# tlepoint/fhe.rs

Measured on NVIDIA H100. Metric: bfv_ct_mul_relin_per_sec_n32768_14x62bit, higher is better.
Workload: dtype u64

## Files before the change

### fhe_rs_b200/csrc/capi.cu

```cuda
#include <algorithm>
#include <atomic>
#include <cstring>
#include <map>
#include <memory>
#include <mutex>
#include <string>
#include <vector>

#include "../../include/fhe_b200.h"
#include "engine.hpp"
#include "host/precompute.hpp"

using namespace fhe_b200;

namespace {

thread_local std::string g_last_error;

struct ScalerData {
  ScalerTablesH h;
  ScalerDev dev;
};

struct LevelData {
  u32 level = 0, L = 0, E = 0, K = 0;
  RowIds ctx_ids, mul_ids;
  std::vector<u64> mul_moduli;
  ScalerData ext, down;
  bool has_sd = false;
  SwitchDownDev sd;
  u64 q_mod_t = 0;
  std::vector<u64> delta;
  const u64 *d_delta = nullptr, *d_delta_s = nullptr;
};

template <typename ToDev, typename IndexOf>
void upload_scaler_tables(ScalerData& s, const std::vector<u64>& to_moduli, ToDev&& to_dev, IndexOf&& index_of) {
  ScalerDev& d = s.dev;
  std::memset(&d, 0, sizeof(d));
  d.n_from = s.h.n_from; d.n_to = s.h.n_to; d.is_one = s.h.is_one; d.shift = s.h.shift;
  d.tg_lo = s.h.theta_gamma_lo; d.tg_hi = s.h.theta_gamma_hi; d.tg_sign = s.h.theta_gamma_sign;
  for (size_t j = 0; j < to_moduli.size(); j++) d.to_ids[j] = (unsigned short)index_of(to_moduli[j]);
  d.all_solinas = switches().no_solinas ? 0 : 1;
  for (u64 q : to_moduli)
    if ((q >> 61) != 1 || ((1ull << 62) - q) >= (1ull << 28)) d.all_solinas = 0;
  d.gamma = to_dev(s.h.gamma);
  d.omega = to_dev(s.h.omega);
  d.to_lo = to_dev(s.h.theta_omega_lo);
  d.to_hi = to_dev(s.h.theta_omega_hi);
  d.to_sign = to_dev(s.h.theta_omega_sign);
  std::vector<unsigned char> order;
  d.n_pos = 0;
  for (int sg = 0; sg < 2; sg++)
    for (size_t i = 0; i < s.h.theta_omega_sign.size(); i++)
      if ((int)s.h.theta_omega_sign[i] == sg && (s.h.theta_omega_lo[i] | s.h.theta_omega_hi[i]) != 0) {
        order.push_back((unsigned char)i);
        d.n_pos += sg == 0;
      }
  d.n_terms = (u32)order.size();
  if (order.empty()) order.push_back(0);
  d.to_order = to_dev(order);
  d.tgar_lo = to_dev(s.h.theta_garner_lo);
  d.tgar_hi = to_dev(s.h.theta_garner_hi);
}

}

struct fhe_b200_params {
  std::atomic<int> refs{1};
  int device = -1;
  u32 N = 0, logn = 0, Lmax = 0;
  std::vector<u64> moduli, ext, primes, psi;
  std::vector<u32> moduli_sizes;
  BigUint t;
  bool t_small = false;
  PlainMod t_mod{0, 0, 0};
  std::vector<NttTablesH> tables;
  std::vector<LimbDev> h_limbs;
  LimbDev* d_limbs = nullptr;
  std::vector<void*> d_allocs;
  cudaMemPool_t pool = nullptr;
  mutable cudaStream_t side[4] = {nullptr, nullptr, nullptr, nullptr};
  mutable std::mutex mu;
  mutable std::map<u32, std::unique_ptr<LevelData>> levels;
  mutable std::map<u32, int*> perms;

  template <typename T>
  T* to_dev(const std::vector<T>& v) const {
    if (device < 0 || v.empty()) return nullptr;
    T* d = nullptr;
    struct Restore {
      int prev = -1;
      ~Restore() { if (prev >= 0) cudaSetDevice(prev); }
    } restore;
    if (cudaGetDevice(&restore.prev) != cudaSuccess) { cudaGetLastError(); restore.prev = -1; }
    if (restore.prev == device) restore.prev = -1;
    else FHE_CUDA(cudaSetDevice(device));
    FHE_CUDA(cudaMalloc(&d, v.size() * sizeof(T)));
    const_cast<fhe_b200_params*>(this)->d_allocs.push_back(d);
    FHE_CUDA(cudaMemcpy(d, v.data(), v.size() * sizeof(T), cudaMemcpyHostToDevice));
    return d;
  }
  int prime_index(u64 q) const {
    for (size_t i = 0; i < primes.size(); i++)
      if (primes[i] == q) return (int)i;
    return -1;
  }
  void upload_scaler(ScalerData& s, const std::vector<u64>& to_moduli) const {
    upload_scaler_tables(s, to_moduli, [&](const auto& v) { return to_dev(v); }, [&](u64 q) { return prime_index(q); });
  }

  const LevelData& level(u32 lv) const {
    std::lock_guard<std::mutex> g(mu);
    auto it = levels.find(lv);
    if (it != levels.end()) return *it->second;
    if (lv >= Lmax) throw FheError(FHE_B200_INVALID_LEVEL, "InvalidLevel: level " + std::to_string(lv));
    std::unique_ptr<LevelData> d(new LevelData());
    d->level = lv;
    d->L = Lmax - lv;
    u32 bits = 0;
    for (u32 i = 0; i < d->L; i++) bits += moduli_sizes[i];
    d->E = (bits + 60 + 61) / 62;
    d->K = d->L + d->E;
    if (d->K > (u32)kMaxPos) throw FheError(FHE_B200_UNSUPPORTED, "too many limbs");
    std::vector<u64> ctx(moduli.begin(), moduli.begin() + d->L);
    d->mul_moduli = ctx;
    d->mul_moduli.insert(d->mul_moduli.end(), ext.begin(), ext.begin() + d->E);
    std::memset(&d->ctx_ids, 0, sizeof(RowIds));
    std::memset(&d->mul_ids, 0, sizeof(RowIds));
    d->ctx_ids.limbs_per_poly = d->L;
    d->mul_ids.limbs_per_poly = d->K;
    for (u32 i = 0; i < d->L; i++) d->ctx_ids.ids[i] = d->mul_ids.ids[i] = (unsigned short)i;
    for (u32 j = 0; j < d->E; j++) d->mul_ids.ids[d->L + j] = (unsigned short)(Lmax + j);
    RnsContextH from(ctx), to(d->mul_moduli);
    d->ext.h = make_scaler_tables(from, to, BigUint(1), BigUint(1));
    d->down.h = make_scaler_tables(to, from, t, from.product);
    upload_scaler(d->ext, d->mul_moduli);
    upload_scaler(d->down, ctx);
    if (d->L >= 2) {
      d->has_sd = true;
      u64 ql = ctx.back();
      std::vector<u64> half_mod, inv, inv_s;
      for (u32 i = 0; i + 1 < d->L; i++) {
        u64 qi = ctx[i], iv;
        if (!invmod_h(ql % qi, qi, &iv)) throw FheError(FHE_B200_INVALID_MODULUS, "NonCoprimeModuli");
        half_mod.push_back(qi - (ql / 2) % qi);
        inv.push_back(iv);
        inv_s.push_back(ModulusH(qi).shoup(iv));
      }
      d->sd.q_last = ql;
      d->sd.q_last_half = ql / 2;
      d->sd.half_mod = to_dev(half_mod);
      d->sd.inv = to_dev(inv);
      d->sd.inv_s = to_dev(inv_s);
    }
    if (t_small) d->q_mod_t = from.product.mod_u64(t_mod.t);
    std::vector<u64> delta_s;
    for (u64 qi : ctx) {
      u64 iv;
      if (!invmod_h(qi - t.mod_u64(qi), qi, &iv)) throw FheError(FHE_B200_INVALID_MODULUS, "PlaintextModulusNotCoprime");
      d->delta.push_back(iv);
      delta_s.push_back(ModulusH(qi).shoup(iv));
    }
    d->d_delta = to_dev(d->delta);
    d->d_delta_s = to_dev(delta_s);
    auto* raw = d.get();
    levels[lv] = std::move(d);
    return *raw;
  }

  const int* perm(u32 exponent) const {
    std::lock_guard<std::mutex> g(mu);
    auto it = perms.find(exponent);
    if (it != perms.end()) return it->second;
    std::vector<int> p(N);
    auto brev = [&](u32 x) {
      u32 r = 0;
      for (u32 b = 0; b < logn; b++) r |= ((x >> b) & 1) << (logn - 1 - b);
      return r;
    };
    u64 power = (exponent - 1) / 2;
    for (u32 j = 0; j < N; j++) {
      p[brev(j)] = (int)brev((u32)(power & (N - 1)));
      power += exponent;
    }
    int* d = to_dev(p);
    perms[exponent] = d;
    return d;
  }
};

struct fhe_b200_batch {
  const fhe_b200_params* par;
  u32 count, parts, level, limbs;
  int repr;
  bool mul_basis;
  u64* d;
  size_t words_per_ct() const { return ((size_t)parts * limbs) << par->logn; }
};

struct fhe_b200_ksk {
  const fhe_b200_params* par;
  u32 ct_level, ksk_level, n_dig, Lk;
  u32 log_base;
  u64 *k0, *k1;
};

struct fhe_b200_multiplicator {
  const fhe_b200_params* par;
  u32 level = 0, L = 0, K = 0;
  u32 nc_l = 0, nc_r = 0, nc_d = 0;
  std::vector<u64> mul_moduli, plan_primes;
  RowIds mul_ids;
  std::vector<LimbDev> h_limbs;
  LimbDev* d_limbs = nullptr;
  ScalerData ext_l, ext_r, down;
  std::vector<void*> d_allocs;
  template <typename T>
  T* to_dev(const std::vector<T>& v) {
    if (v.empty()) return nullptr;
    T* d = nullptr;
    FHE_CUDA(cudaMalloc(&d, v.size() * sizeof(T)));
    d_allocs.push_back(d);
    FHE_CUDA(cudaMemcpy(d, v.data(), v.size() * sizeof(T), cudaMemcpyHostToDevice));
    return d;
  }
  int prime_index(u64 q) const {
    for (size_t i = 0; i < plan_primes.size(); i++)
      if (plan_primes[i] == q) return (int)i;
    return -1;
  }
  void upload_scaler(ScalerData& sd, const std::vector<u64>& to_moduli) {
    upload_scaler_tables(sd, to_moduli, [&](const auto& v) { return to_dev(v); }, [&](u64 q) { return prime_index(q); });
  }
};

struct fhe_b200_encoder {
  const fhe_b200_params* par;
  bool has_ntt = false;
  u64 psi_t = 0;
  NttTablesH tables;
  std::vector<u32> index_map;
  std::vector<LimbDev> h_limbs;
  LimbDev* d_limbs = nullptr;
  u32* d_inv_map = nullptr;
  RowIds t_ids;
  std::vector<void*> d_allocs;
  template <typename T>
  T* to_dev(const std::vector<T>& v) {
    if (par->device < 0 || v.empty()) return nullptr;
    T* d = nullptr;
    FHE_CUDA(cudaMalloc(&d, v.size() * sizeof(T)));
    d_allocs.push_back(d);
    FHE_CUDA(cudaMemcpy(d, v.data(), v.size() * sizeof(T), cudaMemcpyHostToDevice));
    return d;
  }
};

namespace {

void params_release(const fhe_b200_params* cp) {
  fhe_b200_params* p = const_cast<fhe_b200_params*>(cp);
  if (!p || p->refs.fetch_sub(1) != 1) return;
  if (p->device >= 0) {
    int prev = -1;
    cudaGetDevice(&prev);
    cudaSetDevice(p->device);
    for (void* d : p->d_allocs) cudaFree(d);
    for (cudaStream_t ss : p->side)
      if (ss) cudaStreamDestroy(ss);
    if (p->pool) {
      cudaDeviceSynchronize();
      cudaMemPoolDestroy(p->pool);
    }
    if (prev >= 0) cudaSetDevice(prev);
    cudaGetLastError();
  }
  delete p;
}
const fhe_b200_params* params_retain(const fhe_b200_params* p) {
  const_cast<fhe_b200_params*>(p)->refs.fetch_add(1);
  return p;
}

template <typename ToDev>
LimbDev make_limb_dev(u64 q, const NttTablesH& t, ToDev&& to_dev) {
  ModulusH m(q);
  LimbDev d;
  std::memset(&d, 0, sizeof(d));
  d.p = q; d.p2 = 2 * q; d.bhi = m.bhi; d.blo = m.blo; d.c128 = m.c128;
  d.ninv = t.ninv; d.zn = t.zn;
  const u64 cc = (1ull << 62) - q;
  const bool sol = (q >> 61) == 1 && cc < (1ull << 28) && !switches().no_solinas;
  const bool sol_ntt = switches().solinas_ntt;
  auto pairs = [&](const std::vector<u64>& v, const std::vector<u64>& shoup) {
    std::vector<ulonglong2> o(v.size());
    for (size_t k = 0; k < v.size(); k++) {
      o[k].x = v[k];
      o[k].y = (sol && sol_ntt) ? (u64)((((u128)v[k]) << 32) % q) : shoup[k];
    }
    return o;
  };
  d.sol_c = sol ? cc : 0;
  d.sol_ntt = (sol && sol_ntt) ? 1 : 0;
  d.ninv_s = (sol && sol_ntt) ? (u64)((((u128)t.ninv) << 32) % q) : t.ninv_s;
  d.zn_s = (sol && sol_ntt) ? (u64)((((u128)t.zn) << 32) % q) : t.zn_s;
  d.om = to_dev(pairs(t.om, t.om_s));
  d.zi = to_dev(pairs(t.zi, t.zi_s));
  return d;
}

struct DeviceGuard {
  int prev = -1;
  explicit DeviceGuard(const fhe_b200_params* p) {
    if (p->device < 0) throw FheError(FHE_B200_NO_DEVICE, "parameter set was created without a CUDA device");
    if (cudaGetDevice(&prev) != cudaSuccess) { cudaGetLastError(); prev = -1; }
    if (prev != p->device) FHE_CUDA(cudaSetDevice(p->device));
    else prev = -1;
  }
  ~DeviceGuard() {
    if (prev >= 0) cudaSetDevice(prev);
  }
  DeviceGuard(const DeviceGuard&) = delete;
  DeviceGuard& operator=(const DeviceGuard&) = delete;
};

struct ScopedDevice {
  int prev = -1;
  explicit ScopedDevice(int device) {
    if (device < 0) return;
    if (cudaGetDevice(&prev) != cudaSuccess) prev = -1;
    if (prev == device) prev = -1;
    else cudaSetDevice(device);
    cudaGetLastError();
  }
  ~ScopedDevice() {
    if (prev >= 0) cudaSetDevice(prev);
    cudaGetLastError();
  }
};

struct DevPtr {
  void* p = nullptr;
  ~DevPtr() { if (p) { cudaFree(p); cudaGetLastError(); } }
  void* release() { void* r = p; p = nullptr; return r; }
};

struct Workspace {
  cudaStream_t st;
  cudaMemPool_t pool;
  std::vector<void*> ptrs;
  Workspace(const fhe_b200_params* par, cudaStream_t s) : st(s), pool(par->pool) {}
  u64* words(size_t n) {
    void* p = nullptr;
    FHE_CUDA(cudaMallocFromPoolAsync(&p, n * sizeof(u64), pool, st));
    ptrs.push_back(p);
    return (u64*)p;
  }
  ~Workspace() {
    for (void* p : ptrs) cudaFreeAsync(p, st);
  }
};

u32 chunk_size() { return switches().chunk; }

struct ChunkRunner {
  const fhe_b200_params* par;
  cudaStream_t user;
  u32 count, chunk, ns;
  cudaEvent_t ev[5] = {nullptr, nullptr, nullptr, nullptr, nullptr};
  static u32 streams() { return switches().streams; }
  ChunkRunner(const fhe_b200_params* p, u32 n, cudaStream_t st) : par(p), user(st), count(n), chunk(chunk_size()), ns(1) {
    if (streams() < 2 || count <= chunk || chunk < streams()) return;
    ns = streams();
    chunk = (chunk + ns - 1) / ns;
    {
      std::lock_guard<std::mutex> g(par->mu);
      for (u32 i = 0; i < ns; i++)
        if (!par->side[i]) FHE_CUDA(cudaStreamCreateWithFlags(&par->side[i], cudaStreamNonBlocking));
    }
    for (u32 i = 0; i <= ns; i++) FHE_CUDA(cudaEventCreateWithFlags(&ev[i], cudaEventDisableTiming));
    FHE_CUDA(cudaEventRecord(ev[ns], user));
    for (u32 i = 0; i < ns; i++) FHE_CUDA(cudaStreamWaitEvent(par->side[i], ev[ns], 0));
  }
  template <class F>
  void run(F&& body) {
    u32 k = 0;
    for (u32 c0 = 0; c0 < count; c0 += chunk, k++) body(c0, std::min(chunk, count - c0), ns > 1 ? par->side[k % ns] : user);
    join();
  }
  void join() {
    if (ns < 2 || joined) return;
    joined = true;
    for (u32 i = 0; i < ns; i++)
      if (cudaEventRecord(ev[i], par->side[i]) == cudaSuccess) cudaStreamWaitEvent(user, ev[i], 0);
  }
  ~ChunkRunner() {
    join();
    for (cudaEvent_t e : ev)
      if (e) cudaEventDestroy(e);
  }
  bool joined = false;
};

void check_same(const fhe_b200_batch* a, const fhe_b200_batch* b) {
  if (a->par != b->par) throw FheError(FHE_B200_CONTEXT_MISMATCH, "ParameterMismatch: batches use different parameters");
  if (a->level != b->level) throw FheError(FHE_B200_INVALID_LEVEL, "InvalidLevel: operands are at different levels");
  if (a->mul_basis != b->mul_basis || a->limbs != b->limbs)
    throw FheError(FHE_B200_CONTEXT_MISMATCH, "PolynomialContextMismatch");
}
void need_repr(const fhe_b200_batch* b, int repr) {
  if (b->repr != repr) throw FheError(FHE_B200_INVALID_REPRESENTATION, "IncorrectRepresentation");
}
const RowIds& ids_of(const fhe_b200_batch* b) {
  const LevelData& lv = b->par->level(b->level);
  return b->mul_basis ? lv.mul_ids : lv.ctx_ids;
}

void key_switch_core(const fhe_b200_params* par, const fhe_b200_ksk* k, const u64* c2, u32 cts, const u64* base0,
                     const u64* base1, u64* out0, u64* out1, u32 out_ct_rows, Workspace& ws, cudaStream_t st) {
  const LevelData& kl = par->level(k->ksk_level);
  const u32 L = k->n_dig, Lk = k->Lk;
  u64* inter = ws.words(((size_t)cts * L * Lk) << par->logn);
  bool adjacent = false;
  if (k->log_base) {
    u64* dig = ws.words(((size_t)cts * L) << par->logn);
    launch_decompose(c2, dig, cts, L, k->log_base, par->logn, st);
    launch_ntt(dig, inter, cts * L, kl.ctx_ids, par->d_limbs, par->logn, false, 1, false, st, true);
  } else {
  u64 qmax = 0, qmin = ~0ull;
  for (u32 i = 0; i < L; i++) qmax = std::max(qmax, par->moduli[i]);
  for (u32 j = 0; j < Lk; j++) qmin = std::min(qmin, par->moduli[j]);
  const bool reduce = qmax > 4 * qmin - 1 || qmin < (1ull << 8);
  adjacent = Lk > 1 && ntt_uses_tma(cts * L * Lk, kl.ctx_ids, par->logn, Lk, c2, inter);
  if (adjacent && switches().ksmac == Switches::KSMAC_FUSED &&
      launch_key_switch_tma(c2, inter, k->k0, k->k1, base0, base1, out0, out1, cts, L, Lk, out_ct_rows, kl.ctx_ids,
                            par->d_limbs, par->logn, reduce, st))
    return;
  launch_ntt(c2, inter, cts * L * Lk, kl.ctx_ids, par->d_limbs, par->logn, false, Lk, reduce, st, true, adjacent, L);
  }
  launch_ksmac(inter, k->k0, k->k1, base0, base1, out0, out1, cts, L, Lk, out_ct_rows, kl.ctx_ids, par->d_limbs,
               par->logn, st, adjacent);
}

void key_switch_apply(const fhe_b200_params* par, const fhe_b200_ksk* k, const u64* c2, u32 cts, u64* out,
                      int base_mode, u64* base, Workspace& ws, cudaStream_t st) {
  const LevelData& cl = par->level(k->ct_level);
  const u32 L = cl.L, Lk = k->Lk, logn = par->logn;
  const size_t row = (size_t)1 << logn;
  if (Lk == L) {
    const u64* b0 = base_mode == 1 ? out : base_mode == 2 ? base : nullptr;
    const u64* b1 = base_mode == 1 ? out + L * row : nullptr;
    key_switch_core(par, k, c2, cts, b0, b1, out, out + L * row, 2 * L, ws, st);
    return;
  }
  u64* cur = ws.words((size_t)cts * 2 * Lk * row);
  key_switch_core(par, k, c2, cts, nullptr, nullptr, cur, cur + Lk * row, 2 * Lk, ws, st);
  const LevelData& kl = par->level(k->ksk_level);
  launch_ntt(cur, cur, cts * 2 * Lk, kl.ctx_ids, par->d_limbs, logn, true, 1, false, st);
  for (u32 lv = k->ksk_level; lv < k->ct_level; lv++) {
    const LevelData& from = par->level(lv);
    u64* nxt = ws.words((size_t)cts * 2 * (from.L - 1) * row);
    launch_switch_down(from.sd, cur, nxt, cts * 2, from.L, from.ctx_ids, par->d_limbs, logn, st);
    cur = nxt;
  }
  launch_ntt(cur, cur, cts * 2 * L, cl.ctx_ids, par->d_limbs, logn, false, 1, false, st);
  if (base_mode == 1) {
    launch_ew(EW_ADD, out, cur, (size_t)cts * 2 * L, cl.ctx_ids, par->d_limbs, logn, st);
  } else {
    FHE_CUDA(cudaMemcpyAsync(out, cur, (size_t)cts * 2 * L * row * sizeof(u64), cudaMemcpyDeviceToDevice, st));
    if (base_mode == 2) {
      FHE_CUDA(cudaMemset2DAsync(base + L * row, 2 * L * row * sizeof(u64), 0, L * row * sizeof(u64), cts, st));
      launch_ew(EW_ADD, out, base, (size_t)cts * 2 * L, cl.ctx_ids, par->d_limbs, logn, st);
    }
  }
}

void mul_core(const fhe_b200_params* par, const LevelData& lv, const u64* a, const u64* b, u32 cts, u64* out0,
              u64* out1, int split, Workspace& ws, cudaStream_t st) {
  const u32 L = lv.L, E = lv.E, K = lv.K, logn = par->logn;
  const size_t row = (size_t)1 << logn;
  u64* A_l = ws.words((size_t)cts * 2 * L * row);
  u64* A_r = ws.words((size_t)cts * 2 * L * row);
  u64* X_l = ws.words((size_t)cts * 2 * E * row);
  u64* X_r = ws.words((size_t)cts * 2 * E * row);
  u64* T = ws.words((size_t)cts * 3 * K * row);
  RowIds ext_ids;
  std::memset(&ext_ids, 0, sizeof(ext_ids));
  ext_ids.limbs_per_poly = E;
  for (u32 j = 0; j < E; j++) ext_ids.ids[j] = lv.mul_ids.ids[L + j];
  launch_ntt(a, A_l, cts * 2 * L, lv.ctx_ids, par->d_limbs, logn, true, 1, false, st);
  launch_ntt(b, A_r, cts * 2 * L, lv.ctx_ids, par->d_limbs, logn, true, 1, false, st);
  launch_scale(lv.ext.dev, par->d_limbs, A_l, X_l, nullptr, cts * 2, E, L, E, 0, logn, st);
  launch_scale(lv.ext.dev, par->d_limbs, A_r, X_r, nullptr, cts * 2, E, L, E, 0, logn, st);
  launch_ntt(X_l, X_l, cts * 2 * E, ext_ids, par->d_limbs, logn, false, 1, false, st);
  launch_ntt(X_r, X_r, cts * 2 * E, ext_ids, par->d_limbs, logn, false, 1, false, st);
  if (!launch_tensor_inverse_ntt(a, b, X_l, X_r, T, cts, L, K, lv.mul_ids, par->d_limbs, logn, st)) {
    launch_tensor(a, b, X_l, X_r, T, cts, L, L, L, K, lv.mul_ids, par->d_limbs, logn, st);
    launch_ntt(T, T, cts * 3 * K, lv.mul_ids, par->d_limbs, logn, true, 1, false, st);
  }
  launch_scale(lv.down.dev, par->d_limbs, T, out0, out1, cts * 3, L, 0, L, split, logn, st);
}

void mul_core_parts(const fhe_b200_params* par, const LevelData& lv, const u64* a, u32 na, const u64* b, u32 nb, u32 cts,
                    u64* out, Workspace& ws, cudaStream_t st) {
  const u32 L = lv.L, E = lv.E, K = lv.K, logn = par->logn, nc = na + nb - 1;
  const size_t row = (size_t)1 << logn;
  RowIds ext_ids;
  std::memset(&ext_ids, 0, sizeof(ext_ids));
  ext_ids.limbs_per_poly = E;
  for (u32 j = 0; j < E; j++) ext_ids.ids[j] = lv.mul_ids.ids[L + j];
  const u64* src[2] = {a, b};
  const u32 np[2] = {na, nb};
  u64* X[2];
  for (int s = 0; s < 2; s++) {
    u64* pb = ws.words((size_t)cts * np[s] * L * row);
    X[s] = ws.words((size_t)cts * np[s] * E * row);
    launch_ntt(src[s], pb, cts * np[s] * L, lv.ctx_ids, par->d_limbs, logn, true, 1, false, st);
    launch_scale(lv.ext.dev, par->d_limbs, pb, X[s], nullptr, cts * np[s], E, L, E, 0, logn, st);
    launch_ntt(X[s], X[s], cts * np[s] * E, ext_ids, par->d_limbs, logn, false, 1, false, st);
  }
  u64* T = ws.words((size_t)cts * nc * K * row);
  launch_tensor_nm(a, b, X[0], X[1], T, cts, L, E, na, nb, lv.mul_ids, par->d_limbs, logn, st);
  launch_ntt(T, T, cts * nc * K, lv.mul_ids, par->d_limbs, logn, true, 1, false, st);
  launch_scale(lv.down.dev, par->d_limbs, T, out, nullptr, cts * nc, L, 0, L, 0, logn, st);
}

void mul_core_general(const fhe_b200_multiplicator* m, const u64* a, const u64* b, u32 cts, u64* out, Workspace& ws,
                      cudaStream_t st) {
  const fhe_b200_params* par = m->par;
  const LevelData& lv = par->level(m->level);
  const u32 L = m->L, K = m->K, logn = par->logn;
  const size_t row = (size_t)1 << logn;
  const u64* src[2] = {a, b};
  const ScalerData* ext[2] = {&m->ext_l, &m->ext_r};
  const u32 nc[2] = {m->nc_l, m->nc_r};
  u64* X[2] = {nullptr, nullptr};
  for (int s = 0; s < 2; s++) {
    const u32 E = K - nc[s];
    if (!E) continue;
    u64* pb = ws.words((size_t)cts * 2 * L * row);
    X[s] = ws.words((size_t)cts * 2 * E * row);
    launch_ntt(src[s], pb, cts * 2 * L, lv.ctx_ids, par->d_limbs, logn, true, 1, false, st);
    launch_scale(ext[s]->dev, m->d_limbs, pb, X[s], nullptr, cts * 2, E, nc[s], E, 0, logn, st);
    RowIds ids;
    std::memset(&ids, 0, sizeof(ids));
    ids.limbs_per_poly = E;
    for (u32 j = 0; j < E; j++) ids.ids[j] = m->mul_ids.ids[nc[s] + j];
    launch_ntt(X[s], X[s], cts * 2 * E, ids, m->d_limbs, logn, false, 1, false, st);
  }
  u64* T = ws.words((size_t)cts * 3 * K * row);
  launch_tensor(a, b, X[0], X[1], T, cts, L, nc[0], nc[1], K, m->mul_ids, m->d_limbs, logn, st);
  launch_ntt(T, T, cts * 3 * K, m->mul_ids, m->d_limbs, logn, true, 1, false, st);
  if (m->nc_d)
    FHE_CUDA(cudaMemcpy2DAsync(out, L * row * 8, T, K * row * 8, m->nc_d * row * 8, (size_t)cts * 3,
                               cudaMemcpyDeviceToDevice, st));
  launch_scale(m->down.dev, m->d_limbs, T, out + m->nc_d * row, nullptr, cts * 3, L, m->nc_d, L - m->nc_d, 0, logn, st);
}

}

extern "C" {

#define API_BEGIN try {
#define API_END                                                                   \
  }                                                                               \
  catch (const FheError& e) { g_last_error = e.what(); return e.code; }           \
  catch (const CudaFail& f) {                                                     \
    g_last_error = std::string(f.what) + ": " + cudaGetErrorString(f.err);        \
    cudaGetLastError();                                                           \
    return f.err == cudaErrorMemoryAllocation ? FHE_B200_OUT_OF_MEMORY : FHE_B200_CUDA_ERROR; \
  }                                                                               \
  catch (const std::bad_alloc&) { g_last_error = "host out of memory"; return FHE_B200_OUT_OF_MEMORY; } \
  catch (const std::exception& e) { g_last_error = e.what(); return FHE_B200_INVALID_ARGUMENT; } \
  return FHE_B200_OK;
#define REQUIRE(c, code, msg) \
  do { if (!(c)) throw FheError(code, msg); } while (0)

const char* fhe_b200_version(void) { return "fhe_b200 0.1 (sm_90a)"; }
const char* fhe_b200_last_error(void) { return g_last_error.c_str(); }
uint64_t fhe_b200_launch_count(void) { return g_launches.load(); }

static int params_build(int device, uint32_t degree, const std::vector<u64>& moduli, const uint8_t* pt,
                        uint32_t pt_len, const uint64_t* psi, fhe_b200_params** out) {
  API_BEGIN
  REQUIRE(out && pt && pt_len, FHE_B200_INVALID_ARGUMENT, "null argument");
  REQUIRE(degree >= 8 && degree <= 65536 && (degree & (degree - 1)) == 0, FHE_B200_INVALID_DEGREE,
          "InvalidPolynomialDegree: " + std::to_string(degree));
  REQUIRE(!moduli.empty() && moduli.size() < 32, FHE_B200_INVALID_ARGUMENT, "MissingCiphertextModulusSpecification");
  std::unique_ptr<fhe_b200_params, void (*)(const fhe_b200_params*)> p(new fhe_b200_params(), params_release);
  struct Restore {
    int prev = -1;
    ~Restore() { if (prev >= 0) cudaSetDevice(prev); }
  } restore;
  if (device >= 0 && cudaGetDevice(&restore.prev) != cudaSuccess) { cudaGetLastError(); restore.prev = -1; }
  p->device = device;
  p->N = degree;
  p->logn = (u32)__builtin_ctz(degree);
  p->Lmax = (u32)moduli.size();
  p->moduli = moduli;
  p->t = BigUint::from_le_bytes(pt, pt_len);
  REQUIRE(!p->t.is_zero(), FHE_B200_INVALID_ARGUMENT, "plaintext modulus is zero");
  if (p->t.bits() <= 62 && p->t.to_u64() >= 2) {
    const ModulusH tm(p->t.to_u64());
    p->t_small = true;
    p->t_mod = PlainMod{tm.p, tm.bhi, tm.blo};
  }
  BigUint Q(1);
  for (size_t i = 0; i < moduli.size(); i++) {
    ModulusH m(moduli[i]);
    for (size_t j = 0; j < i; j++) REQUIRE(moduli[j] != moduli[i], FHE_B200_INVALID_MODULUS, "DuplicateModuli");
    REQUIRE(moduli[i] % (2 * (u64)degree) == 1 && is_prime_u64(moduli[i]), FHE_B200_NTT_UNAVAILABLE,
            "CiphertextModulusNotNttFriendly: " + std::to_string(moduli[i]));
    u64 tm = p->t.mod_u64(moduli[i]), dummy;
    REQUIRE(tm != 0 && invmod_h(tm, moduli[i], &dummy), FHE_B200_INVALID_MODULUS, "PlaintextModulusNotCoprime");
    p->moduli_sizes.push_back(64 - (u32)clz64(moduli[i]));
    Q = Q * BigUint(moduli[i]);
  }
  REQUIRE(p->t < Q, FHE_B200_INVALID_ARGUMENT, "PlaintextModulusExceedsCiphertextModulus");
  u64 ub = 1ull << 62;
  while (p->ext.size() != moduli.size() + 1) {
    REQUIRE(generate_prime(62, 2 * (u64)degree, ub, &ub), FHE_B200_INVALID_MODULUS, "NotEnoughPrimes");
    bool dup = false;
    for (u64 q : p->ext) dup |= q == ub;
    for (u64 q : moduli) dup |= q == ub;
    if (!dup) p->ext.push_back(ub);
  }
  p->primes = moduli;
  p->primes.insert(p->primes.end(), p->ext.begin(), p->ext.end());
  if (device >= 0) {
    int ndev = 0;
    if (cudaGetDeviceCount(&ndev) != cudaSuccess || device >= ndev) {
      cudaGetLastError();
      throw FheError(FHE_B200_NO_DEVICE, "CUDA device " + std::to_string(device) + " not available");
    }
    FHE_CUDA(cudaSetDevice(device));
    cudaMemPoolProps props;
    std::memset(&props, 0, sizeof(props));
    props.allocType = cudaMemAllocationTypePinned;
    props.handleTypes = cudaMemHandleTypeNone;
    props.location.type = cudaMemLocationTypeDevice;
    props.location.id = device;
    FHE_CUDA(cudaMemPoolCreate(&p->pool, &props));
    unsigned long long thr = ~0ull;
    FHE_CUDA(cudaMemPoolSetAttribute(p->pool, cudaMemPoolAttrReleaseThreshold, &thr));
    int off = 0;
    FHE_CUDA(cudaMemPoolSetAttribute(p->pool, cudaMemPoolReuseAllowInternalDependencies, &off));
  }
  for (size_t i = 0; i < p->primes.size(); i++) {
    u64 q = p->primes[i];
    u64 r = psi ? psi[i] : default_psi(q, degree);
    p->psi.push_back(r);
    p->tables.push_back(make_ntt_tables(q, degree, r));
    p->h_limbs.push_back(make_limb_dev(q, p->tables.back(), [&](const std::vector<ulonglong2>& v) { return p->to_dev(v); }));
  }
  p->d_limbs = p->to_dev(p->h_limbs);
  *out = p.release();
  API_END
}

int fhe_b200_params_create(int device, uint32_t degree, const uint64_t* moduli, uint32_t n_moduli,
                           const uint8_t* plaintext_le, uint32_t plaintext_len, const uint64_t* psi,
                           fhe_b200_params** out) {
  if (!moduli || !n_moduli) { g_last_error = "null moduli"; return FHE_B200_INVALID_ARGUMENT; }
  std::vector<u64> m(moduli, moduli + n_moduli);
  return params_build(device, degree, m, plaintext_le, plaintext_len, psi, out);
}

int fhe_b200_params_create_from_sizes(int device, uint32_t degree, const uint32_t* sizes, uint32_t n_moduli,
                                      const uint8_t* plaintext_le, uint32_t plaintext_len, fhe_b200_params** out) {
  if (!sizes || !n_moduli) { g_last_error = "null sizes"; return FHE_B200_INVALID_ARGUMENT; }
  if (degree < 8 || (degree & (degree - 1))) { g_last_error = "InvalidPolynomialDegree"; return FHE_B200_INVALID_DEGREE; }
  std::vector<u64> m;
  for (uint32_t i = 0; i < n_moduli; i++) {
    if (sizes[i] > 62 || sizes[i] < 10) { g_last_error = "InvalidModulusSize"; return FHE_B200_INVALID_MODULUS; }
    u64 ub = 1ull << sizes[i];
    for (;;) {
      u64 q;
      if (!generate_prime((int)sizes[i], 2 * (u64)degree, ub, &q)) { g_last_error = "NotEnoughPrimes"; return FHE_B200_INVALID_MODULUS; }
      bool dup = false;
      for (u64 x : m) dup |= x == q;
      if (!dup) { m.push_back(q); break; }
      ub = q;
    }
  }
  return params_build(device, degree, m, plaintext_le, plaintext_len, nullptr, out);
}

int fhe_b200_params_destroy(fhe_b200_params* p) {
  params_release(p);
  return FHE_B200_OK;
}
uint32_t fhe_b200_params_degree(const fhe_b200_params* p) { return p ? p->N : 0; }
uint32_t fhe_b200_params_n_moduli(const fhe_b200_params* p) { return p ? p->Lmax : 0; }
int fhe_b200_params_moduli(const fhe_b200_params* p, uint64_t* out) {
  if (!p || !out) return FHE_B200_INVALID_ARGUMENT;
  for (u32 i = 0; i < p->Lmax; i++) out[i] = p->moduli[i];
  return FHE_B200_OK;
}
int fhe_b200_params_mul_basis(const fhe_b200_params* p, uint32_t level, uint64_t* out, uint32_t* n) {
  API_BEGIN
  REQUIRE(p && n, FHE_B200_INVALID_ARGUMENT, "null argument");
  const LevelData& lv = p->level(level);
  *n = lv.K;
  if (out) for (u32 i = 0; i < lv.K; i++) out[i] = lv.mul_moduli[i];
  API_END
}
int fhe_b200_params_psi(const fhe_b200_params* p, uint64_t q, uint64_t* psi) {
  if (!p || !psi) return FHE_B200_INVALID_ARGUMENT;
  int i = p->prime_index(q);
  if (i < 0) { g_last_error = "prime not in parameter set"; return FHE_B200_INVALID_MODULUS; }
  *psi = p->psi[i];
  return FHE_B200_OK;
}

static int batch_alloc(const fhe_b200_params* p, uint32_t count, uint32_t parts, uint32_t level, int repr,
                       bool mul_basis, fhe_b200_batch** out) {
  API_BEGIN
  REQUIRE(p && out, FHE_B200_INVALID_ARGUMENT, "null argument");
  REQUIRE(count > 0 && parts > 0, FHE_B200_INVALID_ARGUMENT, "empty batch");
  REQUIRE(repr == FHE_B200_POWER_BASIS || repr == FHE_B200_NTT, FHE_B200_INVALID_REPRESENTATION, "bad representation");
  DeviceGuard g(p);
  const LevelData& lv = p->level(level);
  std::unique_ptr<fhe_b200_batch> b(new fhe_b200_batch());
  b->par = p; b->count = count; b->parts = parts; b->level = level; b->repr = repr;
  b->mul_basis = mul_basis;
  b->limbs = mul_basis ? lv.K : lv.L;
  b->d = nullptr;
  FHE_CUDA(cudaMalloc(&b->d, b->words_per_ct() * count * sizeof(u64)));
  params_retain(p);
  *out = b.release();
  API_END
}
int fhe_b200_batch_alloc(const fhe_b200_params* p, uint32_t count, uint32_t parts, uint32_t level, int repr,
                         fhe_b200_batch** out) {
  return batch_alloc(p, count, parts, level, repr, false, out);
}
int fhe_b200_batch_alloc_mul_basis(const fhe_b200_params* p, uint32_t count, uint32_t parts, uint32_t level,
                                   int repr, fhe_b200_batch** out) {
  return batch_alloc(p, count, parts, level, repr, true, out);
}
int fhe_b200_batch_free(fhe_b200_batch* b) {
  if (!b) return FHE_B200_OK;
  {
    ScopedDevice g(b->par->device);
    cudaFree(b->d);
    cudaGetLastError();
  }
  params_release(b->par);
  delete b;
  return FHE_B200_OK;
}
int fhe_b200_batch_info(const fhe_b200_batch* b, uint32_t* count, uint32_t* parts, uint32_t* level, uint32_t* limbs,
                        int* repr) {
  if (!b) return FHE_B200_INVALID_ARGUMENT;
  if (count) *count = b->count;
  if (parts) *parts = b->parts;
  if (level) *level = b->level;
  if (limbs) *limbs = b->limbs;
  if (repr) *repr = b->repr;
  return FHE_B200_OK;
}
int fhe_b200_batch_upload(fhe_b200_batch* b, uint32_t first, uint32_t n, const uint64_t* host, void* stream) {
  API_BEGIN
  REQUIRE(b && host, FHE_B200_INVALID_ARGUMENT, "null argument");
  REQUIRE((uint64_t)first + n <= b->count, FHE_B200_INVALID_ARGUMENT, "range exceeds batch");
  DeviceGuard g(b->par);
  size_t w = b->words_per_ct();
  FHE_CUDA(cudaMemcpyAsync(b->d + w * first, host, w * n * sizeof(u64), cudaMemcpyHostToDevice, (cudaStream_t)stream));
  API_END
}
int fhe_b200_batch_download(const fhe_b200_batch* b, uint32_t first, uint32_t n, uint64_t* host, void* stream) {
  API_BEGIN
  REQUIRE(b && host, FHE_B200_INVALID_ARGUMENT, "null argument");
  REQUIRE((uint64_t)first + n <= b->count, FHE_B200_INVALID_ARGUMENT, "range exceeds batch");
  DeviceGuard g(b->par);
  size_t w = b->words_per_ct();
  FHE_CUDA(cudaMemcpyAsync(host, b->d + w * first, w * n * sizeof(u64), cudaMemcpyDeviceToHost, (cudaStream_t)stream));
  FHE_CUDA(cudaStreamSynchronize((cudaStream_t)stream));
  API_END
}
int fhe_b200_batch_download_async(const fhe_b200_batch* b, uint32_t first, uint32_t n, uint64_t* host, void* stream) {
  API_BEGIN
  REQUIRE(b && host, FHE_B200_INVALID_ARGUMENT, "null argument");
  REQUIRE((uint64_t)first + n <= b->count, FHE_B200_INVALID_ARGUMENT, "range exceeds batch");
  DeviceGuard g(b->par);
  size_t w = b->words_per_ct();
  FHE_CUDA(cudaMemcpyAsync(host, b->d + w * first, w * n * sizeof(u64), cudaMemcpyDeviceToHost, (cudaStream_t)stream));
  API_END
}
int fhe_b200_batch_copy(fhe_b200_batch* dst, const fhe_b200_batch* src, void* stream) {
  API_BEGIN
  REQUIRE(dst && src, FHE_B200_INVALID_ARGUMENT, "null argument");
  check_same(dst, src);
  REQUIRE(dst->parts == src->parts && dst->count == src->count, FHE_B200_BAD_POLY_COUNT, "shapes differ");
  DeviceGuard g(src->par);
  FHE_CUDA(cudaMemcpyAsync(dst->d, src->d, src->words_per_ct() * src->count * sizeof(u64), cudaMemcpyDeviceToDevice,
                           (cudaStream_t)stream));
  dst->repr = src->repr;
  API_END
}
int fhe_b200_host_alloc(size_t bytes, int write_combined, void** out) {
  API_BEGIN
  REQUIRE(out && bytes, FHE_B200_INVALID_ARGUMENT, "null argument");
  void* p = nullptr;
  FHE_CUDA(cudaHostAlloc(&p, bytes, cudaHostAllocPortable | (write_combined ? cudaHostAllocWriteCombined : 0)));
  *out = p;
  API_END
}
int fhe_b200_host_free(void* p) {
  API_BEGIN
  if (p) FHE_CUDA(cudaFreeHost(p));
  API_END
}
int fhe_b200_batch_device_ptr(const fhe_b200_batch* b, uint64_t** dptr, size_t* n_words) {
  if (!b || !dptr) return FHE_B200_INVALID_ARGUMENT;
  *dptr = (uint64_t*)b->d;
  if (n_words) *n_words = b->words_per_ct() * b->count;
  return FHE_B200_OK;
}

int fhe_b200_ksk_upload(const fhe_b200_params* p, uint32_t ciphertext_level, uint32_t ksk_level, const uint64_t* c0,
                        const uint64_t* c1, uint32_t n_digits, fhe_b200_ksk** out) {
  API_BEGIN
  REQUIRE(p && c0 && c1 && out, FHE_B200_INVALID_ARGUMENT, "null argument");
  DeviceGuard g(p);
  const LevelData& cl = p->level(ciphertext_level);
  const LevelData& kl = p->level(ksk_level);
  REQUIRE(ksk_level <= ciphertext_level, FHE_B200_INVALID_LEVEL, "key level must not exceed the ciphertext level");
  u32 log_base = 0;
  if (kl.L == 1) {
    REQUIRE(cl.L == 1, FHE_B200_CONTEXT_MISMATCH, "ParameterMismatch: a single-modulus key serves the last level only");
    const u64 q = p->moduli[0];
    const u32 log_modulus = 64 - (u32)clz64(q - 1);
    log_base = log_modulus / 2;
    REQUIRE(log_base >= 1, FHE_B200_UNSUPPORTED, "modulus too small for the decomposition");
    REQUIRE(n_digits == (log_modulus + log_base - 1) / log_base, FHE_B200_CONTEXT_MISMATCH,
            "n_digits must be ceil(log_modulus / log_base) for a single-modulus key");
  } else {
    REQUIRE(n_digits == cl.L, FHE_B200_CONTEXT_MISMATCH, "n_digits must equal the ciphertext level's limb count");
  }
  std::unique_ptr<fhe_b200_ksk> k(new fhe_b200_ksk());
  k->par = p; k->ct_level = ciphertext_level; k->ksk_level = ksk_level; k->n_dig = n_digits; k->Lk = kl.L;
  k->log_base = log_base;
  size_t bytes = ((size_t)n_digits * kl.L << p->logn) * sizeof(u64);
  DevPtr g0, g1;
  FHE_CUDA(cudaMalloc(&g0.p, bytes));
  FHE_CUDA(cudaMalloc(&g1.p, bytes));
  const size_t rowb = sizeof(u64) << p->logn;
  for (u32 i = 0; i < n_digits; i++) {
    FHE_CUDA(cudaMemcpy2D((char*)g0.p + i * rowb, n_digits * rowb, (const char*)c0 + (size_t)i * kl.L * rowb, rowb, rowb,
                          kl.L, cudaMemcpyHostToDevice));
    FHE_CUDA(cudaMemcpy2D((char*)g1.p + i * rowb, n_digits * rowb, (const char*)c1 + (size_t)i * kl.L * rowb, rowb, rowb,
                          kl.L, cudaMemcpyHostToDevice));
  }
  k->k0 = (u64*)g0.release();
  k->k1 = (u64*)g1.release();
  params_retain(p);
  *out = k.release();
  API_END
}
int fhe_b200_ksk_free(fhe_b200_ksk* k) {
  if (!k) return FHE_B200_OK;
  {
    ScopedDevice g(k->par->device);
    cudaFree(k->k0);
    cudaFree(k->k1);
    cudaGetLastError();
  }
  params_release(k->par);
  delete k;
  return FHE_B200_OK;
}

static int ntt_batch(fhe_b200_batch* b, bool inverse, void* stream) {
  API_BEGIN
  REQUIRE(b, FHE_B200_INVALID_ARGUMENT, "null argument");
  need_repr(b, inverse ? FHE_B200_NTT : FHE_B200_POWER_BASIS);
  DeviceGuard g(b->par);
  launch_ntt(b->d, b->d, b->count * b->parts * b->limbs, ids_of(b), b->par->d_limbs, b->par->logn, inverse, 1, false,
             (cudaStream_t)stream);
  FHE_CUDA(cudaGetLastError());
  b->repr = inverse ? FHE_B200_POWER_BASIS : FHE_B200_NTT;
  API_END
}
int fhe_b200_ntt_forward(fhe_b200_batch* b, void* stream) { return ntt_batch(b, false, stream); }
int fhe_b200_ntt_backward(fhe_b200_batch* b, void* stream) { return ntt_batch(b, true, stream); }

static int ew(EwOp op, fhe_b200_batch* a, const fhe_b200_batch* b, void* stream) {
  API_BEGIN
  REQUIRE(a && (b || op == EW_NEG), FHE_B200_INVALID_ARGUMENT, "null argument");
  if (b) {
    check_same(a, b);
    REQUIRE(a->parts == b->parts && a->count == b->count, FHE_B200_BAD_POLY_COUNT, "operand shapes differ");
    REQUIRE(a->repr == b->repr, FHE_B200_INVALID_REPRESENTATION, "IncorrectRepresentation");
  }
  DeviceGuard g(a->par);
  launch_ew(op, a->d, b ? b->d : nullptr, (size_t)a->count * a->parts * a->limbs, ids_of(a), a->par->d_limbs,
            a->par->logn, (cudaStream_t)stream);
  FHE_CUDA(cudaGetLastError());
  API_END
}
int fhe_b200_add(fhe_b200_batch* a, const fhe_b200_batch* b, void* stream) { return ew(EW_ADD, a, b, stream); }
int fhe_b200_sub(fhe_b200_batch* a, const fhe_b200_batch* b, void* stream) { return ew(EW_SUB, a, b, stream); }
int fhe_b200_neg(fhe_b200_batch* a, void* stream) { return ew(EW_NEG, a, nullptr, stream); }

static int plain_op(fhe_b200_batch* a, const uint64_t* host_polys, uint32_t n_polys, u32 op, void* stream) {
  API_BEGIN
  REQUIRE(a && host_polys, FHE_B200_INVALID_ARGUMENT, "null argument");
  REQUIRE(n_polys == 1 || n_polys == a->count, FHE_B200_INVALID_ARGUMENT, "n_polys must be 1 or the batch size");
  REQUIRE(a->parts >= 1, FHE_B200_BAD_POLY_COUNT, "empty ciphertext");
  need_repr(a, FHE_B200_NTT);
  const fhe_b200_params* par = a->par;
  DeviceGuard g(par);
  cudaStream_t st = (cudaStream_t)stream;
  Workspace ws(par, st);
  const size_t words = ((size_t)n_polys * a->limbs) << par->logn;
  u64* pt = ws.words(words);
  FHE_CUDA(cudaMemcpyAsync(pt, host_polys, words * sizeof(u64), cudaMemcpyHostToDevice, st));
  launch_mul_plain(a->d, pt, a->count, a->parts, n_polys, ids_of(a), par->d_limbs, par->logn, st, op);
  FHE_CUDA(cudaGetLastError());
  API_END
}
int fhe_b200_mul_plain(fhe_b200_batch* a, const uint64_t* host_polys, uint32_t n_polys, void* stream) {
  return plain_op(a, host_polys, n_polys, 0, stream);
}
int fhe_b200_add_plain(fhe_b200_batch* a, const uint64_t* host_polys, uint32_t n_polys, int subtract, void* stream) {
  return plain_op(a, host_polys, n_polys, subtract ? 2 : 1, stream);
}

int fhe_b200_dot_product_scalar(const fhe_b200_batch* cts, const fhe_b200_batch* pts, uint32_t n_terms,
                                fhe_b200_batch* out, void* stream) {
  API_BEGIN
  REQUIRE(cts && pts && out, FHE_B200_INVALID_ARGUMENT, "null argument");
  REQUIRE(n_terms > 0 && cts->count > 0 && pts->count > 0, FHE_B200_INVALID_ARGUMENT, "DotProductError::EmptyInput");
  check_same(cts, pts);
  check_same(cts, out);
  REQUIRE(pts->parts == 1, FHE_B200_BAD_POLY_COUNT, "plaintext batch must hold one polynomial per entry");
  REQUIRE(out->parts == cts->parts, FHE_B200_BAD_POLY_COUNT, "DotProductError::CiphertextPolynomialCountMismatch");
  const size_t total = (size_t)out->count * n_terms;
  REQUIRE((cts->count == total || cts->count == n_terms) && (pts->count == total || pts->count == n_terms),
          FHE_B200_INVALID_ARGUMENT, "DotProductError::OperandCountMismatch");
  need_repr(cts, FHE_B200_NTT);
  need_repr(pts, FHE_B200_NTT);
  DeviceGuard g(cts->par);
  launch_dot(cts->d, pts->d, out->d, out->count, n_terms, cts->parts, cts->count, pts->count, ids_of(cts),
             cts->par->d_limbs, cts->par->logn, (cudaStream_t)stream);
  FHE_CUDA(cudaGetLastError());
  out->repr = FHE_B200_NTT;
  API_END
}

int fhe_b200_encoder_create(const fhe_b200_params* p, const uint64_t* psi_t, fhe_b200_encoder** out) {
  API_BEGIN
  REQUIRE(p && out, FHE_B200_INVALID_ARGUMENT, "null argument");
  ScopedDevice g(p->device);
  std::unique_ptr<fhe_b200_encoder> e(new fhe_b200_encoder());
  struct Cleanup {
    fhe_b200_encoder* e;
    ~Cleanup() { if (e) { for (void* d : e->d_allocs) cudaFree(d); cudaGetLastError(); } }
  } cleanup{e.get()};
  e->par = p;
  const u32 N = p->N;
  e->index_map.resize(N);
  auto brev = [&](u64 x) {
    u32 r = 0;
    for (u32 b = 0; b < p->logn; b++) r |= (u32)((x >> b) & 1) << (p->logn - 1 - b);
    return r;
  };
  const u64 m = 2 * (u64)N;
  u64 pos = 1;
  for (u32 i = 0; i < N / 2; i++) {
    e->index_map[i] = brev((pos - 1) >> 1);
    e->index_map[N / 2 + i] = brev((m - pos - 1) >> 1);
    pos = (pos * 3) & (m - 1);
  }
  std::vector<u32> inv(N);
  for (u32 i = 0; i < N; i++) inv[e->index_map[i]] = i;
  e->h_limbs = p->h_limbs;
  std::memset(&e->t_ids, 0, sizeof(RowIds));
  e->t_ids.limbs_per_poly = 1;
  e->t_ids.ids[0] = (unsigned short)p->h_limbs.size();
  const u64 t = p->t_mod.t;
  e->has_ntt = p->t_small && t % m == 1 && is_prime_u64(t);
  if (e->has_ntt) {
    e->psi_t = psi_t ? *psi_t : default_psi(t, N);
    e->tables = make_ntt_tables(t, N, e->psi_t);
    e->h_limbs.push_back(make_limb_dev(t, e->tables, [&](const std::vector<ulonglong2>& v) { return e->to_dev(v); }));
  }
  e->d_limbs = e->to_dev(e->h_limbs);
  e->d_inv_map = e->to_dev(inv);
  params_retain(p);
  cleanup.e = nullptr;
  *out = e.release();
  API_END
}

int fhe_b200_encoder_free(fhe_b200_encoder* e) {
  if (!e) return FHE_B200_OK;
  if (e->par->device >= 0) {
    ScopedDevice g(e->par->device);
    for (void* d : e->d_allocs) cudaFree(d);
    cudaGetLastError();
  }
  params_release(e->par);
  delete e;
  return FHE_B200_OK;
}

int fhe_b200_encode(const fhe_b200_encoder* e, int encoding, int is_signed, const void* values, size_t n_values,
                    fhe_b200_batch* out, void* stream) {
  API_BEGIN
  REQUIRE(e, FHE_B200_INVALID_ARGUMENT, "null encoder");
  const fhe_b200_params* par = e->par;
  DeviceGuard g(par);
  REQUIRE(out, FHE_B200_INVALID_ARGUMENT, "null argument");
  REQUIRE(encoding == FHE_B200_ENCODING_POLY || encoding == FHE_B200_ENCODING_SIMD, FHE_B200_INVALID_ARGUMENT,
          "unknown encoding");
  REQUIRE(par->t_small, FHE_B200_UNSUPPORTED, "the plaintext modulus does not fit a u64 Modulus");
  const bool simd = encoding == FHE_B200_ENCODING_SIMD;
  REQUIRE(!simd || e->has_ntt, FHE_B200_NTT_UNAVAILABLE, "EncodingError::SimdUnavailable");
  REQUIRE(out->par == par, FHE_B200_CONTEXT_MISMATCH, "ParameterMismatch");
  REQUIRE(!out->mul_basis, FHE_B200_CONTEXT_MISMATCH, "PolynomialContextMismatch");
  const LevelData& lv = par->level(out->level);
  REQUIRE(out->parts == 1, FHE_B200_BAD_POLY_COUNT, "a plaintext batch has one polynomial per entry");
  const size_t N = par->N;
  const size_t count = std::max<size_t>(1, (n_values + N - 1) / N);
  REQUIRE(out->count == count, FHE_B200_INVALID_ARGUMENT, "batch must hold max(1, ceil(n_values / N)) plaintexts");
  REQUIRE(values || !n_values, FHE_B200_INVALID_ARGUMENT, "null values");
  const u32 L = lv.L, logn = par->logn;
  const bool poly_u64 = !simd && !is_signed;
  u64 qmin = ~0ull;
  for (u32 j = 0; j < L; j++) qmin = std::min(qmin, par->moduli[j]);
  const bool reduce = poly_u64 || par->t_mod.t > 4 * qmin - 1;
  const char* src = (const char*)values;
  ChunkRunner chunks(par, (u32)count, (cudaStream_t)stream);
  chunks.run([&](u32 c0, u32 n, cudaStream_t st) {
    Workspace ws(par, st);
    const size_t v0 = (size_t)c0 * N, vn = n_values > v0 ? std::min(n_values - v0, (size_t)n * N) : 0;
    u64* staged = ws.words(std::max<size_t>(vn, 1));
    if (vn) FHE_CUDA(cudaMemcpyAsync(staged, src + v0 * sizeof(u64), vn * sizeof(u64), cudaMemcpyDefault, st));
    const u64* coeffs = staged;
    if (!(poly_u64 && vn == (size_t)n * N)) {
      u64* c = ws.words((size_t)n * N);
      launch_encode_load(staged, c, n, vn, simd ? e->d_inv_map : nullptr, is_signed != 0, par->t_mod, logn, st);
      if (simd) launch_ntt(c, c, n, e->t_ids, e->d_limbs, logn, true, 1, false, st);
      coeffs = c;
    }
    launch_ntt(coeffs, out->d + (size_t)c0 * L * N, n * L, lv.ctx_ids, e->d_limbs, logn, false, L, reduce, st);
  });
  FHE_CUDA(cudaGetLastError());
  out->repr = FHE_B200_NTT;
  API_END
}

static void check_plain_batch(const fhe_b200_batch* a, const fhe_b200_batch* pts) {
  REQUIRE(a && pts, FHE_B200_INVALID_ARGUMENT, "null argument");
  check_same(a, pts);
  REQUIRE(pts->count == 1 || pts->count == a->count, FHE_B200_INVALID_ARGUMENT, "plaintext count must be 1 or the batch size");
  REQUIRE(a->parts >= 1 && pts->parts == 1, FHE_B200_BAD_POLY_COUNT, "plaintext batch must hold one polynomial per entry");
  need_repr(a, FHE_B200_NTT);
  need_repr(pts, FHE_B200_NTT);
}

int fhe_b200_mul_plain_batch(fhe_b200_batch* a, const fhe_b200_batch* pts, void* stream) {
  API_BEGIN
  check_plain_batch(a, pts);
  DeviceGuard g(a->par);
  launch_mul_plain(a->d, pts->d, a->count, a->parts, pts->count, ids_of(a), a->par->d_limbs, a->par->logn,
                   (cudaStream_t)stream, 0);
  FHE_CUDA(cudaGetLastError());
  API_END
}

int fhe_b200_add_plain_batch(fhe_b200_batch* a, const fhe_b200_batch* pts, int subtract, void* stream) {
  API_BEGIN
  check_plain_batch(a, pts);
  const fhe_b200_params* par = a->par;
  REQUIRE(par->t_small && par->t_mod.t < par->moduli[0], FHE_B200_UNSUPPORTED,
          "to_poly needs t below the first ciphertext modulus");
  DeviceGuard g(par);
  const LevelData& lv = par->level(a->level);
  const u32 L = lv.L, logn = par->logn;
  const size_t N = par->N;
  u64 qmin = ~0ull;
  for (u32 j = 0; j < L; j++) qmin = std::min(qmin, par->moduli[j]);
  const bool reduce = par->t_mod.t > 4 * qmin - 1;
  RowIds q0_ids;
  std::memset(&q0_ids, 0, sizeof(RowIds));
  q0_ids.limbs_per_poly = 1;
  auto to_poly = [&](u32 p0, u32 n, u64* m, Workspace& ws, cudaStream_t st) {
    u64* x = ws.words((size_t)n * N);
    FHE_CUDA(cudaMemcpy2DAsync(x, N * 8, pts->d + (size_t)p0 * L * N, L * N * 8, N * 8, n, cudaMemcpyDeviceToDevice, st));
    launch_ntt(x, x, n, q0_ids, par->d_limbs, logn, true, 1, false, st);
    launch_to_poly_load(x, (size_t)n * N, par->t_mod, lv.q_mod_t, st);
    launch_ntt(x, m, n * L, lv.ctx_ids, par->d_limbs, logn, false, L, reduce, st);
  };
  cudaStream_t user = (cudaStream_t)stream;
  Workspace shared_ws(par, user);
  const bool shared = pts->count == 1;
  u64* m_shared = nullptr;
  if (shared) {
    m_shared = shared_ws.words((size_t)L * N);
    to_poly(0, 1, m_shared, shared_ws, user);
  }
  ChunkRunner chunks(par, a->count, user);
  chunks.run([&](u32 c0, u32 n, cudaStream_t st) {
    Workspace ws(par, st);
    const u64* m = m_shared;
    if (!shared) {
      u64* mc = ws.words((size_t)n * L * N);
      to_poly(c0, n, mc, ws, st);
      m = mc;
    }
    launch_add_scaled(a->d + (size_t)c0 * a->parts * L * N, m, n, a->parts, shared ? 1 : n, lv.d_delta, lv.d_delta_s,
                      subtract != 0, lv.ctx_ids, par->d_limbs, logn, st);
  });
  FHE_CUDA(cudaGetLastError());
  API_END
}

int fhe_b200_mul(const fhe_b200_batch* a, const fhe_b200_batch* b, fhe_b200_batch* out3, void* stream) {
  API_BEGIN
  REQUIRE(a && b && out3, FHE_B200_INVALID_ARGUMENT, "null argument");
  check_same(a, b);
  check_same(a, out3);
  REQUIRE(!a->mul_basis, FHE_B200_CONTEXT_MISMATCH, "PolynomialContextMismatch");
  REQUIRE(a->parts >= 1 && b->parts >= 1 && out3->parts == a->parts + b->parts - 1, FHE_B200_BAD_POLY_COUNT,
          "MultiplicationPolynomialCount: expected n x m -> n + m - 1 parts");
  REQUIRE(a->count == b->count && a->count == out3->count, FHE_B200_INVALID_ARGUMENT, "batch sizes differ");
  need_repr(a, FHE_B200_NTT);
  need_repr(b, FHE_B200_NTT);
  DeviceGuard g(a->par);
  cudaStream_t st_user = (cudaStream_t)stream;
  const fhe_b200_params* par = a->par;
  const LevelData& lv = par->level(a->level);
  const size_t row = (size_t)1 << par->logn;
  const u32 na = a->parts, nb = b->parts, nc = na + nb - 1;
  ChunkRunner chunks(par, a->count, st_user);
  chunks.run([&](u32 c0, u32 n, cudaStream_t st) {
    Workspace ws(par, st);
    u64* o = out3->d + (size_t)c0 * nc * lv.L * row;
    const u64* pa = a->d + (size_t)c0 * na * lv.L * row;
    const u64* pb = b->d + (size_t)c0 * nb * lv.L * row;
    if (na == 2 && nb == 2) mul_core(par, lv, pa, pb, n, o, nullptr, 0, ws, st);
    else mul_core_parts(par, lv, pa, na, pb, nb, n, o, ws, st);
    launch_ntt(o, o, n * nc * lv.L, lv.ctx_ids, par->d_limbs, par->logn, false, 1, false, st);
  });
  FHE_CUDA(cudaGetLastError());
  out3->repr = FHE_B200_NTT;
  API_END
}

static void check_ksk(const fhe_b200_ksk* k, const fhe_b200_params* par, u32 level) {
  REQUIRE(k->par == par, FHE_B200_CONTEXT_MISMATCH, "ParameterMismatch: key belongs to other parameters");
  REQUIRE(k->ct_level == level, FHE_B200_INVALID_LEVEL, "InvalidLevel: key is for another ciphertext level");
}

int fhe_b200_relinearize(const fhe_b200_batch* ct3, const fhe_b200_ksk* rk, fhe_b200_batch* out2, void* stream) {
  API_BEGIN
  REQUIRE(ct3 && rk && out2, FHE_B200_INVALID_ARGUMENT, "null argument");
  check_same(ct3, out2);
  REQUIRE(!ct3->mul_basis, FHE_B200_CONTEXT_MISMATCH, "PolynomialContextMismatch");
  REQUIRE(ct3->parts == 3 && out2->parts == 2, FHE_B200_BAD_POLY_COUNT, "InvalidPolynomialCount: expected 3 -> 2");
  REQUIRE(ct3->count == out2->count, FHE_B200_INVALID_ARGUMENT, "batch sizes differ");
  need_repr(ct3, FHE_B200_NTT);
  check_ksk(rk, ct3->par, ct3->level);
  DeviceGuard g(ct3->par);
  cudaStream_t st_user = (cudaStream_t)stream;
  const fhe_b200_params* par = ct3->par;
  const LevelData& lv = par->level(ct3->level);
  const size_t row = (size_t)1 << par->logn, L = lv.L;
  ChunkRunner chunks(par, ct3->count, st_user);
  chunks.run([&](u32 c0, u32 n, cudaStream_t st) {
    Workspace ws(par, st);
    const u64* src = ct3->d + (size_t)c0 * 3 * L * row;
    u64* dst = out2->d + (size_t)c0 * 2 * L * row;
    u64* c2 = ws.words((size_t)n * L * row);
    FHE_CUDA(cudaMemcpy2DAsync(dst, 2 * L * row * 8, src, 3 * L * row * 8, 2 * L * row * 8, n, cudaMemcpyDeviceToDevice, st));
    FHE_CUDA(cudaMemcpy2DAsync(c2, L * row * 8, src + 2 * L * row, 3 * L * row * 8, L * row * 8, n, cudaMemcpyDeviceToDevice, st));
    launch_ntt(c2, c2, n * (u32)L, lv.ctx_ids, par->d_limbs, par->logn, true, 1, false, st);
    key_switch_apply(par, rk, c2, n, dst, 1, nullptr, ws, st);
  });
  FHE_CUDA(cudaGetLastError());
  out2->repr = FHE_B200_NTT;
  API_END
}

int fhe_b200_mul_relin(const fhe_b200_batch* a, const fhe_b200_batch* b, const fhe_b200_ksk* rk, int mod_switch,
                       fhe_b200_batch* out2, void* stream) {
  API_BEGIN
  REQUIRE(a && b && rk && out2, FHE_B200_INVALID_ARGUMENT, "null argument");
  check_same(a, b);
  REQUIRE(a->par == out2->par, FHE_B200_CONTEXT_MISMATCH, "ParameterMismatch");
  REQUIRE(!a->mul_basis && !out2->mul_basis, FHE_B200_CONTEXT_MISMATCH, "PolynomialContextMismatch");
  REQUIRE(a->parts == 2 && b->parts == 2 && out2->parts == 2, FHE_B200_BAD_POLY_COUNT,
          "MultiplicationPolynomialCount: expected 2 x 2 -> 2");
  REQUIRE(a->count == b->count && a->count == out2->count, FHE_B200_INVALID_ARGUMENT, "batch sizes differ");
  need_repr(a, FHE_B200_NTT);
  need_repr(b, FHE_B200_NTT);
  check_ksk(rk, a->par, a->level);
  const fhe_b200_params* par = a->par;
  const LevelData& lv = par->level(a->level);
  if (mod_switch) {
    REQUIRE(lv.L >= 2, FHE_B200_NO_MORE_CONTEXT, "NoMoreContext");
    REQUIRE(out2->level == a->level + 1, FHE_B200_INVALID_LEVEL, "output batch must be one level down");
  } else {
    REQUIRE(out2->level == a->level, FHE_B200_INVALID_LEVEL, "output batch must be at the operand level");
  }
  DeviceGuard g(par);
  const size_t row = (size_t)1 << par->logn, L = lv.L;
  ChunkRunner chunks(par, a->count, (cudaStream_t)stream);
  chunks.run([&](u32 c0, u32 n, cudaStream_t st) {
    Workspace ws(par, st);
    u64* o = mod_switch ? ws.words((size_t)n * 2 * L * row) : out2->d + (size_t)c0 * 2 * L * row;
    u64* c2 = ws.words((size_t)n * L * row);
    mul_core(par, lv, a->d + (size_t)c0 * 2 * L * row, b->d + (size_t)c0 * 2 * L * row, n, o, c2, 1, ws, st);
    launch_ntt(o, o, n * 2 * (u32)L, lv.ctx_ids, par->d_limbs, par->logn, false, 1, false, st);
    key_switch_apply(par, rk, c2, n, o, 1, nullptr, ws, st);
    if (mod_switch) {
      launch_ntt(o, o, n * 2 * (u32)L, lv.ctx_ids, par->d_limbs, par->logn, true, 1, false, st);
      u64* dst = out2->d + (size_t)c0 * 2 * (L - 1) * row;
      launch_switch_down(lv.sd, o, dst, n * 2, (u32)L, lv.ctx_ids, par->d_limbs, par->logn, st);
      const LevelData& nl = par->level(a->level + 1);
      launch_ntt(dst, dst, n * 2 * (u32)(L - 1), nl.ctx_ids, par->d_limbs, par->logn, false, 1, false, st);
    }
  });
  FHE_CUDA(cudaGetLastError());
  out2->repr = FHE_B200_NTT;
  API_END
}

int fhe_b200_multiplicator_create(const fhe_b200_params* p, uint32_t level, const uint8_t* lhs_num, uint32_t lhs_num_len,
                                  const uint8_t* lhs_den, uint32_t lhs_den_len, const uint8_t* rhs_num,
                                  uint32_t rhs_num_len, const uint8_t* rhs_den, uint32_t rhs_den_len,
                                  const uint64_t* extended_basis, uint32_t n_basis, const uint64_t* psi,
                                  const uint8_t* post_num, uint32_t post_num_len, const uint8_t* post_den,
                                  uint32_t post_den_len, fhe_b200_multiplicator** out) {
  API_BEGIN
  REQUIRE(p && out && extended_basis && n_basis && lhs_num && lhs_den && rhs_num && rhs_den && post_num && post_den,
          FHE_B200_INVALID_ARGUMENT, "null argument");
  REQUIRE(n_basis <= (u32)kMaxPos, FHE_B200_UNSUPPORTED, "too many limbs");
  const LevelData& lv = p->level(level);
  DeviceGuard g(p);
  std::unique_ptr<fhe_b200_multiplicator> m(new fhe_b200_multiplicator());
  struct Cleanup {
    fhe_b200_multiplicator* m;
    ~Cleanup() { if (m) { for (void* d : m->d_allocs) cudaFree(d); cudaGetLastError(); } }
  } cleanup{m.get()};
  m->par = p;
  m->level = level;
  m->L = lv.L;
  m->K = n_basis;
  m->mul_moduli.assign(extended_basis, extended_basis + n_basis);
  for (u32 i = 0; i < n_basis; i++) {
    const u64 q = extended_basis[i];
    for (u32 j = 0; j < i; j++) REQUIRE(extended_basis[j] != q, FHE_B200_INVALID_MODULUS, "DuplicateModuli");
    REQUIRE(q >= 2 && (q >> 62) == 0, FHE_B200_INVALID_MODULUS, "InvalidModulus: " + std::to_string(q));
    REQUIRE(q % (2 * (u64)p->N) == 1 && is_prime_u64(q), FHE_B200_NTT_UNAVAILABLE,
            "modulus does not support the NTT: " + std::to_string(q));
  }
  m->plan_primes = p->primes;
  m->h_limbs = p->h_limbs;
  std::memset(&m->mul_ids, 0, sizeof(RowIds));
  m->mul_ids.limbs_per_poly = n_basis;
  for (u32 i = 0; i < n_basis; i++) {
    const u64 q = extended_basis[i];
    int idx = m->prime_index(q);
    if (idx >= 0 && psi && psi[i] != p->psi[(size_t)idx] && (size_t)idx < p->primes.size())
      throw FheError(FHE_B200_INVALID_ARGUMENT, "psi differs from the parameter set's root for " + std::to_string(q));
    if (idx < 0) {
      const u64 r = psi ? psi[i] : default_psi(q, p->N);
      NttTablesH t = make_ntt_tables(q, p->N, r);
      idx = (int)m->plan_primes.size();
      m->plan_primes.push_back(q);
      m->h_limbs.push_back(make_limb_dev(q, t, [&](const std::vector<ulonglong2>& v) { return m->to_dev(v); }));
    }
    m->mul_ids.ids[i] = (unsigned short)idx;
  }
  m->d_limbs = m->to_dev(m->h_limbs);
  std::vector<u64> base(p->moduli.begin(), p->moduli.begin() + lv.L);
  RnsContextH from(base), to(m->mul_moduli);
  auto factor = [](const uint8_t* b, uint32_t n) { return BigUint::from_le_bytes(b, n); };
  const BigUint ln = factor(lhs_num, lhs_num_len), ld = factor(lhs_den, lhs_den_len);
  const BigUint rn = factor(rhs_num, rhs_num_len), rd = factor(rhs_den, rhs_den_len);
  const BigUint pn = factor(post_num, post_num_len), pd = factor(post_den, post_den_len);
  REQUIRE(!ld.is_zero() && !rd.is_zero() && !pd.is_zero(), FHE_B200_INVALID_ARGUMENT, "zero denominator");
  m->ext_l.h = make_scaler_tables(from, to, ln, ld);
  m->ext_r.h = make_scaler_tables(from, to, rn, rd);
  m->down.h = make_scaler_tables(to, from, pn, pd);
  auto common = [&](const ScalerData& sd, const std::vector<u64>& x, const std::vector<u64>& y) {
    u32 n = 0;
    if (sd.h.is_one)
      while (n < x.size() && n < y.size() && x[n] == y[n]) n++;
    return n;
  };
  m->nc_l = common(m->ext_l, base, m->mul_moduli);
  m->nc_r = common(m->ext_r, base, m->mul_moduli);
  m->nc_d = common(m->down, m->mul_moduli, base);
  m->upload_scaler(m->ext_l, m->mul_moduli);
  m->upload_scaler(m->ext_r, m->mul_moduli);
  m->upload_scaler(m->down, base);
  params_retain(p);
  cleanup.m = nullptr;
  *out = m.release();
  API_END
}

int fhe_b200_multiplicator_free(fhe_b200_multiplicator* m) {
  if (!m) return FHE_B200_OK;
  if (m->par->device >= 0) {
    ScopedDevice g(m->par->device);
    for (void* d : m->d_allocs) cudaFree(d);
    cudaGetLastError();
  }
  params_release(m->par);
  delete m;
  return FHE_B200_OK;
}

int fhe_b200_multiplicator_multiply(const fhe_b200_multiplicator* m, const fhe_b200_batch* a, const fhe_b200_batch* b,
                                    const fhe_b200_ksk* rk, int mod_switch, fhe_b200_batch* out, void* stream) {
  API_BEGIN
  REQUIRE(m && a && b && out, FHE_B200_INVALID_ARGUMENT, "null argument");
  const fhe_b200_params* par = m->par;
  REQUIRE(a->par == par && b->par == par && out->par == par, FHE_B200_CONTEXT_MISMATCH, "ParameterMismatch");
  REQUIRE(a->level == m->level && b->level == m->level, FHE_B200_INVALID_LEVEL, "InvalidLevel");
  REQUIRE(!a->mul_basis && !b->mul_basis && !out->mul_basis, FHE_B200_CONTEXT_MISMATCH, "PolynomialContextMismatch");
  const u32 out_parts = rk ? 2 : 3;
  REQUIRE(a->parts == 2 && b->parts == 2 && out->parts == out_parts, FHE_B200_BAD_POLY_COUNT,
          "MultiplicationPolynomialCount");
  REQUIRE(a->count == b->count && a->count == out->count, FHE_B200_INVALID_ARGUMENT, "batch sizes differ");
  need_repr(a, FHE_B200_NTT);
  need_repr(b, FHE_B200_NTT);
  if (rk) {
    REQUIRE(rk->par == par && rk->ct_level == m->level, FHE_B200_CONTEXT_MISMATCH,
            "ParameterMismatch: relinearization key and multiplicator contexts differ");
  }
  const LevelData& lv = par->level(m->level);
  if (mod_switch) {
    REQUIRE(lv.L >= 2, FHE_B200_NO_MORE_CONTEXT, "NoMoreContext");
    REQUIRE(out->level == m->level + 1, FHE_B200_INVALID_LEVEL, "output batch must be one level down");
  } else {
    REQUIRE(out->level == m->level, FHE_B200_INVALID_LEVEL, "output batch must be at the operand level");
  }
  DeviceGuard g(par);
  const size_t row = (size_t)1 << par->logn, L = lv.L;
  ChunkRunner chunks(par, a->count, (cudaStream_t)stream);
  chunks.run([&](u32 c0, u32 n, cudaStream_t st) {
    Workspace ws(par, st);
    const bool direct = !rk && !mod_switch;
    u64* W = direct ? out->d + (size_t)c0 * 3 * L * row : ws.words((size_t)n * 3 * L * row);
    mul_core_general(m, a->d + (size_t)c0 * 2 * L * row, b->d + (size_t)c0 * 2 * L * row, n, W, ws, st);
    u64* o = W;
    if (rk) {
      o = mod_switch ? ws.words((size_t)n * 2 * L * row) : out->d + (size_t)c0 * 2 * L * row;
      u64* c2 = ws.words((size_t)n * L * row);
      FHE_CUDA(cudaMemcpy2DAsync(o, 2 * L * row * 8, W, 3 * L * row * 8, 2 * L * row * 8, n, cudaMemcpyDeviceToDevice, st));
      FHE_CUDA(cudaMemcpy2DAsync(c2, L * row * 8, W + 2 * L * row, 3 * L * row * 8, L * row * 8, n,
                                 cudaMemcpyDeviceToDevice, st));
      launch_ntt(o, o, n * 2 * (u32)L, lv.ctx_ids, par->d_limbs, par->logn, false, 1, false, st);
      key_switch_apply(par, rk, c2, n, o, 1, nullptr, ws, st);
    } else {
      launch_ntt(o, o, n * 3 * (u32)L, lv.ctx_ids, par->d_limbs, par->logn, false, 1, false, st);
    }
    if (mod_switch) {
      launch_ntt(o, o, n * out_parts * (u32)L, lv.ctx_ids, par->d_limbs, par->logn, true, 1, false, st);
      u64* dst = out->d + (size_t)c0 * out_parts * (L - 1) * row;
      launch_switch_down(lv.sd, o, dst, n * out_parts, (u32)L, lv.ctx_ids, par->d_limbs, par->logn, st);
      const LevelData& nl = par->level(m->level + 1);
      launch_ntt(dst, dst, n * out_parts * (u32)(L - 1), nl.ctx_ids, par->d_limbs, par->logn, false, 1, false, st);
    }
  });
  FHE_CUDA(cudaGetLastError());
  out->repr = FHE_B200_NTT;
  API_END
}

int fhe_b200_substitute(const fhe_b200_batch* in, uint32_t exponent, fhe_b200_batch* out, void* stream) {
  API_BEGIN
  REQUIRE(in && out && in != out, FHE_B200_INVALID_ARGUMENT, "null or aliased argument");
  check_same(in, out);
  REQUIRE(in->parts == out->parts && in->count == out->count, FHE_B200_BAD_POLY_COUNT, "shapes differ");
  const fhe_b200_params* par = in->par;
  exponent %= 2 * par->N;
  REQUIRE(exponent & 1, FHE_B200_INVALID_EXPONENT, "InvalidSubstitutionExponent");
  DeviceGuard g(par);
  const size_t rows = (size_t)in->count * in->parts * in->limbs;
  if (in->repr == FHE_B200_NTT)
    launch_gather(in->d, out->d, rows, par->perm(exponent), par->logn, (cudaStream_t)stream);
  else
    launch_substitute_power(in->d, out->d, rows, exponent, ids_of(in), par->d_limbs, par->logn, (cudaStream_t)stream);
  FHE_CUDA(cudaGetLastError());
  out->repr = in->repr;
  API_END
}

int fhe_b200_galois(const fhe_b200_batch* ct, uint32_t exponent, const fhe_b200_ksk* gk, fhe_b200_batch* out,
                    void* stream) {
  API_BEGIN
  REQUIRE(ct && gk && out && ct != out, FHE_B200_INVALID_ARGUMENT, "null or aliased argument");
  check_same(ct, out);
  REQUIRE(!ct->mul_basis, FHE_B200_CONTEXT_MISMATCH, "PolynomialContextMismatch");
  REQUIRE(ct->parts == 2 && out->parts == 2, FHE_B200_BAD_POLY_COUNT, "InvalidPolynomialCount: expected 2");
  REQUIRE(ct->count == out->count, FHE_B200_INVALID_ARGUMENT, "batch sizes differ");
  need_repr(ct, FHE_B200_NTT);
  check_ksk(gk, ct->par, ct->level);
  const fhe_b200_params* par = ct->par;
  exponent %= 2 * par->N;
  REQUIRE(exponent & 1, FHE_B200_INVALID_EXPONENT, "InvalidSubstitutionExponent");
  DeviceGuard g(par);
  const LevelData& lv = par->level(ct->level);
  const size_t row = (size_t)1 << par->logn, L = lv.L;
  const int* perm = par->perm(exponent);
  ChunkRunner chunks(par, ct->count, (cudaStream_t)stream);
  chunks.run([&](u32 c0, u32 n, cudaStream_t st) {
    Workspace ws(par, st);
    const u64* src = ct->d + (size_t)c0 * 2 * L * row;
    u64* dst = out->d + (size_t)c0 * 2 * L * row;
    u64* s = ws.words((size_t)n * 2 * L * row);
    u64* c2 = ws.words((size_t)n * L * row);
    launch_gather(src, s, (size_t)n * 2 * L, perm, par->logn, st);
    FHE_CUDA(cudaMemcpy2DAsync(c2, L * row * 8, s + L * row, 2 * L * row * 8, L * row * 8, n, cudaMemcpyDeviceToDevice, st));
    launch_ntt(c2, c2, n * (u32)L, lv.ctx_ids, par->d_limbs, par->logn, true, 1, false, st);
    key_switch_apply(par, gk, c2, n, dst, 2, s, ws, st);
  });
  FHE_CUDA(cudaGetLastError());
  out->repr = FHE_B200_NTT;
  API_END
}

int fhe_b200_key_switch(const fhe_b200_batch* pb, uint32_t part, const fhe_b200_ksk* k, fhe_b200_batch* out2,
                        void* stream) {
  API_BEGIN
  REQUIRE(pb && k && out2, FHE_B200_INVALID_ARGUMENT, "null argument");
  REQUIRE(pb->par == out2->par && pb->par == k->par, FHE_B200_CONTEXT_MISMATCH, "ParameterMismatch");
  REQUIRE(!pb->mul_basis && !out2->mul_basis, FHE_B200_CONTEXT_MISMATCH, "PolynomialContextMismatch");
  REQUIRE(part < pb->parts && out2->parts == 2, FHE_B200_BAD_POLY_COUNT, "bad part index / output parts");
  REQUIRE(pb->level == k->ct_level && out2->level == k->ksk_level, FHE_B200_INVALID_LEVEL, "InvalidLevel");
  REQUIRE(pb->count == out2->count, FHE_B200_INVALID_ARGUMENT, "batch sizes differ");
  need_repr(pb, FHE_B200_POWER_BASIS);
  const fhe_b200_params* par = pb->par;
  DeviceGuard g(par);
  cudaStream_t st_user = (cudaStream_t)stream;
  const size_t row = (size_t)1 << par->logn, L = pb->limbs, Lk = k->Lk;
  ChunkRunner chunks(par, pb->count, st_user);
  chunks.run([&](u32 c0, u32 n, cudaStream_t st) {
    Workspace ws(par, st);
    u64* c2 = ws.words((size_t)n * L * row);
    FHE_CUDA(cudaMemcpy2DAsync(c2, L * row * 8, pb->d + ((size_t)c0 * pb->parts + part) * L * row,
                               pb->parts * L * row * 8, L * row * 8, n, cudaMemcpyDeviceToDevice, st));
    u64* dst = out2->d + (size_t)c0 * 2 * Lk * row;
    key_switch_core(par, k, c2, n, nullptr, nullptr, dst, dst + Lk * row, 2 * (u32)Lk, ws, st);
  });
  FHE_CUDA(cudaGetLastError());
  out2->repr = FHE_B200_NTT;
  API_END
}

int fhe_b200_switch_down(fhe_b200_batch* b, void* stream) {
  API_BEGIN
  REQUIRE(b, FHE_B200_INVALID_ARGUMENT, "null argument");
  REQUIRE(!b->mul_basis, FHE_B200_CONTEXT_MISMATCH, "PolynomialContextMismatch");
  need_repr(b, FHE_B200_NTT);
  const fhe_b200_params* par = b->par;
  const LevelData& lv = par->level(b->level);
  REQUIRE(lv.L >= 2, FHE_B200_NO_MORE_CONTEXT, "NoMoreContext");
  DeviceGuard g(par);
  cudaStream_t st = (cudaStream_t)stream;
  const LevelData& nl = par->level(b->level + 1);
  const u32 polys = b->count * b->parts;
  Workspace ws(par, st);
  u64* tmp = ws.words((size_t)polys * nl.L << par->logn);
  launch_ntt(b->d, b->d, polys * lv.L, lv.ctx_ids, par->d_limbs, par->logn, true, 1, false, st);
  launch_switch_down(lv.sd, b->d, tmp, polys, lv.L, lv.ctx_ids, par->d_limbs, par->logn, st);
  launch_ntt(tmp, b->d, polys * nl.L, nl.ctx_ids, par->d_limbs, par->logn, false, 1, false, st);
  FHE_CUDA(cudaGetLastError());
  b->level += 1;
  b->limbs = nl.L;
  API_END
}

int fhe_b200_scale(const fhe_b200_batch* in, int which, fhe_b200_batch* out, void* stream) {
  API_BEGIN
  REQUIRE(in && out && in != out, FHE_B200_INVALID_ARGUMENT, "null or aliased argument");
  REQUIRE(in->par == out->par, FHE_B200_CONTEXT_MISMATCH, "ParameterMismatch");
  REQUIRE(in->level == out->level, FHE_B200_INVALID_LEVEL, "InvalidLevel");
  REQUIRE(in->count == out->count && in->parts == out->parts, FHE_B200_BAD_POLY_COUNT, "shapes differ");
  REQUIRE(which == 0 || which == 1, FHE_B200_INVALID_ARGUMENT, "which must be 0 or 1");
  REQUIRE(in->mul_basis == (which == 1) && out->mul_basis == (which == 0), FHE_B200_CONTEXT_MISMATCH,
          "PolynomialContextMismatch");
  need_repr(in, FHE_B200_NTT);
  const fhe_b200_params* par = in->par;
  DeviceGuard g(par);
  cudaStream_t st = (cudaStream_t)stream;
  const LevelData& lv = par->level(in->level);
  const size_t row = (size_t)1 << par->logn;
  const u32 polys = in->count * in->parts;
  Workspace ws(par, st);
  u64* pb = ws.words((size_t)polys * in->limbs * row);
  launch_ntt(in->d, pb, polys * in->limbs, ids_of(in), par->d_limbs, par->logn, true, 1, false, st);
  if (which == 0) {
    FHE_CUDA(cudaMemcpy2DAsync(out->d, lv.K * row * 8, in->d, lv.L * row * 8, lv.L * row * 8, polys,
                               cudaMemcpyDeviceToDevice, st));
    u64* x = ws.words((size_t)polys * lv.E * row);
    launch_scale(lv.ext.dev, par->d_limbs, pb, x, nullptr, polys, lv.E, lv.L, lv.E, 0, par->logn, st);
    RowIds ext_ids;
    std::memset(&ext_ids, 0, sizeof(ext_ids));
    ext_ids.limbs_per_poly = lv.E;
    for (u32 j = 0; j < lv.E; j++) ext_ids.ids[j] = lv.mul_ids.ids[lv.L + j];
    launch_ntt(x, x, polys * lv.E, ext_ids, par->d_limbs, par->logn, false, 1, false, st);
    FHE_CUDA(cudaMemcpy2DAsync(out->d + lv.L * row, lv.K * row * 8, x, lv.E * row * 8, lv.E * row * 8, polys,
                               cudaMemcpyDeviceToDevice, st));
  } else {
    launch_scale(lv.down.dev, par->d_limbs, pb, out->d, nullptr, polys, lv.L, 0, lv.L, 0, par->logn, st);
    launch_ntt(out->d, out->d, polys * lv.L, lv.ctx_ids, par->d_limbs, par->logn, false, 1, false, st);
  }
  FHE_CUDA(cudaGetLastError());
  out->repr = FHE_B200_NTT;
  API_END
}

static PackDev pack_desc(const fhe_b200_batch* b) {
  const fhe_b200_params* par = b->par;
  const LevelData& lv = par->level(b->level);
  PackDev P;
  std::memset(&P, 0, sizeof(P));
  P.limbs = b->limbs;
  u32 off = 0;
  for (u32 i = 0; i < b->limbs; i++) {
    const u64 q = b->mul_basis ? lv.mul_moduli[i] : par->moduli[i];
    const u32 nb = 64 - (u32)clz64(q - 1);
    P.nbits[i] = (unsigned char)nb;
    P.offs[i] = off;
    off += nb * (par->N / 8);
  }
  P.poly_bytes = off;
  return P;
}
int fhe_b200_poly_packed_bytes(const fhe_b200_params* p, uint32_t level, size_t* nbytes) {
  API_BEGIN
  REQUIRE(p && nbytes, FHE_B200_INVALID_ARGUMENT, "null argument");
  const LevelData& lv = p->level(level);
  size_t n = 0;
  for (u32 i = 0; i < lv.L; i++) n += (size_t)(64 - clz64(p->moduli[i] - 1)) * (p->N / 8);
  *nbytes = n;
  API_END
}
int fhe_b200_batch_packed_bytes(const fhe_b200_batch* b, size_t* nbytes) {
  API_BEGIN
  REQUIRE(b && nbytes, FHE_B200_INVALID_ARGUMENT, "null argument");
  *nbytes = pack_desc(b).poly_bytes;
  API_END
}
int fhe_b200_batch_pack(const fhe_b200_batch* b, uint32_t first, uint32_t n, uint8_t* host_out, void* stream) {
  API_BEGIN
  REQUIRE(b && host_out, FHE_B200_INVALID_ARGUMENT, "null argument");
  REQUIRE((uint64_t)first + n <= b->count, FHE_B200_INVALID_ARGUMENT, "range exceeds batch");
  const fhe_b200_params* par = b->par;
  DeviceGuard g(par);
  cudaStream_t st = (cudaStream_t)stream;
  const PackDev P = pack_desc(b);
  const size_t rows = (size_t)n * b->parts * b->limbs, row = (size_t)1 << par->logn;
  Workspace ws(par, st);
  const u64* src = b->d + b->words_per_ct() * first;
  if (b->repr == FHE_B200_NTT) {
    u64* pb = ws.words(rows * row);
    launch_ntt(src, pb, (u32)rows, ids_of(b), par->d_limbs, par->logn, true, 1, false, st);
    src = pb;
  }
  const size_t nbytes = (size_t)n * b->parts * P.poly_bytes;
  unsigned char* dbytes = (unsigned char*)ws.words((nbytes + 7) / 8);
  launch_pack(P, src, dbytes, rows, par->logn, st);
  FHE_CUDA(cudaGetLastError());
  FHE_CUDA(cudaMemcpyAsync(host_out, dbytes, nbytes, cudaMemcpyDeviceToHost, st));
  FHE_CUDA(cudaStreamSynchronize(st));
  API_END
}
int fhe_b200_batch_unpack(fhe_b200_batch* b, uint32_t first, uint32_t n, const uint8_t* host_in, void* stream) {
  API_BEGIN
  REQUIRE(b && host_in, FHE_B200_INVALID_ARGUMENT, "null argument");
  REQUIRE((uint64_t)first + n <= b->count, FHE_B200_INVALID_ARGUMENT, "range exceeds batch");
  const fhe_b200_params* par = b->par;
  DeviceGuard g(par);
  cudaStream_t st = (cudaStream_t)stream;
  const PackDev P = pack_desc(b);
  const size_t rows = (size_t)n * b->parts * b->limbs;
  Workspace ws(par, st);
  const size_t nbytes = (size_t)n * b->parts * P.poly_bytes;
  unsigned char* dbytes = (unsigned char*)ws.words((nbytes + 7) / 8);
  FHE_CUDA(cudaMemcpyAsync(dbytes, host_in, nbytes, cudaMemcpyHostToDevice, st));
  u64* dst = b->d + b->words_per_ct() * first;
  launch_unpack(P, dbytes, dst, rows, par->logn, st);
  if (b->repr == FHE_B200_NTT)
    launch_ntt(dst, dst, (u32)rows, ids_of(b), par->d_limbs, par->logn, false, 1, false, st);
  FHE_CUDA(cudaGetLastError());
  API_END
}

int fhe_b200_sync(void* stream) {
  API_BEGIN
  FHE_CUDA(cudaStreamSynchronize((cudaStream_t)stream));
  API_END
}

int fhe_b200_debug_scaler_tables(const fhe_b200_params* p, uint32_t level, int which, uint32_t* n_from, uint32_t* n_to,
                                 uint32_t* shift, uint64_t* gamma, uint64_t* omega, uint64_t* theta_gamma,
                                 uint64_t* theta_omega_lo, uint64_t* theta_omega_hi, uint8_t* theta_omega_sign,
                                 uint64_t* theta_garner_lo, uint64_t* theta_garner_hi) {
  API_BEGIN
  REQUIRE(p, FHE_B200_INVALID_ARGUMENT, "null argument");
  const LevelData& lv = p->level(level);
  const ScalerTablesH& h = which ? lv.down.h : lv.ext.h;
  if (n_from) *n_from = h.n_from;
  if (n_to) *n_to = h.n_to;
  if (shift) *shift = h.shift;
  auto cp = [](uint64_t* dst, const std::vector<u64>& v) {
    if (dst) for (size_t i = 0; i < v.size(); i++) dst[i] = v[i];
  };
  cp(gamma, h.gamma);
  cp(omega, h.omega);
  if (theta_gamma) { theta_gamma[0] = h.theta_gamma_lo; theta_gamma[1] = h.theta_gamma_hi; theta_gamma[2] = h.theta_gamma_sign; }
  cp(theta_omega_lo, h.theta_omega_lo);
  cp(theta_omega_hi, h.theta_omega_hi);
  if (theta_omega_sign) for (size_t i = 0; i < h.theta_omega_sign.size(); i++) theta_omega_sign[i] = h.theta_omega_sign[i];
  cp(theta_garner_lo, h.theta_garner_lo);
  cp(theta_garner_hi, h.theta_garner_hi);
  API_END
}

int fhe_b200_debug_ntt_tables(const fhe_b200_params* p, uint64_t q, uint64_t* omegas, uint64_t* omegas_shoup,
                              uint64_t* zetas_inv, uint64_t* zetas_inv_shoup, uint64_t* size_inv) {
  API_BEGIN
  REQUIRE(p, FHE_B200_INVALID_ARGUMENT, "null argument");
  int i = p->prime_index(q);
  REQUIRE(i >= 0, FHE_B200_INVALID_MODULUS, "prime not in parameter set");
  const NttTablesH& t = p->tables[i];
  auto cp = [](uint64_t* dst, const std::vector<u64>& v) {
    if (dst) for (size_t k = 0; k < v.size(); k++) dst[k] = v[k];
  };
  cp(omegas, t.om);
  cp(omegas_shoup, t.om_s);
  cp(zetas_inv, t.zi);
  cp(zetas_inv_shoup, t.zi_s);
  if (size_inv) *size_inv = t.ninv;
  API_END
}

int fhe_b200_debug_encoder_tables(const fhe_b200_encoder* e, uint32_t level, uint32_t* index_map, uint64_t* omegas,
                                  uint64_t* zetas_inv, uint64_t* q_mod_t, uint64_t* delta) {
  API_BEGIN
  REQUIRE(e, FHE_B200_INVALID_ARGUMENT, "null argument");
  const fhe_b200_params* p = e->par;
  const LevelData& lv = p->level(level);
  if (index_map) std::copy(e->index_map.begin(), e->index_map.end(), index_map);
  if (omegas || zetas_inv) {
    REQUIRE(e->has_ntt, FHE_B200_NTT_UNAVAILABLE, "NttOperatorUnavailable: plaintext modulus");
    if (omegas) std::copy(e->tables.om.begin(), e->tables.om.end(), omegas);
    if (zetas_inv) std::copy(e->tables.zi.begin(), e->tables.zi.end(), zetas_inv);
  }
  if (q_mod_t) {
    REQUIRE(p->t_small, FHE_B200_UNSUPPORTED, "the plaintext modulus does not fit a u64 Modulus");
    *q_mod_t = lv.q_mod_t;
  }
  if (delta) std::copy(lv.delta.begin(), lv.delta.end(), delta);
  API_END
}

}
```

### fhe_rs_b200/csrc/engine.hpp

```cpp
#pragma once
#include <atomic>
#include <cuda.h>
#include <cuda_runtime.h>

#include "ntt.cuh"

namespace fhe_b200 {

extern std::atomic<unsigned long long> g_launches;

struct Switches {
  enum Ntt { NTT_FAST, NTT_AUTO, NTT_TMA };
  enum Ksmac { KSMAC_FUSED, KSMAC_TMA, KSMAC_CLASSIC };
  u32 chunk;
  u32 streams;
  Ntt ntt;
  bool generic_ntt;
  bool solinas_ntt;
  bool no_solinas;
  bool no_tensor_fusion;
  bool classic_scaler;
  Ksmac ksmac;
  int tma_cols;
  int scale_unroll;
  u32 ks_stages;
  bool generic_tiles() const { return generic_ntt || solinas_ntt; }
  bool tma_allowed() const { return ntt != NTT_FAST && !generic_tiles(); }
};
const Switches& switches();

typedef CUresult (*EncodeTiledFn)(CUtensorMap*, CUtensorMapDataType, cuuint32_t, void*, const cuuint64_t*,
                                  const cuuint64_t*, const cuuint32_t*, const cuuint32_t*, CUtensorMapInterleave,
                                  CUtensorMapSwizzle, CUtensorMapL2promotion, CUtensorMapFloatOOBfill);
EncodeTiledFn tensor_map_encoder();
bool box_map(CUtensorMap* m, const u64* base, u64 rows, u32 logn, u32 box_cols, u32 box_rows);
int sm_count();

struct CudaFail {
  cudaError_t err;
  const char* what;
};
#define FHE_CUDA(x)                                         \
  do {                                                      \
    cudaError_t e__ = (x);                                  \
    if (e__ != cudaSuccess) throw CudaFail{e__, #x};        \
  } while (0)

void ensure_dynamic_smem(const void* kernel, size_t bytes);

struct RowIds {
  u32 limbs_per_poly;
  unsigned short ids[kMaxPos];
};

void launch_ntt(const u64* in, u64* out, u32 n_rows, const RowIds& ids, const LimbDev* limbs, u32 logn,
                bool inverse, u32 in_div, bool reduce_on_load, cudaStream_t st, bool lazy_out = false,
                bool digit_adjacent = false, u32 n_dig = 1);

bool launch_tensor_inverse_ntt(const u64* a, const u64* b, const u64* xa, const u64* xb, u64* T, u32 cts, u32 L, u32 K,
                               const RowIds& mul_ids, const LimbDev* limbs, u32 logn, cudaStream_t st);

enum EwOp { EW_ADD = 0, EW_SUB = 1, EW_NEG = 2 };
void launch_ew(EwOp op, u64* a, const u64* b, size_t n_rows, const RowIds& ids, const LimbDev* limbs, u32 logn,
               cudaStream_t st);

void launch_mul_plain(u64* a, const u64* pt, u32 cts, u32 parts, u32 n_pt, const RowIds& ids, const LimbDev* limbs,
                      u32 logn, cudaStream_t st, u32 op = 0);

void launch_dot(const u64* ct, const u64* pt, u64* out, u32 groups, u32 n_terms, u32 parts, u32 ct_count,
                u32 pt_count, const RowIds& ids, const LimbDev* limbs, u32 logn, cudaStream_t st);

void launch_tensor(const u64* a, const u64* b, const u64* xa, const u64* xb, u64* out, u32 cts, u32 L, u32 nca,
                   u32 ncb, u32 K, const RowIds& mul_ids, const LimbDev* limbs, u32 logn, cudaStream_t st);

void launch_tensor_nm(const u64* a, const u64* b, const u64* xa, const u64* xb, u64* out, u32 cts, u32 L, u32 E, u32 na,
                      u32 nb, const RowIds& mul_ids, const LimbDev* limbs, u32 logn, cudaStream_t st);

struct ScalerDev {
  u32 n_from, n_to, is_one, shift;
  u64 tg_lo, tg_hi;
  u32 tg_sign;
  u32 all_solinas;
  const u64* gamma;
  const u64* omega;
  const u64* to_lo;
  const u64* to_hi;
  const unsigned char* to_sign;
  const unsigned char* to_order;
  u32 n_pos, n_terms;
  const u64* tgar_lo;
  const u64* tgar_hi;
  unsigned short to_ids[kMaxPos];
};
void launch_scale(const ScalerDev& S, const LimbDev* limbs, const u64* in, u64* out0, u64* out1, u32 polys,
                  u32 out_rows_per_poly, u32 start, u32 n_out, int split3, u32 logn, cudaStream_t st);

void launch_ksmac(const u64* inter, const u64* k0, const u64* k1, const u64* base0, const u64* base1, u64* out0,
                  u64* out1, u32 cts, u32 n_dig, u32 Lk, u32 out_ct_rows, const RowIds& ids, const LimbDev* limbs,
                  u32 logn, cudaStream_t st, bool adjacent = false);

bool ntt_uses_tma(u32 n_rows, const RowIds& ids, u32 logn, u32 in_div, const u64* in, const u64* out);

bool launch_key_switch_tma(const u64* c2, u64* inter, const u64* k0, const u64* k1, const u64* base0,
                           const u64* base1, u64* out0, u64* out1, u32 cts, u32 n_dig, u32 Lk, u32 out_ct_rows,
                           const RowIds& ids, const LimbDev* limbs, u32 logn, bool reduce, cudaStream_t st);

void launch_decompose(const u64* in, u64* out, size_t polys, u32 n_dig, u32 log_base, u32 logn, cudaStream_t st);

void launch_gather(const u64* in, u64* out, size_t n_rows, const int* perm, u32 logn, cudaStream_t st);
void launch_substitute_power(const u64* in, u64* out, size_t n_rows, u32 exponent, const RowIds& ids,
                             const LimbDev* limbs, u32 logn, cudaStream_t st);

struct SwitchDownDev {
  u64 q_last, q_last_half;
  const u64* half_mod;
  const u64* inv;
  const u64* inv_s;
};
void launch_switch_down(const SwitchDownDev& S, const u64* in, u64* out, u32 polys, u32 L, const RowIds& ids,
                        const LimbDev* limbs, u32 logn, cudaStream_t st);

struct PlainMod {
  u64 t, bhi, blo;
};
void launch_encode_load(const u64* staged, u64* coeffs, u32 n_pt, size_t n_values, const u32* inv_map, bool is_signed,
                        const PlainMod& T, u32 logn, cudaStream_t st);
void launch_to_poly_load(u64* x, size_t n_words, const PlainMod& T, u64 q_mod_t, cudaStream_t st);
void launch_add_scaled(u64* a, const u64* m, u32 cts, u32 parts, u32 n_pt, const u64* delta, const u64* delta_s,
                       bool subtract, const RowIds& ids, const LimbDev* limbs, u32 logn, cudaStream_t st);

struct PackDev {
  u32 limbs;
  unsigned char nbits[kMaxPos];
  u32 offs[kMaxPos];
  u32 poly_bytes;
};
void launch_pack(const PackDev& P, const u64* words, unsigned char* bytes, size_t n_rows, u32 logn, cudaStream_t st);
void launch_unpack(const PackDev& P, const unsigned char* bytes, u64* words, size_t n_rows, u32 logn, cudaStream_t st);

}
```

### fhe_rs_b200/csrc/ntt.cu

```cuda
#include <algorithm>
#include <climits>
#include <cstdint>
#include <cstdlib>
#include <cstring>
#include <map>
#include <mutex>
#include <utility>

#include "engine.hpp"
#include "ntt_fast.cuh"
#include "ntt_tma.cuh"

namespace fhe_b200 {

std::atomic<unsigned long long> g_launches{0};

const Switches& switches() {
  static const Switches s = [] {
    auto set = [](const char* name) { return getenv(name) != nullptr; };
    auto is = [](const char* name, const char* value) {
      const char* e = getenv(name);
      return e && !strcmp(e, value);
    };
    auto number = [](const char* name, int dflt) {
      const char* e = getenv(name);
      return e ? atoi(e) : dflt;
    };
    auto clamped = [&](const char* name, int dflt, int lo, int hi) {
      const int v = number(name, dflt);
      return (u32)(v < lo ? lo : v > hi ? hi : v);
    };
    Switches w;
    w.chunk = clamped("FHE_B200_CHUNK", 256, 1, INT_MAX);
    w.streams = clamped("FHE_B200_STREAMS", 2, 1, 4);
    w.ntt = is("FHE_B200_NTT", "fast") ? Switches::NTT_FAST : is("FHE_B200_NTT", "tma") ? Switches::NTT_TMA
                                                                                         : Switches::NTT_AUTO;
    w.generic_ntt = set("FHE_B200_GENERIC_NTT");
    w.solinas_ntt = set("FHE_B200_SOLINAS_NTT");
    w.no_solinas = set("FHE_B200_NO_SOLINAS");
    w.no_tensor_fusion = set("FHE_B200_NO_TENSOR_FUSION");
    w.classic_scaler = is("FHE_B200_SCALER", "classic");
    w.ksmac = is("FHE_B200_KSMAC", "tma")       ? Switches::KSMAC_TMA
              : is("FHE_B200_KSMAC", "classic") ? Switches::KSMAC_CLASSIC
                                                : Switches::KSMAC_FUSED;
    w.tma_cols = number("FHE_B200_TMA_COLS", 3);
    w.scale_unroll = number("FHE_B200_SCALE_UNROLL", 2);
    w.ks_stages = clamped("FHE_B200_KS_STAGES", 2, 2, 4);
    return w;
  }();
  return s;
}

EncodeTiledFn tensor_map_encoder() {
  static EncodeTiledFn fn = [] {
    void* p = nullptr;
    cudaDriverEntryPointQueryResult q = cudaDriverEntryPointSymbolNotFound;
    if (cudaGetDriverEntryPoint("cuTensorMapEncodeTiled", &p, cudaEnableDefault, &q) != cudaSuccess ||
        q != cudaDriverEntryPointSuccess)
      p = nullptr;
    cudaGetLastError();
    return (EncodeTiledFn)p;
  }();
  return fn;
}

bool box_map(CUtensorMap* m, const u64* base, u64 rows, u32 logn, u32 box_cols, u32 box_rows) {
  const cuuint64_t gdim[2] = {(cuuint64_t)1 << logn, rows};
  const cuuint64_t gstride[1] = {(cuuint64_t)8 << logn};
  const cuuint32_t box[2] = {box_cols, box_rows};
  const cuuint32_t es[2] = {1, 1};
  return tensor_map_encoder() &&
         tensor_map_encoder()(m, CU_TENSOR_MAP_DATA_TYPE_UINT64, 2, (void*)base, gdim, gstride, box, es,
                              CU_TENSOR_MAP_INTERLEAVE_NONE, CU_TENSOR_MAP_SWIZZLE_NONE,
                              CU_TENSOR_MAP_L2_PROMOTION_L2_128B, CU_TENSOR_MAP_FLOAT_OOB_FILL_NONE) == CUDA_SUCCESS;
}

int sm_count() {
  static std::mutex mu;
  static std::map<int, int> cache;
  int dev = 0;
  FHE_CUDA(cudaGetDevice(&dev));
  std::lock_guard<std::mutex> g(mu);
  auto it = cache.find(dev);
  if (it != cache.end()) return it->second;
  int n = 0;
  FHE_CUDA(cudaDeviceGetAttribute(&n, cudaDevAttrMultiProcessorCount, dev));
  return cache[dev] = n;
}

void ensure_dynamic_smem(const void* kernel, size_t bytes) {
  if (bytes <= 48 * 1024) return;
  static std::mutex mu;
  static std::map<std::pair<int, const void*>, size_t> granted;
  int dev = 0;
  FHE_CUDA(cudaGetDevice(&dev));
  std::lock_guard<std::mutex> g(mu);
  size_t& have = granted[std::make_pair(dev, kernel)];
  if (have >= bytes) return;
  FHE_CUDA(cudaFuncSetAttribute(kernel, cudaFuncAttributeMaxDynamicSharedMemorySize, (int)bytes));
  have = bytes;
}

namespace {

constexpr int kTileLog = 12;

template <int LOGP, int LOGB, bool INV>
void run_rows(const NttArgs& a, cudaStream_t st) {
  constexpr u32 T = 1u << (LOGP + LOGB);
  const u32 tiles = (1u << a.logn1) >> LOGB;
  const u32 threads = T / 8 >= 256 ? 256 : (T / 8 < 32 ? 32 : T / 8);
  const size_t smem = (T + (T >> 5) + 1) * sizeof(u64);
  ntt_rows_kernel<LOGP, LOGB, INV><<<a.n_rows * tiles, threads, smem, st>>>(a);
  g_launches++;
}
template <int LOGP, int LOGB, bool INV>
void run_cols(const NttArgs& a, cudaStream_t st) {
  constexpr u32 T = 1u << (LOGP + LOGB);
  const u32 tiles = (1u << (a.logn - LOGP)) >> LOGB;
  const size_t smem = (T + (T >> 5) + 1) * sizeof(u64);
  ntt_cols_kernel<LOGP, LOGB, INV><<<a.n_rows * tiles, 256, smem, st>>>(a);
  g_launches++;
}

template <int LOGP, bool COLS, bool INV, int TLOG>
void run_fast(const NttArgs& a, cudaStream_t st) {
  constexpr size_t smem = 2 * FastTile<LOGP, COLS, INV, TLOG>::TW * sizeof(u64);
  ensure_dynamic_smem((const void*)ntt_fast_kernel<LOGP, COLS, INV, TLOG>, smem);
  constexpr int LOGB = TLOG - LOGP;
  const u32 tiles = COLS ? ((1u << (a.logn - LOGP)) >> LOGB) : ((1u << a.logn1) >> LOGB);
  ntt_fast_kernel<LOGP, COLS, INV, TLOG><<<a.n_rows * tiles, 1 << (TLOG - 3), smem, st>>>(a);
  g_launches++;
}
template <bool INV>
void run_fast_cols_for(const NttArgs& a, cudaStream_t st) {
  switch (a.logn1) {
    case 7: run_fast<7, true, INV, 11>(a, st); break;
    case 8: run_fast<8, true, INV, 11>(a, st); break;
    case 9: run_fast<9, true, INV, 11>(a, st); break;
    case 10: run_fast<10, true, INV, 12>(a, st); break;
    default: break;
  }
}

template <bool INV>
void run_single(const NttArgs& a, cudaStream_t st) {
  switch (a.logn) {
    case 3: run_rows<3, 0, INV>(a, st); break;
    case 4: run_rows<4, 0, INV>(a, st); break;
    case 5: run_rows<5, 0, INV>(a, st); break;
    case 6: run_rows<6, 0, INV>(a, st); break;
    case 7: run_rows<7, 0, INV>(a, st); break;
    case 8: run_rows<8, 0, INV>(a, st); break;
    case 9: run_rows<9, 0, INV>(a, st); break;
    case 10: run_rows<10, 0, INV>(a, st); break;
    case 11: run_rows<11, 0, INV>(a, st); break;
    case 12: run_rows<12, 0, INV>(a, st); break;
    default: break;
  }
}
template <bool INV>
void run_cols_for(const NttArgs& a, cudaStream_t st) {
  switch (a.logn1) {
    case 7: run_cols<7, kTileLog - 7, INV>(a, st); break;
    case 8: run_cols<8, kTileLog - 8, INV>(a, st); break;
    case 9: run_cols<9, kTileLog - 9, INV>(a, st); break;
    case 10: run_cols<10, kTileLog - 10, INV>(a, st); break;
    default: break;
  }
}

struct TmaFail {};
CUtensorMap rows_map(const u64* base, u64 rows, u32 logn, u32 box_rows) {
  CUtensorMap m;
  const cuuint64_t gdim[2] = {16, (rows << logn) >> 4};
  const cuuint64_t gstride[1] = {128};
  const cuuint32_t box[2] = {16, box_rows};
  const cuuint32_t es[2] = {1, 1};
  if (gdim[1] >= (1ull << 31) ||
      tensor_map_encoder()(&m, CU_TENSOR_MAP_DATA_TYPE_UINT64, 2, (void*)base, gdim, gstride, box, es,
                           CU_TENSOR_MAP_INTERLEAVE_NONE, CU_TENSOR_MAP_SWIZZLE_128B, CU_TENSOR_MAP_L2_PROMOTION_L2_128B,
                           CU_TENSOR_MAP_FLOAT_OOB_FILL_NONE) != CUDA_SUCCESS)
    throw TmaFail{};
  return m;
}
CUtensorMap cols_map(const u64* base, u64 rows, u32 logn, u32 box_rows) {
  CUtensorMap m;
  const cuuint64_t gdim[3] = {64, (cuuint64_t)1 << (logn - 6), rows};
  const cuuint64_t gstride[2] = {512, (cuuint64_t)8 << logn};
  const cuuint32_t box[3] = {16, box_rows, 1};
  const cuuint32_t es[3] = {1, 1, 1};
  if (tensor_map_encoder()(&m, CU_TENSOR_MAP_DATA_TYPE_UINT64, 3, (void*)base, gdim, gstride, box, es,
                           CU_TENSOR_MAP_INTERLEAVE_NONE, CU_TENSOR_MAP_SWIZZLE_NONE, CU_TENSOR_MAP_L2_PROMOTION_L2_128B,
                           CU_TENSOR_MAP_FLOAT_OOB_FILL_NONE) != CUDA_SUCCESS)
    throw TmaFail{};
  return m;
}

constexpr int kRowsRlog = 4;

template <bool INV, int STAGES, int MINB>
void run_tma_rows_one(const u64* in, u64 in_rows, u64* out, u64 out_rows, NttTmaArgs A, cudaStream_t st) {
  using Cfg = RowsCfg<kRowsRlog, STAGES>;
  const CUtensorMap mi = rows_map(in, in_rows, A.logn, 4 * Cfg::R), mo = rows_map(out, out_rows, A.logn, 4 * Cfg::R);
  A.tiles_per_row = (1u << (A.logn - 6)) / Cfg::R;
  A.tiles_total = A.lpp * A.tiles_per_row * A.n_polys;
  const u32 grid = std::min<u64>(A.tiles_total, (u64)sm_count() * MINB);
  if (!INV && A.lazy_out) {
    auto k = ntt_tma_rows_kernel<INV, kRowsRlog, STAGES, MINB, !INV>;
    ensure_dynamic_smem((const void*)k, Cfg::SMEM);
    k<<<grid, Cfg::NT + 32, Cfg::SMEM, st>>>(mi, mo, A);
  } else {
    auto k = ntt_tma_rows_kernel<INV, kRowsRlog, STAGES, MINB, false>;
    ensure_dynamic_smem((const void*)k, Cfg::SMEM);
    k<<<grid, Cfg::NT + 32, Cfg::SMEM, st>>>(mi, mo, A);
  }
  g_launches++;
}
template <bool INV, int STAGES, int MINB>
void run_tma_rows_pair(const u64* in, u64 in_rows, u64* out, u64 out_rows, NttTmaArgs A, cudaStream_t st) {
  using Cfg = RowsCfg<kRowsRlog, STAGES>;
  constexpr size_t smem = (size_t)STAGES * 2 * Cfg::TILE_BYTES + Cfg::TW_PAIRS * 16 + 2 * STAGES * 8 + 1024;
  const CUtensorMap mi = rows_map(in, in_rows, A.logn, 4 * Cfg::R), mo = rows_map(out, out_rows, A.logn, 4 * Cfg::R);
  A.tiles_per_row = (1u << (A.logn - 6)) / Cfg::R;
  A.n_polys /= 2;
  A.tiles_total = A.lpp * A.tiles_per_row * A.n_polys;
  const u32 grid = std::min<u64>(A.tiles_total, (u64)sm_count() * MINB);
  if (!INV && A.lazy_out) {
    auto k = ntt_tma_rows_pair_kernel<INV, kRowsRlog, STAGES, MINB, !INV>;
    ensure_dynamic_smem((const void*)k, smem);
    k<<<grid, Cfg::NT + 32, smem, st>>>(mi, mo, A);
  } else {
    auto k = ntt_tma_rows_pair_kernel<INV, kRowsRlog, STAGES, MINB, false>;
    ensure_dynamic_smem((const void*)k, smem);
    k<<<grid, Cfg::NT + 32, smem, st>>>(mi, mo, A);
  }
  g_launches++;
}

template <bool INV>
void run_tma_rows(const u64* in, u64 in_rows, u64* out, u64 out_rows, const NttTmaArgs& A, cudaStream_t st) {
  if (A.n_polys % 2 == 0 && !(A.digit_adjacent && A.n_dig % 2))
    run_tma_rows_pair<INV, 3, 3>(in, in_rows, out, out_rows, A, st);
  else
    run_tma_rows_one<INV, 4, 4>(in, in_rows, out, out_rows, A, st);
}
template <int LOGP, bool INV, int STAGES, int MINB>
void run_tma_cols(const u64* in, u64 in_rows, u64* out, u64 out_rows, NttTmaArgs A, cudaStream_t st) {
  using Cfg = ColsCfg<LOGP, STAGES>;
  const CUtensorMap mi = cols_map(in, in_rows, A.logn, Cfg::BOX_ROWS), mo = cols_map(out, out_rows, A.logn, Cfg::BOX_ROWS);
  A.tiles_per_row = 4;
  A.tiles_total = A.lpp * 4 * A.n_polys;
  const u32 grid = std::min<u64>(A.tiles_total, (u64)sm_count() * MINB);
  if (!INV && A.reduce_on_load) {
    auto k = ntt_tma_cols_kernel<LOGP, INV, STAGES, MINB, !INV>;
    ensure_dynamic_smem((const void*)k, Cfg::SMEM);
    k<<<grid, Cfg::NT + 32, Cfg::SMEM, st>>>(mi, mo, A);
  } else {
    auto k = ntt_tma_cols_kernel<LOGP, INV, STAGES, MINB, false>;
    ensure_dynamic_smem((const void*)k, Cfg::SMEM);
    k<<<grid, Cfg::NT + 32, Cfg::SMEM, st>>>(mi, mo, A);
  }
  g_launches++;
}
template <bool INV>
void run_tma_cols_for(const u64* in, u64 in_rows, u64* out, u64 out_rows, const NttTmaArgs& A, cudaStream_t st) {
  const bool d2 = switches().tma_cols == 2;
  switch (A.logn - 6) {
    case 7:
      if (d2) run_tma_cols<7, INV, 2, 6>(in, in_rows, out, out_rows, A, st);
      else run_tma_cols<7, INV, 3, 4>(in, in_rows, out, out_rows, A, st);
      break;
    case 8:
      if (d2) run_tma_cols<8, INV, 2, 3>(in, in_rows, out, out_rows, A, st);
      else run_tma_cols<8, INV, 3, 2>(in, in_rows, out, out_rows, A, st);
      break;
    case 9:
      if (d2) run_tma_cols<9, INV, 2, 1>(in, in_rows, out, out_rows, A, st);
      else run_tma_cols<9, INV, 3, 1>(in, in_rows, out, out_rows, A, st);
      break;
    default: throw TmaFail{};
  }
}

bool launch_ntt_tma(const u64* in, u64* out, u32 n_rows, const RowIds& ids, const LimbDev* limbs, u32 logn, bool inverse,
                    u32 in_div, bool reduce_on_load, cudaStream_t st, bool lazy_out, bool digit_adjacent, u32 n_dig) {
  const u32 lpp = ids.limbs_per_poly;
  if (logn < 13 || logn > 15 || !tensor_map_encoder()) return false;
  if (n_rows % lpp != 0 || (in_div != 1 && in_div != lpp)) return false;
  if (digit_adjacent && ((n_rows / lpp) % n_dig != 0 || n_dig == 0)) return false;
  if ((reinterpret_cast<uintptr_t>(in) | reinterpret_cast<uintptr_t>(out)) & 127) return false;
  NttTmaArgs A;
  std::memset(&A, 0, sizeof(A));
  A.limbs = limbs;
  A.n_polys = n_rows / lpp;
  A.lpp = lpp;
  A.logn = logn;
  A.digit_adjacent = digit_adjacent ? 1 : 0;
  A.n_dig = digit_adjacent ? n_dig : 1;
  for (int i = 0; i < kMaxPos; i++) A.ids[i] = ids.ids[i];
  const u64 in_rows = in_div == 1 ? n_rows : n_rows / lpp;
  try {
    NttTmaArgs first = A, second = A;
    first.in_bcast = first.limb_inner = in_div != 1;
    if (!inverse) {
      first.reduce_on_load = reduce_on_load;
      second.lazy_out = lazy_out;
      run_tma_cols_for<false>(in, in_rows, out, n_rows, first, st);
      run_tma_rows<false>(out, n_rows, out, n_rows, second, st);
    } else {
      if (reduce_on_load || in_div != 1) return false;
      run_tma_rows<true>(in, in_rows, out, n_rows, first, st);
      run_tma_cols_for<true>(out, n_rows, out, n_rows, second, st);
    }
  } catch (const TmaFail&) {
    return false;
  }
  return true;
}

template <int STAGES, int MINB>
void run_tensor_rows(const CUtensorMap& ma, const CUtensorMap& mb, const CUtensorMap& mxa, const CUtensorMap& mxb,
                     const CUtensorMap& mo, TensorRowsArgs A, cudaStream_t st) {
  using Cfg = TensorRowsCfg<kRowsRlog, STAGES>;
  auto k = ntt_tma_tensor_rows_kernel<kRowsRlog, STAGES, MINB>;
  ensure_dynamic_smem((const void*)k, Cfg::SMEM);
  const u32 grid = std::min<u64>(A.items_total, (u64)sm_count() * MINB);
  k<<<grid, Cfg::NT + 32, Cfg::SMEM, st>>>(ma, mb, mxa, mxb, mo, A);
  g_launches++;
}

bool launch_tensor_intt_tma(const u64* a, const u64* b, const u64* xa, const u64* xb, u64* T, u32 cts, u32 L, u32 K,
                            const RowIds& mul_ids, const LimbDev* limbs, u32 logn, cudaStream_t st) {
  constexpr u32 R = 1u << kRowsRlog;
  const u32 E = K - L;
  try {
    const CUtensorMap ma = rows_map(a, (u64)cts * 2 * L, logn, 4 * R), mb = rows_map(b, (u64)cts * 2 * L, logn, 4 * R);
    const CUtensorMap mxa = rows_map(xa, (u64)cts * 2 * E, logn, 4 * R), mxb = rows_map(xb, (u64)cts * 2 * E, logn, 4 * R);
    const CUtensorMap mo = rows_map(T, (u64)cts * 3 * K, logn, 4 * R);
    TensorRowsArgs A;
    std::memset(&A, 0, sizeof(A));
    A.limbs = limbs; A.cts = cts; A.L = L; A.K = K; A.logn = logn;
    A.tiles_per_row = (1u << (logn - 6)) / R;
    A.items_total = K * A.tiles_per_row * cts;
    for (int i = 0; i < kMaxPos; i++) A.ids[i] = mul_ids.ids[i];
    run_tensor_rows<2, 2>(ma, mb, mxa, mxb, mo, A, st);
    NttTmaArgs C;
    std::memset(&C, 0, sizeof(C));
    C.limbs = limbs; C.n_polys = cts * 3; C.lpp = K; C.logn = logn; C.n_dig = 1;
    for (int i = 0; i < kMaxPos; i++) C.ids[i] = mul_ids.ids[i];
    run_tma_cols_for<true>(T, (u64)cts * 3 * K, T, (u64)cts * 3 * K, C, st);
  } catch (const TmaFail&) {
    return false;
  }
  return true;
}

template <int STAGES>
void run_ks_rows_mac(const CUtensorMap& mi, const CUtensorMap& m0, const CUtensorMap& m1, const KsRowsArgs& A,
                     cudaStream_t st) {
  using Cfg = KsRowsCfg<STAGES>;
  auto k = ks_rows_mac_tma_kernel<STAGES, 3>;
  const size_t smem = Cfg::smem(A.n_dig);
  ensure_dynamic_smem((const void*)k, smem);
  int per_sm = 0;
  FHE_CUDA(cudaOccupancyMaxActiveBlocksPerMultiprocessor(&per_sm, (const void*)k, Cfg::NT + 32, smem));
  const u32 grid = (u32)std::min<u64>(A.items_total, (u64)sm_count() * std::max(per_sm, 1));
  k<<<grid, Cfg::NT + 32, smem, st>>>(mi, m0, m1, A);
  g_launches++;
}

}

bool ntt_uses_tma(u32 n_rows, const RowIds& ids, u32 logn, u32 in_div, const u64* in, const u64* out) {
  const Switches& sw = switches();
  const u32 lpp = ids.limbs_per_poly;
  if (!sw.tma_allowed() || logn < 13 || logn > 15 || !tensor_map_encoder()) return false;
  if (n_rows % lpp != 0 || (in_div != 1 && in_div != lpp)) return false;
  if ((reinterpret_cast<uintptr_t>(in) | reinterpret_cast<uintptr_t>(out)) & 127) return false;
  return sw.ntt == Switches::NTT_TMA || n_rows / lpp >= 8;
}

bool launch_tensor_inverse_ntt(const u64* a, const u64* b, const u64* xa, const u64* xb, u64* T, u32 cts, u32 L, u32 K,
                               const RowIds& mul_ids, const LimbDev* limbs, u32 logn, cudaStream_t st) {
  if (switches().no_tensor_fusion || K <= L || !ntt_uses_tma(cts * 3 * K, mul_ids, logn, 1, T, T)) return false;
  if ((reinterpret_cast<uintptr_t>(a) | reinterpret_cast<uintptr_t>(b) | reinterpret_cast<uintptr_t>(xa) |
       reinterpret_cast<uintptr_t>(xb)) & 127)
    return false;
  return launch_tensor_intt_tma(a, b, xa, xb, T, cts, L, K, mul_ids, limbs, logn, st);
}

bool launch_key_switch_tma(const u64* c2, u64* inter, const u64* k0, const u64* k1, const u64* base0,
                           const u64* base1, u64* out0, u64* out1, u32 cts, u32 n_dig, u32 Lk, u32 out_ct_rows,
                           const RowIds& ids, const LimbDev* limbs, u32 logn, bool reduce, cudaStream_t st) {
  const int stages = switches().ks_stages >= 3 ? 3 : 2;
  using Cfg = KsRowsCfg<2>;
  const u32 n_rows = cts * n_dig * Lk;
  if (logn < 13 || logn > 15 || !tensor_map_encoder() || ids.limbs_per_poly != Lk || n_dig == 0 || n_dig > 256)
    return false;
  if ((reinterpret_cast<uintptr_t>(c2) | reinterpret_cast<uintptr_t>(inter) | reinterpret_cast<uintptr_t>(k0) |
       reinterpret_cast<uintptr_t>(k1)) & 127)
    return false;
  if ((stages == 3 ? KsRowsCfg<3>::smem(n_dig) : Cfg::smem(n_dig)) > 227 * 1024) return false;
  CUtensorMap m0, m1;
  if (!box_map(&m0, k0, (u64)Lk * n_dig, logn, Cfg::TC, n_dig) || !box_map(&m1, k1, (u64)Lk * n_dig, logn, Cfg::TC, n_dig))
    return false;
  try {
    const CUtensorMap mi = rows_map(inter, n_rows, logn, 4 * Cfg::R);
    NttTmaArgs C;
    std::memset(&C, 0, sizeof(C));
    C.limbs = limbs;
    C.n_polys = cts * n_dig;
    C.lpp = Lk;
    C.in_bcast = C.limb_inner = 1;
    C.digit_adjacent = 1;
    C.n_dig = n_dig;
    C.reduce_on_load = reduce ? 1 : 0;
    C.logn = logn;
    for (int i = 0; i < kMaxPos; i++) C.ids[i] = ids.ids[i];
    run_tma_cols_for<false>(c2, (u64)cts * n_dig, inter, n_rows, C, st);
    KsRowsArgs A;
    std::memset(&A, 0, sizeof(A));
    A.limbs = limbs;
    A.base0 = base0; A.base1 = base1; A.out0 = out0; A.out1 = out1;
    A.cts = cts; A.n_dig = n_dig; A.Lk = Lk; A.out_ct_rows = out_ct_rows; A.logn = logn;
    A.tiles_per_row = (1u << logn) / Cfg::TC;
    A.items_total = Lk * A.tiles_per_row * cts;
    for (int i = 0; i < kMaxPos; i++) A.ids[i] = ids.ids[i];
    if (stages == 3) run_ks_rows_mac<3>(mi, m0, m1, A, st);
    else run_ks_rows_mac<2>(mi, m0, m1, A, st);
  } catch (const TmaFail&) {
    return false;
  }
  return true;
}

void launch_ntt(const u64* in, u64* out, u32 n_rows, const RowIds& ids, const LimbDev* limbs, u32 logn,
                bool inverse, u32 in_div, bool reduce_on_load, cudaStream_t st, bool lazy_out, bool digit_adjacent,
                u32 n_dig) {
  if (n_rows == 0) return;
  NttArgs a;
  a.in = in;
  a.out = out;
  a.limbs = limbs;
  a.n_rows = n_rows;
  a.limbs_per_poly = ids.limbs_per_poly;
  a.in_div = in_div;
  a.reduce_on_load = reduce_on_load ? 1 : 0;
  a.lazy_out = (lazy_out && !inverse) ? 1 : 0;
  a.logn = logn;
  for (int i = 0; i < kMaxPos; i++) a.ids[i] = ids.ids[i];
  if (logn <= 12) {
    a.logn1 = 0;
    if (inverse) run_single<true>(a, st); else run_single<false>(a, st);
    return;
  }
  a.logn1 = logn - 6;
  NttArgs second = a;
  second.in = out;
  second.in_div = 1;
  second.reduce_on_load = 0;
  if (ntt_uses_tma(n_rows, ids, logn, in_div, in, out) &&
      launch_ntt_tma(in, out, n_rows, ids, limbs, logn, inverse, in_div, reduce_on_load, st, lazy_out, digit_adjacent,
                     n_dig))
    return;
  if (digit_adjacent) throw CudaFail{cudaErrorNotSupported, "digit-adjacent NTT output needs the TMA kernels"};
  if (switches().generic_tiles()) {
    if (!inverse) {
      run_cols_for<false>(a, st);
      run_rows<6, 6, false>(second, st);
    } else {
      run_rows<6, 6, true>(a, st);
      run_cols_for<true>(second, st);
    }
    return;
  }
  if (!inverse) {
    run_fast_cols_for<false>(a, st);
    run_fast<6, false, false, 10>(second, st);
  } else {
    run_fast<6, false, true, 10>(a, st);
    run_fast_cols_for<true>(second, st);
  }
}

}
```

### fhe_rs_b200/csrc/ntt_tma.cuh

```cuda
#pragma once
#include <cuda.h>

#include "ntt.cuh"

namespace fhe_b200 {

struct NttTmaArgs {
  const LimbDev* limbs;
  u32 n_polys;
  u32 lpp;
  u32 in_bcast;
  u32 digit_adjacent;
  u32 n_dig;
  u32 reduce_on_load;
  u32 lazy_out;
  u32 logn;
  u32 tiles_per_row;
  u32 tiles_total;
  u32 limb_inner;
  unsigned short ids[kMaxPos];
};

namespace tma {

__device__ __forceinline__ u32 smem_u32(const void* p) { return (u32)__cvta_generic_to_shared(p); }
__device__ __forceinline__ void mbar_init(u32 bar, u32 count) {
  asm volatile("mbarrier.init.shared::cta.b64 [%0], %1;" ::"r"(bar), "r"(count) : "memory");
}
__device__ __forceinline__ void mbar_expect_tx(u32 bar, u32 bytes) {
  asm volatile("mbarrier.arrive.expect_tx.shared::cta.b64 _, [%0], %1;" ::"r"(bar), "r"(bytes) : "memory");
}
__device__ __forceinline__ void mbar_arrive(u32 bar) {
  asm volatile("mbarrier.arrive.shared::cta.b64 _, [%0];" ::"r"(bar) : "memory");
}
__device__ __forceinline__ u32 mbar_try_wait(u32 bar, u32 parity, u32 ns) {
  u32 ok;
  asm volatile(
      "{\n\t"
      ".reg .pred p;\n\t"
      "mbarrier.try_wait.parity.shared::cta.b64 p, [%1], %2, %3;\n\t"
      "selp.u32 %0, 1, 0, p;\n\t"
      "}"
      : "=r"(ok)
      : "r"(bar), "r"(parity), "r"(ns)
      : "memory");
  return ok;
}
__device__ __forceinline__ void mbar_wait(u32 bar, u32 parity) {
  u32 tries = 0;
  while (!mbar_try_wait(bar, parity, 100000u)) {
    if (++tries > 4000000u) __trap();
  }
}
__device__ __forceinline__ void fence_proxy_async() { asm volatile("fence.proxy.async.shared::cta;" ::: "memory"); }
__device__ __forceinline__ void bulk_commit() { asm volatile("cp.async.bulk.commit_group;" ::: "memory"); }
template <int N>
__device__ __forceinline__ void bulk_wait_read() {
  asm volatile("cp.async.bulk.wait_group.read %0;" ::"n"(N) : "memory");
}
__device__ __forceinline__ void bulk_wait_all() { asm volatile("cp.async.bulk.wait_group 0;" ::: "memory"); }
template <int NT>
__device__ __forceinline__ void consumer_sync() {
  asm volatile("bar.sync 1, %0;" ::"n"(NT) : "memory");
}

__device__ __forceinline__ void load_2d(u32 dst, const CUtensorMap* tm, u32 c0, u32 c1, u32 bar) {
  asm volatile(
      "cp.async.bulk.tensor.2d.shared::cluster.global.tile.mbarrier::complete_tx::bytes [%0], [%1, {%2, %3}], [%4];"
      ::"r"(dst), "l"(tm), "r"(c0), "r"(c1), "r"(bar)
      : "memory");
}
__device__ __forceinline__ void store_2d(const CUtensorMap* tm, u32 c0, u32 c1, u32 src) {
  asm volatile("cp.async.bulk.tensor.2d.global.shared::cta.tile.bulk_group [%0, {%1, %2}], [%3];" ::"l"(tm), "r"(c0),
               "r"(c1), "r"(src)
               : "memory");
}
__device__ __forceinline__ void load_3d(u32 dst, const CUtensorMap* tm, u32 c0, u32 c1, u32 c2, u32 bar) {
  asm volatile(
      "cp.async.bulk.tensor.3d.shared::cluster.global.tile.mbarrier::complete_tx::bytes [%0], [%1, {%2, %3, %4}], "
      "[%5];" ::"r"(dst),
      "l"(tm), "r"(c0), "r"(c1), "r"(c2), "r"(bar)
      : "memory");
}
__device__ __forceinline__ void store_3d(const CUtensorMap* tm, u32 c0, u32 c1, u32 c2, u32 src) {
  asm volatile("cp.async.bulk.tensor.3d.global.shared::cta.tile.bulk_group [%0, {%1, %2, %3}], [%4];" ::"l"(tm),
               "r"(c0), "r"(c1), "r"(c2), "r"(src)
               : "memory");
}
__device__ __forceinline__ void prefetch_map(const CUtensorMap* tm) {
  asm volatile("prefetch.tensormap [%0];" ::"l"(tm) : "memory");
}

__device__ __forceinline__ u64 lds64(u32 a) {
  u64 v;
  asm volatile("ld.shared.u64 %0, [%1];" : "=l"(v) : "r"(a));
  return v;
}
__device__ __forceinline__ void sts64(u32 a, u64 v) { asm volatile("st.shared.u64 [%0], %1;" ::"r"(a), "l"(v) : "memory"); }
__device__ __forceinline__ ulonglong2 lds128(u32 a) {
  ulonglong2 v;
  asm volatile("ld.shared.v2.u64 {%0, %1}, [%2];" : "=l"(v.x), "=l"(v.y) : "r"(a));
  return v;
}
__device__ __forceinline__ void sts128(u32 a, u64 x, u64 y) {
  asm volatile("st.shared.v2.u64 [%0], {%1, %2};" ::"r"(a), "l"(x), "l"(y) : "memory");
}

template <int NS>
__device__ __forceinline__ void fwd_stages(u64* v, const ulonglong2* tw, u64 p, u64 p2) {
  constexpr int R = 1 << NS;
#pragma unroll
  for (int u = 0; u < NS; u++) {
    const int half = R >> (u + 1);
#pragma unroll
    for (int m = 0; m < (1 << u); m++) {
      const ulonglong2 w = tw[(1 << u) - 1 + m];
#pragma unroll
      for (int e = 0; e < half; e++) {
        const int jj = m * 2 * half + e;
        bf_fwd<false>(v[jj], v[jj + half], w.x, w.y, p, p2, 0);
      }
    }
  }
}
template <class TW>
__device__ __forceinline__ void fwd_stages3_staged(u64* v, u64 p, u64 p2, const TW& tw) {
#pragma unroll
  for (int u = 0; u < 3; u++) {
    const int half = 8 >> (u + 1);
    ulonglong2 w[4];
#pragma unroll
    for (int m = 0; m < (1 << u); m++) w[m] = tw(u, m);
#pragma unroll
    for (int m = 0; m < (1 << u); m++) {
#pragma unroll
      for (int e = 0; e < half; e++) {
        const int jj = m * 2 * half + e;
        bf_fwd<false>(v[jj], v[jj + half], w[m].x, w[m].y, p, p2, 0);
      }
    }
  }
}
struct LastStage {
  u64 ninv, ninv_s, zn, zn_s;
};
template <int NS, typename LS>
__device__ __forceinline__ void inv_stages(u64* v, const ulonglong2* tz, u64 p, u64 p2, bool last, const LS& L) {
  constexpr int R = 1 << NS;
#pragma unroll
  for (int u = NS - 1; u >= 0; u--) {
    const int half = R >> (u + 1);
    if (u == 0 && last) {
#pragma unroll
      for (int e = 0; e < half; e++) {
        const u64 a = v[e], b2 = v[e + half];
        v[e] = csub(mul_shoup_lazy(a + b2, L.ninv, L.ninv_s, p), p);
        v[e + half] = csub(mul_shoup_lazy(p2 + a - b2, L.zn, L.zn_s, p), p);
      }
    } else {
#pragma unroll
      for (int m = 0; m < (1 << u); m++) {
        const ulonglong2 z = tz[(1 << u) - 1 + m];
#pragma unroll
        for (int e = 0; e < half; e++) {
          const int jj = m * 2 * half + e;
          bf_inv<false>(v[jj], v[jj + half], z.x, z.y, p, p2, 0);
        }
      }
    }
  }
}

struct TileWalk {
  u32 jt, p, n_polys;
  __device__ __forceinline__ void init(u32 idx, u32 np) {
    n_polys = np;
    jt = idx / np;
    p = idx - jt * np;
  }
  __device__ __forceinline__ bool next() {
    if (++p == n_polys) {
      p = 0;
      jt++;
      return true;
    }
    return false;
  }
};

__device__ __forceinline__ u32 out_row_of(const NttTmaArgs& A, u32 p, u32 j) {
  if (A.digit_adjacent) {
    const u32 ct = p / A.n_dig, d = p - ct * A.n_dig;
    return (ct * A.lpp + j) * A.n_dig + d;
  }
  return p * A.lpp + j;
}

}

template <int RLOG, int STAGES>
struct RowsCfg {
  static constexpr u32 R = 1u << RLOG;
  static constexpr u32 NT = 8 * R;
  static constexpr u32 TILE_BYTES = 512 * R;
  static constexpr u32 TW_PAIRS = 63 * R;
  static constexpr u32 SMEM = STAGES * TILE_BYTES + TW_PAIRS * 16 + 2 * STAGES * 8 + 1024;
};

template <bool INV, int RLOG, int STAGES, int MINB, bool LAZY>
__global__ void __launch_bounds__(RowsCfg<RLOG, STAGES>::NT + 32, MINB)
    ntt_tma_rows_kernel(const __grid_constant__ CUtensorMap tm_in, const __grid_constant__ CUtensorMap tm_out,
                        const NttTmaArgs A) {
  using namespace tma;
  using Cfg = RowsCfg<RLOG, STAGES>;
  constexpr u32 R = Cfg::R, NT = Cfg::NT, TILE_BYTES = Cfg::TILE_BYTES;
  extern __shared__ unsigned char smem_raw[];
  const u32 base = (smem_u32(smem_raw) + 1023u) & ~1023u;
  const u32 tw_base = base + STAGES * TILE_BYTES;
  const u32 bar_full = tw_base + Cfg::TW_PAIRS * 16;
  const u32 bar_done = bar_full + STAGES * 8;

  if (threadIdx.x == 0) {
#pragma unroll
    for (int s = 0; s < STAGES; s++) {
      mbar_init(bar_full + 8 * s, 1);
      mbar_init(bar_done + 8 * s, NT);
    }
    asm volatile("fence.mbarrier_init.release.cluster;" ::: "memory");
  }
  __syncthreads();

  const u32 lo = (u32)(((u64)A.tiles_total * blockIdx.x) / gridDim.x);
  const u32 hi = (u32)(((u64)A.tiles_total * (blockIdx.x + 1)) / gridDim.x);
  const u32 n = hi - lo;
  const u32 box_rows_per_row = (1u << A.logn) >> 4;

  if (threadIdx.x >= NT) {
    if (threadIdx.x != NT) return;
    prefetch_map(&tm_in);
    prefetch_map(&tm_out);
    TileWalk wl, ws;
    wl.init(lo, A.n_polys);
    ws.init(lo, A.n_polys);
    auto coord = [&](const TileWalk& w, bool input) -> u32 {
      const u32 j = w.jt / A.tiles_per_row, tau = w.jt - j * A.tiles_per_row;
      const u32 row = (input && A.in_bcast) ? w.p : out_row_of(A, w.p, j);
      return row * box_rows_per_row + tau * (4 * R);
    };
    u32 loaded = 0;
    auto load_next = [&]() {
      const u32 s = loaded % STAGES;
      mbar_expect_tx(bar_full + 8 * s, TILE_BYTES);
      load_2d(base + s * TILE_BYTES, &tm_in, 0, coord(wl, true), bar_full + 8 * s);
      wl.next();
      loaded++;
    };
    while (loaded < n && loaded < (u32)STAGES) load_next();
    for (u32 i = 0; i < n; i++) {
      const u32 s = i % STAGES;
      mbar_wait(bar_done + 8 * s, (i / STAGES) & 1);
      store_2d(&tm_out, 0, coord(ws, false), base + s * TILE_BYTES);
      bulk_commit();
      ws.next();
      if (loaded < n) {
        bulk_wait_read<0>();
        load_next();
      }
    }
    bulk_wait_all();
    return;
  }

  const u32 tid = threadIdx.x;
  const u32 x = tid & 7, b = tid >> 3;
  u32 off0[8];
#pragma unroll
  for (int e = 0; e < 8; e++) {
    const u32 i = 64 * b + x + 8 * e;
    off0[e] = ((i >> 4) << 7) | ((((i >> 1) & 7) ^ ((i >> 4) & 7)) << 4) | ((i & 1) << 3);
  }
  u32 off1[4];
#pragma unroll
  for (int k = 0; k < 4; k++) {
    const u32 i = 64 * b + 8 * x + 2 * k;
    off1[k] = ((i >> 4) << 7) | ((((i >> 1) & 7) ^ ((i >> 4) & 7)) << 4);
  }
  const u32 tw0 = tw_base + 16 * (b);
  const u32 tw1 = tw_base + 16 * (R * 1 + (b << 1));
  const u32 tw2 = tw_base + 16 * (R * 3 + (b << 2));
  const u32 tw3 = tw_base + 16 * (R * 7 + tid);
  const u32 tw4 = tw_base + 16 * (R * 15 + tid);
  const u32 tw5 = tw_base + 16 * (R * 31 + tid);

  TileWalk w;
  w.init(lo, A.n_polys);
  bool fresh = true;
  u64 p = 0, p2 = 0;
  const u32 logn1 = A.logn - 6;
  for (u32 i = 0; i < n; i++) {
    if (fresh) {
      const u32 j = w.jt / A.tiles_per_row, tau = w.jt - j * A.tiles_per_row;
      const LimbDev& L = A.limbs[A.ids[j]];
      p = L.p;
      p2 = L.p2;
      const ulonglong2* tab = INV ? L.zi : L.om;
      const u32 row0 = tau * R;
      if (i) consumer_sync<NT>();
#pragma unroll
      for (int tl = 0; tl < 6; tl++) {
        const u32 s = logn1 + tl;
        const u32 g0 = (INV ? ((1u << A.logn) - (2u << s)) : (1u << s)) + (row0 << tl);
        for (u32 k = tid; k < (R << tl); k += NT) {
          const ulonglong2 v = __ldg(tab + g0 + k);
          const u32 dst = tl < 3 ? k : (k & ((1u << (tl >= 3 ? tl - 3 : 0)) - 1)) * (8 * R) + (k >> (tl >= 3 ? tl - 3 : 0));
          sts128(tw_base + 16 * (R * ((1u << tl) - 1) + dst), v.x, v.y);
        }
      }
      consumer_sync<NT>();
    }
    const u32 s = i % STAGES;
    const u32 buf = base + s * TILE_BYTES;
    mbar_wait(bar_full + 8 * s, (i / STAGES) & 1);
    u64 v[8];
    ulonglong2 tw[7];
    if (!INV) {
#pragma unroll
      for (int e = 0; e < 8; e++) v[e] = lds64(buf + off0[e]);
      tw[0] = lds128(tw0);
      tw[1] = lds128(tw1);
      tw[2] = lds128(tw1 + 16);
#pragma unroll
      for (int m = 0; m < 4; m++) tw[3 + m] = lds128(tw2 + 16 * m);
      fwd_stages<3>(v, tw, p, p2);
#pragma unroll
      for (int e = 0; e < 8; e++) sts64(buf + off0[e], v[e]);
      consumer_sync<NT>();
#pragma unroll
      for (int k = 0; k < 4; k++) {
        const ulonglong2 t = lds128(buf + off1[k]);
        v[2 * k] = t.x;
        v[2 * k + 1] = t.y;
      }
      tw[0] = lds128(tw3);
      tw[1] = lds128(tw4);
      tw[2] = lds128(tw4 + 16 * 8 * R);
#pragma unroll
      for (int m = 0; m < 4; m++) tw[3 + m] = lds128(tw5 + 16 * 8 * R * m);
      fwd_stages<3>(v, tw, p, p2);
      if (!LAZY) {
#pragma unroll
        for (int e = 0; e < 8; e++) v[e] = fwd_final<false>(v[e], p, p2, 0);
      }
#pragma unroll
      for (int k = 0; k < 4; k++) sts128(buf + off1[k], v[2 * k], v[2 * k + 1]);
    } else {
#pragma unroll
      for (int k = 0; k < 4; k++) {
        const ulonglong2 t = lds128(buf + off1[k]);
        v[2 * k] = t.x;
        v[2 * k + 1] = t.y;
      }
      tw[0] = lds128(tw3);
      tw[1] = lds128(tw4);
      tw[2] = lds128(tw4 + 16 * 8 * R);
#pragma unroll
      for (int m = 0; m < 4; m++) tw[3 + m] = lds128(tw5 + 16 * 8 * R * m);
      inv_stages<3>(v, tw, p, p2, false, A.limbs[0]);
#pragma unroll
      for (int k = 0; k < 4; k++) sts128(buf + off1[k], v[2 * k], v[2 * k + 1]);
      consumer_sync<NT>();
#pragma unroll
      for (int e = 0; e < 8; e++) v[e] = lds64(buf + off0[e]);
      tw[0] = lds128(tw0);
      tw[1] = lds128(tw1);
      tw[2] = lds128(tw1 + 16);
#pragma unroll
      for (int m = 0; m < 4; m++) tw[3 + m] = lds128(tw2 + 16 * m);
      inv_stages<3>(v, tw, p, p2, false, A.limbs[0]);
#pragma unroll
      for (int e = 0; e < 8; e++) sts64(buf + off0[e], v[e]);
    }
    fence_proxy_async();
    mbar_arrive(bar_done + 8 * s);
    fresh = w.next();
  }
}

template <bool INV, int RLOG, int STAGES, int MINB, bool LAZY>
__global__ void __launch_bounds__(RowsCfg<RLOG, STAGES>::NT + 32, MINB)
    ntt_tma_rows_pair_kernel(const __grid_constant__ CUtensorMap tm_in, const __grid_constant__ CUtensorMap tm_out,
                        const NttTmaArgs A) {
  using namespace tma;
  using Cfg = RowsCfg<RLOG, STAGES>;
  constexpr u32 R = Cfg::R, NT = Cfg::NT, TILE_BYTES = Cfg::TILE_BYTES, STAGE_BYTES = 2 * TILE_BYTES;
  extern __shared__ unsigned char smem_raw[];
  const u32 base = (smem_u32(smem_raw) + 1023u) & ~1023u;
  const u32 tw_base = base + STAGES * STAGE_BYTES;
  const u32 bar_full = tw_base + Cfg::TW_PAIRS * 16;
  const u32 bar_done = bar_full + STAGES * 8;

  if (threadIdx.x == 0) {
#pragma unroll
    for (int s = 0; s < STAGES; s++) {
      mbar_init(bar_full + 8 * s, 1);
      mbar_init(bar_done + 8 * s, NT);
    }
    asm volatile("fence.mbarrier_init.release.cluster;" ::: "memory");
  }
  __syncthreads();

  const u32 lo = (u32)(((u64)A.tiles_total * blockIdx.x) / gridDim.x);
  const u32 hi = (u32)(((u64)A.tiles_total * (blockIdx.x + 1)) / gridDim.x);
  const u32 n = hi - lo;
  const u32 box_rows_per_row = (1u << A.logn) >> 4;

  if (threadIdx.x >= NT) {
    if (threadIdx.x != NT) return;
    prefetch_map(&tm_in);
    prefetch_map(&tm_out);
    TileWalk wl, ws;
    wl.init(lo, A.n_polys);
    ws.init(lo, A.n_polys);
    auto coord = [&](const TileWalk& w, bool input, u32 h) -> u32 {
      const u32 j = w.jt / A.tiles_per_row, tau = w.jt - j * A.tiles_per_row;
      const u32 poly = 2 * w.p + h;
      const u32 row = (input && A.in_bcast) ? poly : out_row_of(A, poly, j);
      return row * box_rows_per_row + tau * (4 * R);
    };
    u32 loaded = 0;
    auto load_next = [&]() {
      const u32 s = loaded % STAGES;
      mbar_expect_tx(bar_full + 8 * s, STAGE_BYTES);
      load_2d(base + s * STAGE_BYTES, &tm_in, 0, coord(wl, true, 0), bar_full + 8 * s);
      load_2d(base + s * STAGE_BYTES + TILE_BYTES, &tm_in, 0, coord(wl, true, 1), bar_full + 8 * s);
      wl.next();
      loaded++;
    };
    while (loaded < n && loaded < (u32)STAGES) load_next();
    for (u32 i = 0; i < n; i++) {
      const u32 s = i % STAGES;
      mbar_wait(bar_done + 8 * s, (i / STAGES) & 1);
      store_2d(&tm_out, 0, coord(ws, false, 0), base + s * STAGE_BYTES);
      store_2d(&tm_out, 0, coord(ws, false, 1), base + s * STAGE_BYTES + TILE_BYTES);
      bulk_commit();
      ws.next();
      if (loaded < n) {
        bulk_wait_read<0>();
        load_next();
      }
    }
    bulk_wait_all();
    return;
  }

  const u32 tid = threadIdx.x;
  const u32 x = tid & 7, b = tid >> 3;
  u32 off0[8];
#pragma unroll
  for (int e = 0; e < 8; e++) {
    const u32 i = 64 * b + x + 8 * e;
    off0[e] = ((i >> 4) << 7) | ((((i >> 1) & 7) ^ ((i >> 4) & 7)) << 4) | ((i & 1) << 3);
  }
  u32 off1[4];
#pragma unroll
  for (int k = 0; k < 4; k++) {
    const u32 i = 64 * b + 8 * x + 2 * k;
    off1[k] = ((i >> 4) << 7) | ((((i >> 1) & 7) ^ ((i >> 4) & 7)) << 4);
  }
  const u32 tw0 = tw_base + 16 * (b);
  const u32 tw1 = tw_base + 16 * (R * 1 + (b << 1));
  const u32 tw2 = tw_base + 16 * (R * 3 + (b << 2));
  const u32 tw3 = tw_base + 16 * (R * 7 + tid);
  const u32 tw4 = tw_base + 16 * (R * 15 + tid);
  const u32 tw5 = tw_base + 16 * (R * 31 + tid);

  TileWalk w;
  w.init(lo, A.n_polys);
  bool fresh = true;
  u64 p = 0, p2 = 0;
  const u32 logn1 = A.logn - 6;
  for (u32 i = 0; i < n; i++) {
    if (fresh) {
      const u32 j = w.jt / A.tiles_per_row, tau = w.jt - j * A.tiles_per_row;
      const LimbDev& L = A.limbs[A.ids[j]];
      p = L.p;
      p2 = L.p2;
      const ulonglong2* tab = INV ? L.zi : L.om;
      const u32 row0 = tau * R;
      if (i) consumer_sync<NT>();
#pragma unroll
      for (int tl = 0; tl < 6; tl++) {
        const u32 s = logn1 + tl;
        const u32 g0 = (INV ? ((1u << A.logn) - (2u << s)) : (1u << s)) + (row0 << tl);
        for (u32 k = tid; k < (R << tl); k += NT) {
          const ulonglong2 v = __ldg(tab + g0 + k);
          const u32 dst = tl < 3 ? k : (k & ((1u << (tl >= 3 ? tl - 3 : 0)) - 1)) * (8 * R) + (k >> (tl >= 3 ? tl - 3 : 0));
          sts128(tw_base + 16 * (R * ((1u << tl) - 1) + dst), v.x, v.y);
        }
      }
      consumer_sync<NT>();
    }
    const u32 s = i % STAGES;
    const u32 buf0 = base + s * STAGE_BYTES;
    mbar_wait(bar_full + 8 * s, (i / STAGES) & 1);
    u64 v[8];
    ulonglong2 tw[7];
    if (!INV) {
      tw[0] = lds128(tw0);
      tw[1] = lds128(tw1);
      tw[2] = lds128(tw1 + 16);
#pragma unroll
      for (int m = 0; m < 4; m++) tw[3 + m] = lds128(tw2 + 16 * m);
    } else {
      tw[0] = lds128(tw3);
      tw[1] = lds128(tw4);
      tw[2] = lds128(tw4 + 16 * 8 * R);
#pragma unroll
      for (int m = 0; m < 4; m++) tw[3 + m] = lds128(tw5 + 16 * 8 * R * m);
    }
#pragma unroll
    for (u32 h = 0; h < 2; h++) {
      const u32 buf = buf0 + h * TILE_BYTES;
      if (!INV) {
#pragma unroll
        for (int e = 0; e < 8; e++) v[e] = lds64(buf + off0[e]);
        fwd_stages<3>(v, tw, p, p2);
#pragma unroll
        for (int e = 0; e < 8; e++) sts64(buf + off0[e], v[e]);
      } else {
#pragma unroll
        for (int k = 0; k < 4; k++) {
          const ulonglong2 t = lds128(buf + off1[k]);
          v[2 * k] = t.x;
          v[2 * k + 1] = t.y;
        }
        inv_stages<3>(v, tw, p, p2, false, A.limbs[0]);
#pragma unroll
        for (int k = 0; k < 4; k++) sts128(buf + off1[k], v[2 * k], v[2 * k + 1]);
      }
    }
    consumer_sync<NT>();
    if (!INV) {
      tw[0] = lds128(tw3);
      tw[1] = lds128(tw4);
      tw[2] = lds128(tw4 + 16 * 8 * R);
#pragma unroll
      for (int m = 0; m < 4; m++) tw[3 + m] = lds128(tw5 + 16 * 8 * R * m);
    } else {
      tw[0] = lds128(tw0);
      tw[1] = lds128(tw1);
      tw[2] = lds128(tw1 + 16);
#pragma unroll
      for (int m = 0; m < 4; m++) tw[3 + m] = lds128(tw2 + 16 * m);
    }
#pragma unroll
    for (u32 h = 0; h < 2; h++) {
      const u32 buf = buf0 + h * TILE_BYTES;
      if (!INV) {
#pragma unroll
        for (int k = 0; k < 4; k++) {
          const ulonglong2 t = lds128(buf + off1[k]);
          v[2 * k] = t.x;
          v[2 * k + 1] = t.y;
        }
        fwd_stages<3>(v, tw, p, p2);
        if (!LAZY) {
#pragma unroll
          for (int e = 0; e < 8; e++) v[e] = fwd_final<false>(v[e], p, p2, 0);
        }
#pragma unroll
        for (int k = 0; k < 4; k++) sts128(buf + off1[k], v[2 * k], v[2 * k + 1]);
      } else {
#pragma unroll
        for (int e = 0; e < 8; e++) v[e] = lds64(buf + off0[e]);
        inv_stages<3>(v, tw, p, p2, false, A.limbs[0]);
#pragma unroll
        for (int e = 0; e < 8; e++) sts64(buf + off0[e], v[e]);
      }
    }
    fence_proxy_async();
    mbar_arrive(bar_done + 8 * s);
    fresh = w.next();
  }
}

struct TensorRowsArgs {
  const LimbDev* limbs;
  u32 cts, L, K, logn;
  u32 tiles_per_row;
  u32 items_total;
  unsigned short ids[kMaxPos];
};

template <int RLOG, int STAGES>
struct TensorRowsCfg {
  static constexpr u32 R = 1u << RLOG;
  static constexpr u32 NT = 8 * R;
  static constexpr u32 TILE_BYTES = 512 * R;
  static constexpr u32 STAGE_BYTES = 4 * TILE_BYTES;
  static constexpr u32 TW_PAIRS = 63 * R;
  static constexpr u32 SMEM = STAGES * STAGE_BYTES + TW_PAIRS * 16 + 2 * STAGES * 8 + 1024;
};

template <int RLOG, int STAGES, int MINB>
__global__ void __launch_bounds__(TensorRowsCfg<RLOG, STAGES>::NT + 32, MINB)
    ntt_tma_tensor_rows_kernel(const __grid_constant__ CUtensorMap tm_a, const __grid_constant__ CUtensorMap tm_b,
                               const __grid_constant__ CUtensorMap tm_xa, const __grid_constant__ CUtensorMap tm_xb,
                               const __grid_constant__ CUtensorMap tm_out, const TensorRowsArgs A) {
  using namespace tma;
  using Cfg = TensorRowsCfg<RLOG, STAGES>;
  constexpr u32 R = Cfg::R, NT = Cfg::NT, TILE_BYTES = Cfg::TILE_BYTES, STAGE_BYTES = Cfg::STAGE_BYTES;
  extern __shared__ unsigned char smem_raw[];
  const u32 base = (smem_u32(smem_raw) + 1023u) & ~1023u;
  const u32 tw_base = base + STAGES * STAGE_BYTES;
  const u32 bar_full = tw_base + Cfg::TW_PAIRS * 16;
  const u32 bar_done = bar_full + STAGES * 8;
  if (threadIdx.x == 0) {
#pragma unroll
    for (int s = 0; s < STAGES; s++) {
      mbar_init(bar_full + 8 * s, 1);
      mbar_init(bar_done + 8 * s, NT);
    }
    asm volatile("fence.mbarrier_init.release.cluster;" ::: "memory");
  }
  __syncthreads();

  const u32 lo = (u32)(((u64)A.items_total * blockIdx.x) / gridDim.x);
  const u32 hi = (u32)(((u64)A.items_total * (blockIdx.x + 1)) / gridDim.x);
  const u32 n = hi - lo;
  const u32 box_rows_per_row = (1u << A.logn) >> 4;
  const u32 E = A.K - A.L;

  if (threadIdx.x >= NT) {
    if (threadIdx.x != NT) return;
    prefetch_map(&tm_a);
    prefetch_map(&tm_b);
    prefetch_map(&tm_xa);
    prefetch_map(&tm_xb);
    prefetch_map(&tm_out);
    TileWalk wl, ws;
    wl.init(lo, A.cts);
    ws.init(lo, A.cts);
    u32 loaded = 0;
    auto load_next = [&]() {
      const u32 s = loaded % STAGES;
      const u32 j = wl.jt / A.tiles_per_row, tau = wl.jt - j * A.tiles_per_row;
      const u32 ct = wl.p;
      const bool pre = j < A.L;
      const u32 rows = pre ? A.L : E, jj = pre ? j : j - A.L;
      const CUtensorMap* ma = pre ? &tm_a : &tm_xa;
      const CUtensorMap* mb = pre ? &tm_b : &tm_xb;
      const u32 r0 = ((ct * 2) * rows + jj) * box_rows_per_row + tau * (4 * R);
      const u32 r1 = ((ct * 2 + 1) * rows + jj) * box_rows_per_row + tau * (4 * R);
      const u32 dst = base + s * STAGE_BYTES, bar = bar_full + 8 * s;
      mbar_expect_tx(bar, STAGE_BYTES);
      load_2d(dst, ma, 0, r0, bar);
      load_2d(dst + TILE_BYTES, ma, 0, r1, bar);
      load_2d(dst + 2 * TILE_BYTES, mb, 0, r0, bar);
      load_2d(dst + 3 * TILE_BYTES, mb, 0, r1, bar);
      wl.next();
      loaded++;
    };
    while (loaded < n && loaded < (u32)STAGES) load_next();
    for (u32 i = 0; i < n; i++) {
      const u32 s = i % STAGES;
      mbar_wait(bar_done + 8 * s, (i / STAGES) & 1);
      const u32 j = ws.jt / A.tiles_per_row, tau = ws.jt - j * A.tiles_per_row;
      const u32 ct = ws.p;
      const u32 src = base + s * STAGE_BYTES;
      store_2d(&tm_out, 0, ((ct * 3 + 0) * A.K + j) * box_rows_per_row + tau * (4 * R), src);
      store_2d(&tm_out, 0, ((ct * 3 + 1) * A.K + j) * box_rows_per_row + tau * (4 * R), src + 2 * TILE_BYTES);
      store_2d(&tm_out, 0, ((ct * 3 + 2) * A.K + j) * box_rows_per_row + tau * (4 * R), src + TILE_BYTES);
      bulk_commit();
      ws.next();
      if (loaded < n) {
        bulk_wait_read<0>();
        load_next();
      }
    }
    bulk_wait_all();
    return;
  }

  const u32 tid = threadIdx.x;
  const u32 x = tid & 7, b = tid >> 3;
  u32 off0[8];
#pragma unroll
  for (int e = 0; e < 8; e++) {
    const u32 i = 64 * b + x + 8 * e;
    off0[e] = ((i >> 4) << 7) | ((((i >> 1) & 7) ^ ((i >> 4) & 7)) << 4) | ((i & 1) << 3);
  }
  u32 off1[4];
#pragma unroll
  for (int k = 0; k < 4; k++) {
    const u32 i = 64 * b + 8 * x + 2 * k;
    off1[k] = ((i >> 4) << 7) | ((((i >> 1) & 7) ^ ((i >> 4) & 7)) << 4);
  }
  const u32 tw0 = tw_base + 16 * (b);
  const u32 tw1 = tw_base + 16 * (R * 1 + (b << 1));
  const u32 tw2 = tw_base + 16 * (R * 3 + (b << 2));
  const u32 tw3 = tw_base + 16 * (R * 7 + tid);
  const u32 tw4 = tw_base + 16 * (R * 15 + tid);
  const u32 tw5 = tw_base + 16 * (R * 31 + tid);

  TileWalk w;
  w.init(lo, A.cts);
  bool fresh = true;
  LimbDev M = A.limbs[0];
  const u32 logn1 = A.logn - 6;
  for (u32 i = 0; i < n; i++) {
    if (fresh) {
      const u32 j = w.jt / A.tiles_per_row, tau = w.jt - j * A.tiles_per_row;
      M = A.limbs[A.ids[j]];
      const ulonglong2* tab = M.zi;
      const u32 row0 = tau * R;
      if (i) consumer_sync<NT>();
#pragma unroll
      for (int tl = 0; tl < 6; tl++) {
        const u32 s = logn1 + tl;
        const u32 g0 = ((1u << A.logn) - (2u << s)) + (row0 << tl);
        for (u32 k = tid; k < (R << tl); k += NT) {
          const ulonglong2 v = __ldg(tab + g0 + k);
          const u32 dst = tl < 3 ? k : (k & ((1u << (tl >= 3 ? tl - 3 : 0)) - 1)) * (8 * R) + (k >> (tl >= 3 ? tl - 3 : 0));
          sts128(tw_base + 16 * (R * ((1u << tl) - 1) + dst), v.x, v.y);
        }
      }
      consumer_sync<NT>();
    }
    const u64 p = M.p, p2 = M.p2;
    const u32 s = i % STAGES;
    const u32 buf = base + s * STAGE_BYTES;
    mbar_wait(bar_full + 8 * s, (i / STAGES) & 1);
#pragma unroll 1
    for (u32 k = 0; k < 4; k++) {
      const u32 i = 64 * b + 8 * x + 2 * k;
      const u32 o = buf + (((i >> 4) << 7) | ((((i >> 1) & 7) ^ ((i >> 4) & 7)) << 4));
      const ulonglong2 a0 = lds128(o), a1 = lds128(o + TILE_BYTES);
      const ulonglong2 b0 = lds128(o + 2 * TILE_BYTES), b1 = lds128(o + 3 * TILE_BYTES);
      const u64 c0x = mulmod_limb_lazy(a0.x, b0.x, M), c0y = mulmod_limb_lazy(a0.y, b0.y, M);
      const u64 c2x = mulmod_limb_lazy(a1.x, b1.x, M), c2y = mulmod_limb_lazy(a1.y, b1.y, M);
      Acc192 sx, sy;
      sx.clear();
      sy.clear();
      sx.mac(a0.x, b1.x);
      sx.mac(a1.x, b0.x);
      sy.mac(a0.y, b1.y);
      sy.mac(a1.y, b0.y);
      const u64 c1x = sx.reduce_lazy(M), c1y = sy.reduce_lazy(M);
      sts128(o, c0x, c0y);
      sts128(o + 2 * TILE_BYTES, c1x, c1y);
      sts128(o + TILE_BYTES, c2x, c2y);
    }
    u64 v[8];
    ulonglong2 tw[7];
    tw[0] = lds128(tw3);
    tw[1] = lds128(tw4);
    tw[2] = lds128(tw4 + 16 * 8 * R);
#pragma unroll
    for (int m = 0; m < 4; m++) tw[3 + m] = lds128(tw5 + 16 * 8 * R * m);
#pragma unroll 1
    for (u32 t = 0; t < 3; t++) {
      const u32 tb = buf + t * TILE_BYTES;
#pragma unroll
      for (int k = 0; k < 4; k++) {
        const ulonglong2 q = lds128(tb + off1[k]);
        v[2 * k] = q.x;
        v[2 * k + 1] = q.y;
      }
      inv_stages<3>(v, tw, p, p2, false, M);
#pragma unroll
      for (int k = 0; k < 4; k++) sts128(tb + off1[k], v[2 * k], v[2 * k + 1]);
    }
    consumer_sync<NT>();
    tw[0] = lds128(tw0);
    tw[1] = lds128(tw1);
    tw[2] = lds128(tw1 + 16);
#pragma unroll
    for (int m = 0; m < 4; m++) tw[3 + m] = lds128(tw2 + 16 * m);
#pragma unroll 1
    for (u32 t = 0; t < 3; t++) {
      const u32 tb = buf + t * TILE_BYTES;
#pragma unroll
      for (int e = 0; e < 8; e++) v[e] = lds64(tb + off0[e]);
      inv_stages<3>(v, tw, p, p2, false, M);
#pragma unroll
      for (int e = 0; e < 8; e++) sts64(tb + off0[e], v[e]);
    }
    fence_proxy_async();
    mbar_arrive(bar_done + 8 * s);
    fresh = w.next();
  }
}

struct KsRowsArgs {
  const LimbDev* limbs;
  const u64 *base0, *base1;
  u64 *out0, *out1;
  u32 cts, n_dig, Lk, out_ct_rows, logn;
  u32 tiles_per_row;
  u32 items_total;
  unsigned short ids[kMaxPos];
};

template <int STAGES>
struct KsRowsCfg {
  static constexpr u32 R = 2;
  static constexpr u32 TC = 64 * R;
  static constexpr u32 TILE_BYTES = 512 * R;
  static constexpr u32 GROUPS = 16;
  static constexpr u32 NT = GROUPS * 8 * R;
  static constexpr u32 TW_PAIRS = 63 * R;
  static constexpr size_t smem(u32 nd) {
    return (size_t)STAGES * nd * TILE_BYTES + 2 * (size_t)nd * TC * 8 + TW_PAIRS * 16 + 2 * STAGES * 8 + 8 + 1024;
  }
};

template <int STAGES, int MINB>
__global__ void __launch_bounds__(KsRowsCfg<STAGES>::NT + 32, MINB)
    ks_rows_mac_tma_kernel(const __grid_constant__ CUtensorMap tm_in, const __grid_constant__ CUtensorMap tm_k0,
                           const __grid_constant__ CUtensorMap tm_k1, const KsRowsArgs A) {
  using namespace tma;
  using Cfg = KsRowsCfg<STAGES>;
  constexpr u32 R = Cfg::R, TC = Cfg::TC, NT = Cfg::NT, TILE_BYTES = Cfg::TILE_BYTES, GROUPS = Cfg::GROUPS;
  extern __shared__ unsigned char smem_raw[];
  const u32 nd = A.n_dig;
  const u32 base = (smem_u32(smem_raw) + 1023u) & ~1023u;
  const u32 stage_bytes = nd * TILE_BYTES;
  const u32 k0_base = base + STAGES * stage_bytes;
  const u32 k1_base = k0_base + nd * TC * 8;
  const u32 tw_base = k1_base + nd * TC * 8;
  const u32 bar_full = tw_base + Cfg::TW_PAIRS * 16;
  const u32 bar_done = bar_full + STAGES * 8;
  const u32 bar_key = bar_done + STAGES * 8;

  if (threadIdx.x == 0) {
#pragma unroll
    for (int s = 0; s < STAGES; s++) {
      mbar_init(bar_full + 8 * s, 1);
      mbar_init(bar_done + 8 * s, NT);
    }
    mbar_init(bar_key, 1);
    asm volatile("fence.mbarrier_init.release.cluster;" ::: "memory");
  }
  __syncthreads();

  const u32 lo = (u32)(((u64)A.items_total * blockIdx.x) / gridDim.x);
  const u32 hi = (u32)(((u64)A.items_total * (blockIdx.x + 1)) / gridDim.x);
  const u32 n = hi - lo;
  const u32 box_rows_per_row = (1u << A.logn) >> 4;

  if (threadIdx.x >= NT) {
    if (threadIdx.x != NT) return;
    prefetch_map(&tm_in);
    TileWalk wl;
    wl.init(lo, A.cts);
    for (u32 i = 0; i < n; i++) {
      const u32 s = i % STAGES;
      if (i >= (u32)STAGES) mbar_wait(bar_done + 8 * s, (i / STAGES - 1) & 1);
      const u32 j = wl.jt / A.tiles_per_row, tau = wl.jt - j * A.tiles_per_row;
      const u32 row0 = (wl.p * A.Lk + j) * nd;
      mbar_expect_tx(bar_full + 8 * s, stage_bytes);
      for (u32 d = 0; d < nd; d++)
        load_2d(base + s * stage_bytes + d * TILE_BYTES, &tm_in, 0, (row0 + d) * box_rows_per_row + tau * (4 * R),
                bar_full + 8 * s);
      wl.next();
    }
    return;
  }

  const u32 tid = threadIdx.x;
  const u32 g = tid >> 4, lt = tid & 15;
  const u32 hmask = 0xffffu << (tid & 16);
  const u32 x = lt & 7, b = lt >> 3;
  const u32 off0 = ((4 * b) << 7) | ((((x >> 1) & 7) ^ (4 * b)) << 4) | ((x & 1) << 3);
  const u32 off1 = ((4 * b + (x >> 1)) << 7) | (((4 * (x & 1)) ^ (4 * b + (x >> 1))) << 4);
  auto x0 = [](int e) -> u32 { return ((u32)(e >> 1) << 7) | ((u32)((e >> 1) ^ (4 * (e & 1))) << 4); };
  const u32 tw0 = tw_base + 16 * (b);
  const u32 tw1 = tw_base + 16 * (R * 1 + (b << 1));
  const u32 tw2 = tw_base + 16 * (R * 3 + (b << 2));
  const u32 tw3 = tw_base + 16 * (R * 7 + lt);
  const u32 tw4 = tw_base + 16 * (R * 15 + lt);
  const u32 tw5 = tw_base + 16 * (R * 31 + lt);
  const u32 c = tid & (TC - 1), o = tid / TC;
  const u32 offc = ((c >> 4) << 7) | ((((c >> 1) & 7) ^ ((c >> 4) & 7)) << 4) | ((c & 1) << 3);
  const u32 key_c = (o ? k1_base : k0_base) + 8 * c;
  const u64* bsrc = o ? A.base1 : A.base0;
  u64* dst = o ? A.out1 : A.out0;

  TileWalk w;
  w.init(lo, A.cts);
  bool fresh = true;
  u32 key_phase = 0;
  const LimbDev* Mp = A.limbs;
  u64 p = 0, p2 = 0;
  const u32 logn1 = A.logn - 6;
  for (u32 i = 0; i < n; i++) {
    const u32 j = w.jt / A.tiles_per_row, tau = w.jt - j * A.tiles_per_row;
    const bool new_keys = fresh;
    if (fresh) {
      Mp = A.limbs + A.ids[j];
      p = Mp->p;
      p2 = Mp->p2;
      if (i) consumer_sync<NT>();
      if (tid == 0) {
        mbar_expect_tx(bar_key, 2 * nd * TC * 8);
        load_2d(k0_base, &tm_k0, tau * TC, j * nd, bar_key);
        load_2d(k1_base, &tm_k1, tau * TC, j * nd, bar_key);
      }
      const u32 row0 = tau * R;
#pragma unroll
      for (int tl = 0; tl < 6; tl++) {
        const u32 s = logn1 + tl;
        const u32 g0 = (1u << s) + (row0 << tl);
        if (tid < (R << tl)) {
          const ulonglong2 v = __ldg(Mp->om + g0 + tid);
          const u32 k = tid;
          const u32 dst_pair = tl < 3 ? k : (k & ((1u << (tl >= 3 ? tl - 3 : 0)) - 1)) * (8 * R) + (k >> (tl >= 3 ? tl - 3 : 0));
          sts128(tw_base + 16 * (R * ((1u << tl) - 1) + dst_pair), v.x, v.y);
        }
      }
      consumer_sync<NT>();
    }
    const size_t oi = (((size_t)w.p * A.out_ct_rows + j) << A.logn) + tau * TC + c;
    const u64 bv = bsrc ? bsrc[oi] : 0;
    const u32 s = i % STAGES;
    const u32 ring = base + s * stage_bytes;
    mbar_wait(bar_full + 8 * s, (i / STAGES) & 1);
    for (u32 d = g; d < nd; d += GROUPS) {
      const u32 a0 = ring + d * TILE_BYTES + off0, a1 = ring + d * TILE_BYTES + off1;
      u64 v[8];
#pragma unroll
      for (int e = 0; e < 8; e++) v[e] = lds64(a0 ^ x0(e));
      fwd_stages3_staged(v, p, p2, [&](int u, int m) {
        return lds128(u == 0 ? tw0 : u == 1 ? tw1 + 16 * m : tw2 + 16 * m);
      });
#pragma unroll
      for (int e = 0; e < 8; e++) sts64(a0 ^ x0(e), v[e]);
      __syncwarp(hmask);
#pragma unroll
      for (int k = 0; k < 4; k++) {
        const ulonglong2 t = lds128(a1 ^ (k << 4));
        v[2 * k] = t.x;
        v[2 * k + 1] = t.y;
      }
      fwd_stages3_staged(v, p, p2, [&](int u, int m) {
        return lds128(u == 0 ? tw3 : u == 1 ? tw4 + 16 * 8 * R * m : tw5 + 16 * 8 * R * m);
      });
#pragma unroll
      for (int k = 0; k < 4; k++) sts128(a1 ^ (k << 4), v[2 * k], v[2 * k + 1]);
    }
    if (new_keys) {
      mbar_wait(bar_key, key_phase);
      key_phase ^= 1;
    }
    consumer_sync<NT>();
    Acc192 acc;
    acc.clear();
#pragma unroll 2
    for (u32 d = 0; d < nd; d++) acc.mac(lds64(ring + d * TILE_BYTES + offc), lds64(key_c + d * TC * 8));
    acc.add64(bv);
    dst[oi] = acc.reduce(*Mp);
    mbar_arrive(bar_done + 8 * s);
    fresh = w.next();
  }
}

template <int LOGP, int STAGES>
struct ColsCfg {
  static constexpr u32 P = 1u << LOGP;
  static constexpr u32 NT = P;
  static constexpr u32 TILE_BYTES = P * 128;
  static constexpr u32 BOX_ROWS = P < 256 ? P : 256;
  static constexpr u32 BOXES = P / BOX_ROWS;
  static constexpr u32 SMEM = STAGES * TILE_BYTES + P * 16 + 2 * STAGES * 8 + 1024;
  static constexpr int NR = (LOGP + 2) / 3;
  static constexpr int REM = LOGP - 3 * (NR - 1);
};

template <int LOGP, bool INV, int NS, int T, bool REDUCE, bool ROLL = false>
__device__ __forceinline__ void cols_round(u32 buf, u32 tw_base, u64 p, u64 p2, const tma::LastStage& L, u64 bhi, u64 blo) {
  using namespace tma;
  constexpr int t = T;
  constexpr u32 NT = 1u << LOGP;
  constexpr int R = 1 << NS;
  constexpr u32 UNITS = (1u << (LOGP + 4 - NS)) / NT;
  constexpr int logstride = LOGP - t - NS;
  constexpr u32 stride_bytes = 128u << logstride;
  constexpr bool HI = (LOGP - 4) >= logstride;
  constexpr u32 D_AHI = HI ? (1u << (LOGP - 4 - logstride)) : 0;
  constexpr u32 D_ADDR = (HI ? (D_AHI << (LOGP - t)) : (1u << (LOGP - 4))) * 128;
  const u32 bcol = threadIdx.x & 15, rest = threadIdx.x >> 4;
  const u32 a_lo = rest & ((1u << logstride) - 1);
  u32 a_hi = rest >> logstride;
  u32 addr = buf + ((a_hi << (LOGP - t)) + a_lo) * 128 + bcol * 8;
#pragma unroll(ROLL ? 1 : 8)
  for (u32 q = 0; q < UNITS; q++) {
    u64 v[R];
#pragma unroll
    for (int e = 0; e < R; e++) {
      v[e] = lds64(addr + e * stride_bytes);
      if (REDUCE) v[e] = barrett64(v[e], p, bhi, blo);
    }
    ulonglong2 tw[R - 1];
#pragma unroll
    for (int u = 0; u < NS; u++) {
      const int tl = t + u;
      if (INV && tl == 0) continue;
      const u32 idx = (INV ? ((1u << LOGP) - (2u << tl)) : (1u << tl)) + (a_hi << u);
#pragma unroll
      for (int m = 0; m < (1 << u); m++) tw[(1 << u) - 1 + m] = lds128(tw_base + 16 * (idx + m));
    }
    if (!INV) fwd_stages<NS>(v, tw, p, p2);
    else inv_stages<NS>(v, tw, p, p2, t == 0, L);
#pragma unroll
    for (int e = 0; e < R; e++) sts64(addr + e * stride_bytes, v[e]);
    addr += D_ADDR;
    a_hi += D_AHI;
  }
}

__device__ __forceinline__ void cols_tile(const NttTmaArgs& A, u32 idx, u32& j, u32& tau, u32& p) {
  if (A.limb_inner) {
    const u32 r = idx / A.lpp;
    j = idx - r * A.lpp;
    tau = r / A.n_polys;
    p = r - tau * A.n_polys;
  } else {
    const u32 jt = idx / A.n_polys;
    p = idx - jt * A.n_polys;
    j = jt / A.tiles_per_row;
    tau = jt - j * A.tiles_per_row;
  }
}

template <int LOGP, bool INV, int STAGES, int MINB, bool REDUCE, bool ROLL = false>
__global__ void __launch_bounds__(ColsCfg<LOGP, STAGES>::NT + 32, MINB)
    ntt_tma_cols_kernel(const __grid_constant__ CUtensorMap tm_in, const __grid_constant__ CUtensorMap tm_out,
                        const NttTmaArgs A) {
  using namespace tma;
  using Cfg = ColsCfg<LOGP, STAGES>;
  constexpr u32 NT = Cfg::NT, TILE_BYTES = Cfg::TILE_BYTES, P = Cfg::P;
  constexpr int NR = Cfg::NR, REM = Cfg::REM;
  extern __shared__ unsigned char smem_raw[];
  const u32 base = (smem_u32(smem_raw) + 1023u) & ~1023u;
  const u32 tw_base = base + STAGES * TILE_BYTES;
  const u32 bar_full = tw_base + P * 16;
  const u32 bar_done = bar_full + STAGES * 8;

  if (threadIdx.x == 0) {
#pragma unroll
    for (int s = 0; s < STAGES; s++) {
      mbar_init(bar_full + 8 * s, 1);
      mbar_init(bar_done + 8 * s, NT);
    }
    asm volatile("fence.mbarrier_init.release.cluster;" ::: "memory");
  }
  __syncthreads();

  const u32 lo = (u32)(((u64)A.tiles_total * blockIdx.x) / gridDim.x);
  const u32 hi = (u32)(((u64)A.tiles_total * (blockIdx.x + 1)) / gridDim.x);
  const u32 n = hi - lo;

  if (threadIdx.x >= NT) {
    if (threadIdx.x != NT) return;
    prefetch_map(&tm_in);
    prefetch_map(&tm_out);
    u32 loaded = 0;
    auto load_next = [&]() {
      const u32 s = loaded % STAGES;
      u32 j, tau, pp;
      cols_tile(A, lo + loaded, j, tau, pp);
      const u32 row = A.in_bcast ? pp : out_row_of(A, pp, j);
      mbar_expect_tx(bar_full + 8 * s, TILE_BYTES);
#pragma unroll
      for (u32 h = 0; h < Cfg::BOXES; h++)
        load_3d(base + s * TILE_BYTES + h * Cfg::BOX_ROWS * 128, &tm_in, tau * 16, h * Cfg::BOX_ROWS, row,
                bar_full + 8 * s);
      loaded++;
    };
    while (loaded < n && loaded < (u32)STAGES) load_next();
    for (u32 i = 0; i < n; i++) {
      const u32 s = i % STAGES;
      mbar_wait(bar_done + 8 * s, (i / STAGES) & 1);
      u32 j, tau, pp;
      cols_tile(A, lo + i, j, tau, pp);
      const u32 row = out_row_of(A, pp, j);
#pragma unroll
      for (u32 h = 0; h < Cfg::BOXES; h++)
        store_3d(&tm_out, tau * 16, h * Cfg::BOX_ROWS, row, base + s * TILE_BYTES + h * Cfg::BOX_ROWS * 128);
      bulk_commit();
      if (loaded < n) {
        bulk_wait_read<0>();
        load_next();
      }
    }
    bulk_wait_all();
    return;
  }

  const u32 tid = threadIdx.x;
  u32 cur_j = 0xffffffffu;
  const LimbDev* Lp = A.limbs;
  u64 p = 0, p2 = 0, bhi = 0, blo = 0;
  LastStage ls = {0, 0, 0, 0};
  for (u32 i = 0; i < n; i++) {
    u32 j, tau_unused, p_unused;
    cols_tile(A, lo + i, j, tau_unused, p_unused);
    if (j != cur_j) {
      Lp = A.limbs + A.ids[j];
      p = Lp->p;
      p2 = Lp->p2;
      if (INV) ls = LastStage{Lp->ninv, Lp->ninv_s, Lp->zn, Lp->zn_s};
      if (REDUCE) {
        bhi = Lp->bhi;
        blo = Lp->blo;
      }
      const ulonglong2* tab = INV ? Lp->zi + ((1u << A.logn) - P) : Lp->om;
      if (cur_j != 0xffffffffu) consumer_sync<NT>();
      for (u32 k = tid; k < P; k += NT) {
        const ulonglong2 v = __ldg(tab + k);
        sts128(tw_base + 16 * k, v.x, v.y);
      }
      consumer_sync<NT>();
      cur_j = j;
    }
    const u32 s = i % STAGES;
    const u32 buf = base + s * TILE_BYTES;
    mbar_wait(bar_full + 8 * s, (i / STAGES) & 1);
    if (!INV) {
#pragma unroll
      for (int r = 0; r < NR; r++) {
        if (r == 0) cols_round<LOGP, false, 3, 0, REDUCE, ROLL>(buf, tw_base, p, p2, ls, bhi, blo);
        else if (r == 1 && NR > 2) cols_round<LOGP, false, 3, 3, false, ROLL>(buf, tw_base, p, p2, ls, bhi, blo);
        else cols_round<LOGP, false, REM, 3 * (NR - 1), false, ROLL>(buf, tw_base, p, p2, ls, bhi, blo);
        if (r < NR - 1) consumer_sync<NT>();
      }
    } else {
#pragma unroll
      for (int r = NR - 1; r >= 0; r--) {
        if (r == 0) cols_round<LOGP, true, 3, 0, false, ROLL>(buf, tw_base, p, p2, ls, bhi, blo);
        else if (r == 1 && NR > 2) cols_round<LOGP, true, 3, 3, false, ROLL>(buf, tw_base, p, p2, ls, bhi, blo);
        else cols_round<LOGP, true, REM, 3 * (NR - 1), false, ROLL>(buf, tw_base, p, p2, ls, bhi, blo);
        if (r > 0) consumer_sync<NT>();
      }
    }
    fence_proxy_async();
    mbar_arrive(bar_done + 8 * s);
  }
}

}
```

Baseline: 3697.

## Fuse forward NTT row passes into tensor and key-switch TMA kernels

The forward NTT of the extension rows and of the relinearization base is split. Only the column pass runs standalone, and the row pass is folded into the consumers: the fused tensor/inverse-NTT kernel and the key-switch MAC kernel, which now loads base tiles through TMA. The two extension scale and NTT launches are also batched into a single launch over contiguous buffers. The goal is to cut full read/write round trips and kernel launches, at the cost of more shared memory for twiddles and base tiles and a weighted work split that may unbalance blocks.

```diff
diff --git a/fhe_rs_b200/csrc/capi.cu b/fhe_rs_b200/csrc/capi.cu
--- a/fhe_rs_b200/csrc/capi.cu
+++ b/fhe_rs_b200/csrc/capi.cu
@@ -417,8 +417,23 @@
   return b->mul_basis ? lv.mul_ids : lv.ctx_ids;
 }
 
+bool ks_fused(const fhe_b200_params* par, const fhe_b200_ksk* k, const u64* c2, u32 cts, bool base_post_cols) {
+  const LevelData& kl = par->level(k->ksk_level);
+  const u32 L = k->n_dig, Lk = k->Lk;
+  return !k->log_base && Lk > 1 && switches().ksmac == Switches::KSMAC_FUSED &&
+         ntt_uses_tma(cts * L * Lk, kl.ctx_ids, par->logn, Lk, c2, c2) &&
+         key_switch_tma_serves(L, Lk, kl.ctx_ids, par->logn, base_post_cols);
+}
+
+bool ks_base_after_cols(const fhe_b200_params* par, const fhe_b200_ksk* k, const u64* c2, u32 cts, const u64* out) {
+  const LevelData& cl = par->level(k->ct_level);
+  return k->Lk == cl.L && ks_fused(par, k, c2, cts, true) &&
+         ntt_uses_tma(cts * 2 * cl.L, cl.ctx_ids, par->logn, 1, out, out);
+}
+
 void key_switch_core(const fhe_b200_params* par, const fhe_b200_ksk* k, const u64* c2, u32 cts, const u64* base0,
-                     const u64* base1, u64* out0, u64* out1, u32 out_ct_rows, Workspace& ws, cudaStream_t st) {
+                     const u64* base1, u64* out0, u64* out1, u32 out_ct_rows, Workspace& ws, cudaStream_t st,
+                     bool base_post_cols = false) {
   const LevelData& kl = par->level(k->ksk_level);
   const u32 L = k->n_dig, Lk = k->Lk;
   u64* inter = ws.words(((size_t)cts * L * Lk) << par->logn);
@@ -433,10 +448,11 @@
   for (u32 j = 0; j < Lk; j++) qmin = std::min(qmin, par->moduli[j]);
   const bool reduce = qmax > 4 * qmin - 1 || qmin < (1ull << 8);
   adjacent = Lk > 1 && ntt_uses_tma(cts * L * Lk, kl.ctx_ids, par->logn, Lk, c2, inter);
-  if (adjacent && switches().ksmac == Switches::KSMAC_FUSED &&
+  if (adjacent && ks_fused(par, k, c2, cts, base_post_cols) &&
       launch_key_switch_tma(c2, inter, k->k0, k->k1, base0, base1, out0, out1, cts, L, Lk, out_ct_rows, kl.ctx_ids,
-                            par->d_limbs, par->logn, reduce, st))
+                            par->d_limbs, par->logn, reduce, st, base_post_cols))
     return;
+  if (base_post_cols) throw CudaFail{cudaErrorNotSupported, "post-cols key-switch bases need the fused key switch"};
   launch_ntt(c2, inter, cts * L * Lk, kl.ctx_ids, par->d_limbs, par->logn, false, Lk, reduce, st, true, adjacent, L);
   }
   launch_ksmac(inter, k->k0, k->k1, base0, base1, out0, out1, cts, L, Lk, out_ct_rows, kl.ctx_ids, par->d_limbs,
@@ -444,16 +460,17 @@
 }
 
 void key_switch_apply(const fhe_b200_params* par, const fhe_b200_ksk* k, const u64* c2, u32 cts, u64* out,
-                      int base_mode, u64* base, Workspace& ws, cudaStream_t st) {
+                      int base_mode, u64* base, Workspace& ws, cudaStream_t st, bool base_post_cols = false) {
   const LevelData& cl = par->level(k->ct_level);
   const u32 L = cl.L, Lk = k->Lk, logn = par->logn;
   const size_t row = (size_t)1 << logn;
   if (Lk == L) {
     const u64* b0 = base_mode == 1 ? out : base_mode == 2 ? base : nullptr;
     const u64* b1 = base_mode == 1 ? out + L * row : nullptr;
-    key_switch_core(par, k, c2, cts, b0, b1, out, out + L * row, 2 * L, ws, st);
+    key_switch_core(par, k, c2, cts, b0, b1, out, out + L * row, 2 * L, ws, st, base_post_cols && base_mode == 1);
     return;
   }
+  if (base_post_cols) throw CudaFail{cudaErrorNotSupported, "post-cols key-switch bases need a key at the ciphertext level"};
   u64* cur = ws.words((size_t)cts * 2 * Lk * row);
   key_switch_core(par, k, c2, cts, nullptr, nullptr, cur, cur + Lk * row, 2 * Lk, ws, st);
   const LevelData& kl = par->level(k->ksk_level);
@@ -480,10 +497,10 @@
               u64* out1, int split, Workspace& ws, cudaStream_t st) {
   const u32 L = lv.L, E = lv.E, K = lv.K, logn = par->logn;
   const size_t row = (size_t)1 << logn;
-  u64* A_l = ws.words((size_t)cts * 2 * L * row);
-  u64* A_r = ws.words((size_t)cts * 2 * L * row);
-  u64* X_l = ws.words((size_t)cts * 2 * E * row);
-  u64* X_r = ws.words((size_t)cts * 2 * E * row);
+  u64* A_l = ws.words((size_t)cts * 4 * L * row);
+  u64* A_r = A_l + (size_t)cts * 2 * L * row;
+  u64* X_l = ws.words((size_t)cts * 4 * E * row);
+  u64* X_r = X_l + (size_t)cts * 2 * E * row;
   u64* T = ws.words((size_t)cts * 3 * K * row);
   RowIds ext_ids;
   std::memset(&ext_ids, 0, sizeof(ext_ids));
@@ -491,11 +508,13 @@
   for (u32 j = 0; j < E; j++) ext_ids.ids[j] = lv.mul_ids.ids[L + j];
   launch_ntt(a, A_l, cts * 2 * L, lv.ctx_ids, par->d_limbs, logn, true, 1, false, st);
   launch_ntt(b, A_r, cts * 2 * L, lv.ctx_ids, par->d_limbs, logn, true, 1, false, st);
-  launch_scale(lv.ext.dev, par->d_limbs, A_l, X_l, nullptr, cts * 2, E, L, E, 0, logn, st);
-  launch_scale(lv.ext.dev, par->d_limbs, A_r, X_r, nullptr, cts * 2, E, L, E, 0, logn, st);
-  launch_ntt(X_l, X_l, cts * 2 * E, ext_ids, par->d_limbs, logn, false, 1, false, st);
-  launch_ntt(X_r, X_r, cts * 2 * E, ext_ids, par->d_limbs, logn, false, 1, false, st);
-  if (!launch_tensor_inverse_ntt(a, b, X_l, X_r, T, cts, L, K, lv.mul_ids, par->d_limbs, logn, st)) {
+  launch_scale(lv.ext.dev, par->d_limbs, A_l, X_l, nullptr, cts * 4, E, L, E, 0, logn, st);
+  const bool x_cols = tensor_inverse_ntt_serves(a, b, X_l, X_r, T, cts, L, K, lv.mul_ids, logn) &&
+                      ntt_uses_tma(cts * 4 * E, ext_ids, logn, 1, X_l, X_l);
+  if (x_cols) launch_ntt_fwd_cols(X_l, cts * 4 * E, ext_ids, par->d_limbs, logn, st);
+  else launch_ntt(X_l, X_l, cts * 4 * E, ext_ids, par->d_limbs, logn, false, 1, false, st);
+  if (!launch_tensor_inverse_ntt(a, b, X_l, X_r, T, cts, L, K, lv.mul_ids, par->d_limbs, logn, st, x_cols)) {
+    if (x_cols) throw CudaFail{cudaErrorNotSupported, "post-cols extension rows need the fused tensor kernel"};
     launch_tensor(a, b, X_l, X_r, T, cts, L, L, L, K, lv.mul_ids, par->d_limbs, logn, st);
     launch_ntt(T, T, cts * 3 * K, lv.mul_ids, par->d_limbs, logn, true, 1, false, st);
   }
@@ -1216,8 +1235,10 @@
     u64* o = mod_switch ? ws.words((size_t)n * 2 * L * row) : out2->d + (size_t)c0 * 2 * L * row;
     u64* c2 = ws.words((size_t)n * L * row);
     mul_core(par, lv, a->d + (size_t)c0 * 2 * L * row, b->d + (size_t)c0 * 2 * L * row, n, o, c2, 1, ws, st);
-    launch_ntt(o, o, n * 2 * (u32)L, lv.ctx_ids, par->d_limbs, par->logn, false, 1, false, st);
-    key_switch_apply(par, rk, c2, n, o, 1, nullptr, ws, st);
+    const bool post_cols = ks_base_after_cols(par, rk, c2, n, o);
+    if (post_cols) launch_ntt_fwd_cols(o, n * 2 * (u32)L, lv.ctx_ids, par->d_limbs, par->logn, st);
+    else launch_ntt(o, o, n * 2 * (u32)L, lv.ctx_ids, par->d_limbs, par->logn, false, 1, false, st);
+    key_switch_apply(par, rk, c2, n, o, 1, nullptr, ws, st, post_cols);
     if (mod_switch) {
       launch_ntt(o, o, n * 2 * (u32)L, lv.ctx_ids, par->d_limbs, par->logn, true, 1, false, st);
       u64* dst = out2->d + (size_t)c0 * 2 * (L - 1) * row;
diff --git a/fhe_rs_b200/csrc/engine.hpp b/fhe_rs_b200/csrc/engine.hpp
--- a/fhe_rs_b200/csrc/engine.hpp
+++ b/fhe_rs_b200/csrc/engine.hpp
@@ -56,9 +56,13 @@
 void launch_ntt(const u64* in, u64* out, u32 n_rows, const RowIds& ids, const LimbDev* limbs, u32 logn,
                 bool inverse, u32 in_div, bool reduce_on_load, cudaStream_t st, bool lazy_out = false,
                 bool digit_adjacent = false, u32 n_dig = 1);
+void launch_ntt_fwd_cols(u64* x, u32 n_rows, const RowIds& ids, const LimbDev* limbs, u32 logn, cudaStream_t st);
 
 bool launch_tensor_inverse_ntt(const u64* a, const u64* b, const u64* xa, const u64* xb, u64* T, u32 cts, u32 L, u32 K,
-                               const RowIds& mul_ids, const LimbDev* limbs, u32 logn, cudaStream_t st);
+                               const RowIds& mul_ids, const LimbDev* limbs, u32 logn, cudaStream_t st,
+                               bool x_post_cols = false);
+bool tensor_inverse_ntt_serves(const u64* a, const u64* b, const u64* xa, const u64* xb, const u64* T, u32 cts, u32 L,
+                               u32 K, const RowIds& mul_ids, u32 logn);
 
 enum EwOp { EW_ADD = 0, EW_SUB = 1, EW_NEG = 2 };
 void launch_ew(EwOp op, u64* a, const u64* b, size_t n_rows, const RowIds& ids, const LimbDev* limbs, u32 logn,
@@ -103,7 +107,9 @@
 
 bool launch_key_switch_tma(const u64* c2, u64* inter, const u64* k0, const u64* k1, const u64* base0,
                            const u64* base1, u64* out0, u64* out1, u32 cts, u32 n_dig, u32 Lk, u32 out_ct_rows,
-                           const RowIds& ids, const LimbDev* limbs, u32 logn, bool reduce, cudaStream_t st);
+                           const RowIds& ids, const LimbDev* limbs, u32 logn, bool reduce, cudaStream_t st,
+                           bool base_post_cols);
+bool key_switch_tma_serves(u32 n_dig, u32 Lk, const RowIds& ids, u32 logn, bool base_post_cols);
 
 void launch_decompose(const u64* in, u64* out, size_t polys, u32 n_dig, u32 log_base, u32 logn, cudaStream_t st);
 
diff --git a/fhe_rs_b200/csrc/ntt.cu b/fhe_rs_b200/csrc/ntt.cu
--- a/fhe_rs_b200/csrc/ntt.cu
+++ b/fhe_rs_b200/csrc/ntt.cu
@@ -284,7 +284,8 @@
 }
 
 bool launch_ntt_tma(const u64* in, u64* out, u32 n_rows, const RowIds& ids, const LimbDev* limbs, u32 logn, bool inverse,
-                    u32 in_div, bool reduce_on_load, cudaStream_t st, bool lazy_out, bool digit_adjacent, u32 n_dig) {
+                    u32 in_div, bool reduce_on_load, cudaStream_t st, bool lazy_out, bool digit_adjacent, u32 n_dig,
+                    bool cols_only = false) {
   const u32 lpp = ids.limbs_per_poly;
   if (logn < 13 || logn > 15 || !tensor_map_encoder()) return false;
   if (n_rows % lpp != 0 || (in_div != 1 && in_div != lpp)) return false;
@@ -307,7 +308,7 @@
       first.reduce_on_load = reduce_on_load;
       second.lazy_out = lazy_out;
       run_tma_cols_for<false>(in, in_rows, out, n_rows, first, st);
-      run_tma_rows<false>(out, n_rows, out, n_rows, second, st);
+      if (!cols_only) run_tma_rows<false>(out, n_rows, out, n_rows, second, st);
     } else {
       if (reduce_on_load || in_div != 1) return false;
       run_tma_rows<true>(in, in_rows, out, n_rows, first, st);
@@ -331,7 +332,7 @@
 }
 
 bool launch_tensor_intt_tma(const u64* a, const u64* b, const u64* xa, const u64* xb, u64* T, u32 cts, u32 L, u32 K,
-                            const RowIds& mul_ids, const LimbDev* limbs, u32 logn, cudaStream_t st) {
+                            const RowIds& mul_ids, const LimbDev* limbs, u32 logn, bool x_post_cols, cudaStream_t st) {
   constexpr u32 R = 1u << kRowsRlog;
   const u32 E = K - L;
   try {
@@ -343,6 +344,7 @@
     A.limbs = limbs; A.cts = cts; A.L = L; A.K = K; A.logn = logn;
     A.tiles_per_row = (1u << (logn - 6)) / R;
     A.items_total = K * A.tiles_per_row * cts;
+    A.x_post_cols = x_post_cols ? 1 : 0;
     for (int i = 0; i < kMaxPos; i++) A.ids[i] = mul_ids.ids[i];
     run_tensor_rows<2, 2>(ma, mb, mxa, mxb, mo, A, st);
     NttTmaArgs C;
@@ -357,17 +359,22 @@
 }
 
 template <int STAGES>
-void run_ks_rows_mac(const CUtensorMap& mi, const CUtensorMap& m0, const CUtensorMap& m1, const KsRowsArgs& A,
-                     cudaStream_t st) {
+void run_ks_rows_mac(const CUtensorMap& mi, const CUtensorMap& m0, const CUtensorMap& m1, const CUtensorMap& mb,
+                     const KsRowsArgs& A, cudaStream_t st) {
   using Cfg = KsRowsCfg<STAGES>;
   auto k = ks_rows_mac_tma_kernel<STAGES, 3>;
-  const size_t smem = Cfg::smem(A.n_dig);
+  const size_t smem = Cfg::smem(A.n_dig, A.n_dig + 2 * A.base_tiles);
   ensure_dynamic_smem((const void*)k, smem);
   int per_sm = 0;
   FHE_CUDA(cudaOccupancyMaxActiveBlocksPerMultiprocessor(&per_sm, (const void*)k, Cfg::NT + 32, smem));
   const u32 grid = (u32)std::min<u64>(A.items_total, (u64)sm_count() * std::max(per_sm, 1));
-  k<<<grid, Cfg::NT + 32, smem, st>>>(mi, m0, m1, A);
-  g_launches++;
+  k<<<grid, Cfg::NT + 32, smem, st>>>(mi, m0, m1, mb, A);
+  g_launches++;
+}
+
+size_t ks_rows_mac_smem(u32 n_dig, bool base_tiles) {
+  const u32 nt = n_dig + (base_tiles ? 2 : 0);
+  return switches().ks_stages >= 3 ? KsRowsCfg<3>::smem(n_dig, nt) : KsRowsCfg<2>::smem(n_dig, nt);
 }
 
 }
@@ -381,32 +388,43 @@
   return sw.ntt == Switches::NTT_TMA || n_rows / lpp >= 8;
 }
 
+bool tensor_inverse_ntt_serves(const u64* a, const u64* b, const u64* xa, const u64* xb, const u64* T, u32 cts, u32 L,
+                               u32 K, const RowIds& mul_ids, u32 logn) {
+  return !switches().no_tensor_fusion && K > L && ntt_uses_tma(cts * 3 * K, mul_ids, logn, 1, T, T) &&
+         !((reinterpret_cast<uintptr_t>(a) | reinterpret_cast<uintptr_t>(b) | reinterpret_cast<uintptr_t>(xa) |
+            reinterpret_cast<uintptr_t>(xb)) & 127);
+}
+
 bool launch_tensor_inverse_ntt(const u64* a, const u64* b, const u64* xa, const u64* xb, u64* T, u32 cts, u32 L, u32 K,
-                               const RowIds& mul_ids, const LimbDev* limbs, u32 logn, cudaStream_t st) {
-  if (switches().no_tensor_fusion || K <= L || !ntt_uses_tma(cts * 3 * K, mul_ids, logn, 1, T, T)) return false;
-  if ((reinterpret_cast<uintptr_t>(a) | reinterpret_cast<uintptr_t>(b) | reinterpret_cast<uintptr_t>(xa) |
-       reinterpret_cast<uintptr_t>(xb)) & 127)
-    return false;
-  return launch_tensor_intt_tma(a, b, xa, xb, T, cts, L, K, mul_ids, limbs, logn, st);
+                               const RowIds& mul_ids, const LimbDev* limbs, u32 logn, cudaStream_t st, bool x_post_cols) {
+  if (!tensor_inverse_ntt_serves(a, b, xa, xb, T, cts, L, K, mul_ids, logn)) return false;
+  return launch_tensor_intt_tma(a, b, xa, xb, T, cts, L, K, mul_ids, limbs, logn, x_post_cols, st);
+}
+
+bool key_switch_tma_serves(u32 n_dig, u32 Lk, const RowIds& ids, u32 logn, bool base_post_cols) {
+  return logn >= 13 && logn <= 15 && tensor_map_encoder() && ids.limbs_per_poly == Lk && n_dig > 0 && n_dig <= 256 &&
+         ks_rows_mac_smem(n_dig, base_post_cols) <= 227 * 1024;
 }
 
 bool launch_key_switch_tma(const u64* c2, u64* inter, const u64* k0, const u64* k1, const u64* base0,
                            const u64* base1, u64* out0, u64* out1, u32 cts, u32 n_dig, u32 Lk, u32 out_ct_rows,
-                           const RowIds& ids, const LimbDev* limbs, u32 logn, bool reduce, cudaStream_t st) {
+                           const RowIds& ids, const LimbDev* limbs, u32 logn, bool reduce, cudaStream_t st,
+                           bool base_post_cols) {
   const int stages = switches().ks_stages >= 3 ? 3 : 2;
   using Cfg = KsRowsCfg<2>;
   const u32 n_rows = cts * n_dig * Lk;
-  if (logn < 13 || logn > 15 || !tensor_map_encoder() || ids.limbs_per_poly != Lk || n_dig == 0 || n_dig > 256)
+  if (!key_switch_tma_serves(n_dig, Lk, ids, logn, base_post_cols)) return false;
+  if ((reinterpret_cast<uintptr_t>(c2) | reinterpret_cast<uintptr_t>(inter) | reinterpret_cast<uintptr_t>(k0) |
+       reinterpret_cast<uintptr_t>(k1) | (base_post_cols ? reinterpret_cast<uintptr_t>(base0) : 0)) & 127)
     return false;
-  if ((reinterpret_cast<uintptr_t>(c2) | reinterpret_cast<uintptr_t>(inter) | reinterpret_cast<uintptr_t>(k0) |
-       reinterpret_cast<uintptr_t>(k1)) & 127)
+  if (base_post_cols && (!base0 || !base1 || base1 < base0 || ((base1 - base0) & (((size_t)1 << logn) - 1))))
     return false;
-  if ((stages == 3 ? KsRowsCfg<3>::smem(n_dig) : Cfg::smem(n_dig)) > 227 * 1024) return false;
   CUtensorMap m0, m1;
   if (!box_map(&m0, k0, (u64)Lk * n_dig, logn, Cfg::TC, n_dig) || !box_map(&m1, k1, (u64)Lk * n_dig, logn, Cfg::TC, n_dig))
     return false;
   try {
     const CUtensorMap mi = rows_map(inter, n_rows, logn, 4 * Cfg::R);
+    const CUtensorMap mb = base_post_cols ? rows_map(base0, (u64)cts * out_ct_rows, logn, 4 * Cfg::R) : mi;
     NttTmaArgs C;
     std::memset(&C, 0, sizeof(C));
     C.limbs = limbs;
@@ -426,13 +444,22 @@
     A.cts = cts; A.n_dig = n_dig; A.Lk = Lk; A.out_ct_rows = out_ct_rows; A.logn = logn;
     A.tiles_per_row = (1u << logn) / Cfg::TC;
     A.items_total = Lk * A.tiles_per_row * cts;
+    A.base_tiles = base_post_cols ? 1 : 0;
+    A.base1_rows = base_post_cols ? (u32)((base1 - base0) >> logn) : 0;
     for (int i = 0; i < kMaxPos; i++) A.ids[i] = ids.ids[i];
-    if (stages == 3) run_ks_rows_mac<3>(mi, m0, m1, A, st);
-    else run_ks_rows_mac<2>(mi, m0, m1, A, st);
+    if (stages == 3) run_ks_rows_mac<3>(mi, m0, m1, mb, A, st);
+    else run_ks_rows_mac<2>(mi, m0, m1, mb, A, st);
   } catch (const TmaFail&) {
     return false;
   }
   return true;
+}
+
+void launch_ntt_fwd_cols(u64* x, u32 n_rows, const RowIds& ids, const LimbDev* limbs, u32 logn, cudaStream_t st) {
+  if (n_rows == 0) return;
+  if (!ntt_uses_tma(n_rows, ids, logn, 1, x, x) ||
+      !launch_ntt_tma(x, x, n_rows, ids, limbs, logn, false, 1, false, st, false, false, 1, true))
+    throw CudaFail{cudaErrorNotSupported, "a forward cols pass alone needs the TMA kernels"};
 }
 
 void launch_ntt(const u64* in, u64* out, u32 n_rows, const RowIds& ids, const LimbDev* limbs, u32 logn,
diff --git a/fhe_rs_b200/csrc/ntt_tma.cuh b/fhe_rs_b200/csrc/ntt_tma.cuh
--- a/fhe_rs_b200/csrc/ntt_tma.cuh
+++ b/fhe_rs_b200/csrc/ntt_tma.cuh
@@ -589,6 +589,7 @@
   u32 cts, L, K, logn;
   u32 tiles_per_row;
   u32 items_total;
+  u32 x_post_cols;
   unsigned short ids[kMaxPos];
 };
 
@@ -599,7 +600,7 @@
   static constexpr u32 TILE_BYTES = 512 * R;
   static constexpr u32 STAGE_BYTES = 4 * TILE_BYTES;
   static constexpr u32 TW_PAIRS = 63 * R;
-  static constexpr u32 SMEM = STAGES * STAGE_BYTES + TW_PAIRS * 16 + 2 * STAGES * 8 + 1024;
+  static constexpr u32 SMEM = STAGES * STAGE_BYTES + 2 * TW_PAIRS * 16 + 2 * STAGES * 8 + 1024;
 };
 
 template <int RLOG, int STAGES, int MINB>
@@ -612,8 +613,9 @@
   constexpr u32 R = Cfg::R, NT = Cfg::NT, TILE_BYTES = Cfg::TILE_BYTES, STAGE_BYTES = Cfg::STAGE_BYTES;
   extern __shared__ unsigned char smem_raw[];
   const u32 base = (smem_u32(smem_raw) + 1023u) & ~1023u;
+  constexpr u32 FW = Cfg::TW_PAIRS * 16;
   const u32 tw_base = base + STAGES * STAGE_BYTES;
-  const u32 bar_full = tw_base + Cfg::TW_PAIRS * 16;
+  const u32 bar_full = tw_base + 2 * FW;
   const u32 bar_done = bar_full + STAGES * 8;
   if (threadIdx.x == 0) {
 #pragma unroll
@@ -625,8 +627,16 @@
   }
   __syncthreads();
 
-  const u32 lo = (u32)(((u64)A.items_total * blockIdx.x) / gridDim.x);
-  const u32 hi = (u32)(((u64)A.items_total * (blockIdx.x + 1)) / gridDim.x);
+  u32 lo, hi;
+  {
+    const u64 P = A.x_post_cols ? (u64)A.L * A.tiles_per_row * A.cts : A.items_total;
+    const u64 W = 3 * P + 7 * ((u64)A.items_total - P);
+    auto item_at = [&](u64 c) -> u32 {
+      return (u32)(c <= 3 * P ? (c + 2) / 3 : P + (c - 3 * P + 6) / 7);
+    };
+    lo = item_at(W * blockIdx.x / gridDim.x);
+    hi = item_at(W * (blockIdx.x + 1) / gridDim.x);
+  }
   const u32 n = hi - lo;
   const u32 box_rows_per_row = (1u << A.logn) >> 4;
   const u32 E = A.K - A.L;
@@ -708,21 +718,26 @@
   bool fresh = true;
   LimbDev M = A.limbs[0];
   const u32 logn1 = A.logn - 6;
+  bool ext = false;
   for (u32 i = 0; i < n; i++) {
     if (fresh) {
       const u32 j = w.jt / A.tiles_per_row, tau = w.jt - j * A.tiles_per_row;
       M = A.limbs[A.ids[j]];
-      const ulonglong2* tab = M.zi;
+      ext = A.x_post_cols && j >= A.L;
       const u32 row0 = tau * R;
       if (i) consumer_sync<NT>();
-#pragma unroll
-      for (int tl = 0; tl < 6; tl++) {
-        const u32 s = logn1 + tl;
-        const u32 g0 = ((1u << A.logn) - (2u << s)) + (row0 << tl);
-        for (u32 k = tid; k < (R << tl); k += NT) {
-          const ulonglong2 v = __ldg(tab + g0 + k);
-          const u32 dst = tl < 3 ? k : (k & ((1u << (tl >= 3 ? tl - 3 : 0)) - 1)) * (8 * R) + (k >> (tl >= 3 ? tl - 3 : 0));
-          sts128(tw_base + 16 * (R * ((1u << tl) - 1) + dst), v.x, v.y);
+#pragma unroll 1
+      for (u32 fwd = 0; fwd < (ext ? 2u : 1u); fwd++) {
+        const ulonglong2* tab = fwd ? M.om : M.zi;
+#pragma unroll
+        for (int tl = 0; tl < 6; tl++) {
+          const u32 s = logn1 + tl;
+          const u32 g0 = (fwd ? (1u << s) : ((1u << A.logn) - (2u << s))) + (row0 << tl);
+          for (u32 k = tid; k < (R << tl); k += NT) {
+            const ulonglong2 v = __ldg(tab + g0 + k);
+            const u32 dst = tl < 3 ? k : (k & ((1u << (tl >= 3 ? tl - 3 : 0)) - 1)) * (8 * R) + (k >> (tl >= 3 ? tl - 3 : 0));
+            sts128(tw_base + fwd * FW + 16 * (R * ((1u << tl) - 1) + dst), v.x, v.y);
+          }
         }
       }
       consumer_sync<NT>();
@@ -731,6 +746,45 @@
     const u32 s = i % STAGES;
     const u32 buf = base + s * STAGE_BYTES;
     mbar_wait(bar_full + 8 * s, (i / STAGES) & 1);
+    u64 v[8];
+    ulonglong2 tw[7];
+    if (ext) {
+      tw[0] = lds128(FW + tw0);
+      tw[1] = lds128(FW + tw1);
+      tw[2] = lds128(FW + tw1 + 16);
+#pragma unroll
+      for (int m = 0; m < 4; m++) tw[3 + m] = lds128(FW + tw2 + 16 * m);
+#pragma unroll 1
+      for (u32 t = 0; t < 4; t++) {
+        const u32 tb = buf + t * TILE_BYTES;
+#pragma unroll
+        for (int e = 0; e < 8; e++) v[e] = lds64(tb + off0[e]);
+        fwd_stages<3>(v, tw, p, p2);
+#pragma unroll
+        for (int e = 0; e < 8; e++) sts64(tb + off0[e], v[e]);
+      }
+      consumer_sync<NT>();
+      tw[0] = lds128(FW + tw3);
+      tw[1] = lds128(FW + tw4);
+      tw[2] = lds128(FW + tw4 + 16 * 8 * R);
+#pragma unroll
+      for (int m = 0; m < 4; m++) tw[3 + m] = lds128(FW + tw5 + 16 * 8 * R * m);
+#pragma unroll 1
+      for (u32 t = 0; t < 4; t++) {
+        const u32 tb = buf + t * TILE_BYTES;
+#pragma unroll
+        for (int k = 0; k < 4; k++) {
+          const ulonglong2 q = lds128(tb + off1[k]);
+          v[2 * k] = q.x;
+          v[2 * k + 1] = q.y;
+        }
+        fwd_stages<3>(v, tw, p, p2);
+#pragma unroll
+        for (int e = 0; e < 8; e++) v[e] = fwd_final<false>(v[e], p, p2, 0);
+#pragma unroll
+        for (int k = 0; k < 4; k++) sts128(tb + off1[k], v[2 * k], v[2 * k + 1]);
+      }
+    }
 #pragma unroll 1
     for (u32 k = 0; k < 4; k++) {
       const u32 i = 64 * b + 8 * x + 2 * k;
@@ -751,8 +805,6 @@
       sts128(o + 2 * TILE_BYTES, c1x, c1y);
       sts128(o + TILE_BYTES, c2x, c2y);
     }
-    u64 v[8];
-    ulonglong2 tw[7];
     tw[0] = lds128(tw3);
     tw[1] = lds128(tw4);
     tw[2] = lds128(tw4 + 16 * 8 * R);
@@ -799,6 +851,8 @@
   u32 cts, n_dig, Lk, out_ct_rows, logn;
   u32 tiles_per_row;
   u32 items_total;
+  u32 base_tiles;
+  u32 base1_rows;
   unsigned short ids[kMaxPos];
 };
 
@@ -810,22 +864,24 @@
   static constexpr u32 GROUPS = 16;
   static constexpr u32 NT = GROUPS * 8 * R;
   static constexpr u32 TW_PAIRS = 63 * R;
-  static constexpr size_t smem(u32 nd) {
-    return (size_t)STAGES * nd * TILE_BYTES + 2 * (size_t)nd * TC * 8 + TW_PAIRS * 16 + 2 * STAGES * 8 + 8 + 1024;
+  static constexpr size_t smem(u32 nd, u32 nt) {
+    return (size_t)STAGES * nt * TILE_BYTES + 2 * (size_t)nd * TC * 8 + TW_PAIRS * 16 + 2 * STAGES * 8 + 8 + 1024;
   }
 };
 
 template <int STAGES, int MINB>
 __global__ void __launch_bounds__(KsRowsCfg<STAGES>::NT + 32, MINB)
     ks_rows_mac_tma_kernel(const __grid_constant__ CUtensorMap tm_in, const __grid_constant__ CUtensorMap tm_k0,
-                           const __grid_constant__ CUtensorMap tm_k1, const KsRowsArgs A) {
+                           const __grid_constant__ CUtensorMap tm_k1, const __grid_constant__ CUtensorMap tm_base,
+                           const KsRowsArgs A) {
   using namespace tma;
   using Cfg = KsRowsCfg<STAGES>;
   constexpr u32 R = Cfg::R, TC = Cfg::TC, NT = Cfg::NT, TILE_BYTES = Cfg::TILE_BYTES, GROUPS = Cfg::GROUPS;
   extern __shared__ unsigned char smem_raw[];
   const u32 nd = A.n_dig;
+  const u32 nt = nd + 2 * A.base_tiles;
   const u32 base = (smem_u32(smem_raw) + 1023u) & ~1023u;
-  const u32 stage_bytes = nd * TILE_BYTES;
+  const u32 stage_bytes = nt * TILE_BYTES;
   const u32 k0_base = base + STAGES * stage_bytes;
   const u32 k1_base = k0_base + nd * TC * 8;
   const u32 tw_base = k1_base + nd * TC * 8;
@@ -852,6 +908,7 @@
   if (threadIdx.x >= NT) {
     if (threadIdx.x != NT) return;
     prefetch_map(&tm_in);
+    if (A.base_tiles) prefetch_map(&tm_base);
     TileWalk wl;
     wl.init(lo, A.cts);
     for (u32 i = 0; i < n; i++) {
@@ -863,6 +920,13 @@
       for (u32 d = 0; d < nd; d++)
         load_2d(base + s * stage_bytes + d * TILE_BYTES, &tm_in, 0, (row0 + d) * box_rows_per_row + tau * (4 * R),
                 bar_full + 8 * s);
+      if (A.base_tiles) {
+        const u32 brow = wl.p * A.out_ct_rows + j;
+        load_2d(base + s * stage_bytes + nd * TILE_BYTES, &tm_base, 0, brow * box_rows_per_row + tau * (4 * R),
+                bar_full + 8 * s);
+        load_2d(base + s * stage_bytes + (nd + 1) * TILE_BYTES, &tm_base, 0,
+                (brow + A.base1_rows) * box_rows_per_row + tau * (4 * R), bar_full + 8 * s);
+      }
       wl.next();
     }
     return;
@@ -922,11 +986,11 @@
       consumer_sync<NT>();
     }
     const size_t oi = (((size_t)w.p * A.out_ct_rows + j) << A.logn) + tau * TC + c;
-    const u64 bv = bsrc ? bsrc[oi] : 0;
+    const u64 bv = bsrc && !A.base_tiles ? bsrc[oi] : 0;
     const u32 s = i % STAGES;
     const u32 ring = base + s * stage_bytes;
     mbar_wait(bar_full + 8 * s, (i / STAGES) & 1);
-    for (u32 d = g; d < nd; d += GROUPS) {
+    for (u32 d = g; d < nt; d += GROUPS) {
       const u32 a0 = ring + d * TILE_BYTES + off0, a1 = ring + d * TILE_BYTES + off1;
       u64 v[8];
 #pragma unroll
@@ -958,7 +1022,7 @@
     acc.clear();
 #pragma unroll 2
     for (u32 d = 0; d < nd; d++) acc.mac(lds64(ring + d * TILE_BYTES + offc), lds64(key_c + d * TC * 8));
-    acc.add64(bv);
+    acc.add64(A.base_tiles ? lds64(ring + (nd + o) * TILE_BYTES + offc) : bv);
     dst[oi] = acc.reduce(*Mp);
     mbar_arrive(bar_done + 8 * s);
     fresh = w.next();
```

After: 3749, median of 6. 1.01x the previous value.
